# codex-storage/nim-groth16

Hardware: AMD Instinct MI355X
Metric: proofs/sec (BN254 Groth16, 2^20-constraint circuit) (higher is better)
Workload: dtype u32 (254-bit Montgomery: 8x32-bit limbs; 9x29-bit limbs in the bucket accumulation); 1 GPU; BN254 2^20-constraint synthetic R1CS (squaring chain, m=2^20-2), full prove: buildABC + 6 NTT + 4 G1 MSM + 1 G2 MSM, snarkjs flavour, 1 proof/step/GPU (3 proofs in flight per GPU, one shared key); mode=replica, nvars=1048576, domain_log2=20

## Files before the change

### include/g16hip.h

```cpp
#ifndef G16HIP_H
#define G16HIP_H

#include <stddef.h>
#include <stdint.h>

#ifdef __cplusplus
extern "C" {
#endif

#define G16_OK 0
#define G16_EINVAL (-1)
#define G16_ENODEV (-2)
#define G16_EHIP (-3)
#define G16_ENOMEM (-4)
#define G16_ESELFTEST (-5)

typedef struct g16_ctx g16_ctx;
typedef struct g16_points g16_points;

#define G16_SCALARS_MONT 1u
#define G16_SCALARS_STD 0u
#define G16_SCALARS_DEVICE 2u
#define G16_OUT_PARTIAL 4u
#define G16_OUT_DEVICE 8u
#define G16_NO_HOST_SYNC 32u

int32_t g16_ctx_create(int32_t device, g16_ctx** out);
void g16_ctx_destroy(g16_ctx* ctx);
const char* g16_last_error(const g16_ctx* ctx);
int32_t g16_ctx_set_stream(g16_ctx* ctx, void* hip_stream);
int32_t g16_ctx_synchronize(g16_ctx* ctx);
int32_t g16_ctx_cancel(g16_ctx* ctx);
int32_t g16_selftest(g16_ctx* ctx);

int32_t g16_msm_g1(g16_ctx* ctx, const void* scalars, uint32_t scalar_flags, const void* points, size_t n,
                   void* out_affine);
int32_t g16_msm_g2(g16_ctx* ctx, const void* scalars, uint32_t scalar_flags, const void* points, size_t n,
                   void* out_affine);
int32_t g16_msm_g1_dev(g16_ctx* ctx, const void* d_scalars, uint32_t scalar_flags, const void* d_points, size_t n,
                       void* out_affine);
int32_t g16_msm_g2_dev(g16_ctx* ctx, const void* d_scalars, uint32_t scalar_flags, const void* d_points, size_t n,
                       void* out_affine);
int32_t g16_msm_g1_partial_dev(g16_ctx* ctx, const void* d_scalars, uint32_t scalar_flags, const void* d_points,
                               size_t n, void* out_xyzz);
int32_t g16_msm_g2_partial_dev(g16_ctx* ctx, const void* d_scalars, uint32_t scalar_flags, const void* d_points,
                               size_t n, void* out_xyzz);
int32_t g16_g1_sum_partials(g16_ctx* ctx, const void* xyzz, size_t count, void* out_affine);
int32_t g16_g2_sum_partials(g16_ctx* ctx, const void* xyzz, size_t count, void* out_affine);

int32_t g16_points_register_g1(g16_ctx* ctx, const void* points, size_t n, g16_points** out);
int32_t g16_points_register_g2(g16_ctx* ctx, const void* points, size_t n, g16_points** out);
int32_t g16_points_register_g1_dev(g16_ctx* ctx, const void* d_points, size_t n, g16_points** out);
int32_t g16_points_register_g2_dev(g16_ctx* ctx, const void* d_points, size_t n, g16_points** out);
void g16_points_release(g16_points* pts);
size_t g16_points_count(const g16_points* pts);
size_t g16_points_inf_count(const g16_points* pts);
int32_t g16_points_info(const g16_points* pts, uint32_t* window_bits, uint32_t* ntables);

int32_t g16_points_register_g1_lean(g16_ctx* ctx, const void* points, size_t n, uint32_t table_stride, g16_points** out);
int32_t g16_points_register_g2_lean(g16_ctx* ctx, const void* points, size_t n, uint32_t table_stride, g16_points** out);
int32_t g16_points_register_g1_lean_dev(g16_ctx* ctx, const void* d_points, size_t n, uint32_t table_stride,
                                        g16_points** out);
int32_t g16_points_register_g2_lean_dev(g16_ctx* ctx, const void* d_points, size_t n, uint32_t table_stride,
                                        g16_points** out);
int32_t g16_points_table_bytes(const g16_points* pts, size_t* bytes);
int32_t g16_points_plan(int group, size_t n, uint32_t table_stride, uint32_t* window_bits, uint32_t* ntables,
                        size_t* bytes);
int32_t g16_msm_points(g16_ctx* ctx, const g16_points* pts, const void* scalars, uint32_t flags, void* out);

int32_t g16_points_check_g1(g16_ctx* ctx, const void* points, size_t n, size_t* first_bad);
int32_t g16_points_check_g2(g16_ctx* ctx, const void* points, size_t n, size_t* first_bad);

int32_t g16_fixed_base_g1(g16_ctx* ctx, const void* scalars, uint32_t scalar_flags, size_t n, void* out_points);
int32_t g16_fixed_base_g2(g16_ctx* ctx, const void* scalars, uint32_t scalar_flags, size_t n, void* out_points);

typedef struct {
  uint32_t nvars, npubs, nconstraints;
  uint32_t flavour;
  const uint32_t* row[3];
  const uint32_t* col[3];
  const void* val[3];
  size_t nnz[3];
  uint32_t flags;
  const void *alpha, *beta, *gamma, *delta, *tau;
} g16_setup_desc;
typedef struct {
  void *alpha1, *beta1, *delta1;
  void *beta2, *gamma2, *delta2;
  void* pointsIC;
  void *pointsA1, *pointsB1;
  void* pointsB2;
  void* pointsC1;
  void* pointsH1;
} g16_setup_points;
int32_t g16_setup_log2_domain(const g16_setup_desc* desc, uint32_t* log2_domain);
int32_t g16_fake_setup(g16_ctx* ctx, const g16_setup_desc* desc, g16_setup_points* out);
int32_t g16_lagrange_fr(g16_ctx* ctx, uint32_t log2n, uint32_t first, uint32_t step, size_t count, const void* tau,
                        const void* scale, void* out);
int32_t g16_powers_fr(g16_ctx* ctx, const void* base, const void* scale, size_t count, void* out);

typedef struct g16_r1cs_desc_s g16_r1cs_desc;
typedef struct g16_ptau_desc_s g16_ptau_desc;
int32_t g16_points_intt_g1(g16_ctx* ctx, const void* points, uint32_t log2n, void* out);
int32_t g16_points_intt_g2(g16_ctx* ctx, const void* points, uint32_t log2n, void* out);
int32_t g16_circuit_setup(g16_ctx* ctx, const g16_r1cs_desc* r1cs, const g16_ptau_desc* ptau, const void* delta,
                          g16_setup_points* out);

int32_t g16_ntt_fr(g16_ctx* ctx, const void* src, void* dst, uint32_t log2n, int32_t inverse);
int32_t g16_ntt_fr_dev(g16_ctx* ctx, const void* d_src, void* d_dst, uint32_t log2n, int32_t inverse);

#define G16_FLAVOUR_JENSGROTH 0u
#define G16_FLAVOUR_SNARKJS 1u
int32_t g16_quotient(g16_ctx* ctx, const void* Az, const void* Bz, const void* Cz, uint32_t log2n, uint32_t flavour,
                     void* out);
int32_t g16_quotient_dev(g16_ctx* ctx, const void* d_Az, const void* d_Bz, const void* d_Cz, uint32_t log2n,
                         uint32_t flavour, void* d_out);

typedef struct g16_pkey g16_pkey;
typedef struct {
  uint32_t matrix;
  uint32_t row;
  uint32_t col;
  uint32_t reserved;
  uint8_t value[32];
} g16_coeff;
typedef struct {
  uint32_t nvars, npubs;
  uint32_t log2_domain;
  uint32_t flavour;
  const void *pointsA1, *pointsB1;
  const void* pointsB2;
  const void* pointsC1;
  const void* pointsH1;
  const g16_coeff* coeffs;
  size_t ncoeffs;
  const void *alpha1, *beta1, *delta1;
  const void *beta2, *delta2;
  uint32_t shard_index, shard_count;
} g16_pkey_desc;
typedef struct {
  uint8_t pi_a[64];
  uint8_t pi_b[128];
  uint8_t pi_c[64];
} g16_proof;
int32_t g16_pkey_create(g16_ctx* ctx, const g16_pkey_desc* desc, g16_pkey** out);
int32_t g16_pkey_create_zkey(g16_ctx* ctx, const g16_pkey_desc* desc, const void* section4, size_t section4_bytes,
                             g16_pkey** out);
int32_t g16_pkey_create_lean(g16_ctx* ctx, const g16_pkey_desc* desc, uint32_t table_stride, g16_pkey** out);
int32_t g16_pkey_create_zkey_lean(g16_ctx* ctx, const g16_pkey_desc* desc, const void* section4, size_t section4_bytes,
                                  uint32_t table_stride, g16_pkey** out);
void g16_pkey_destroy(g16_pkey* key);
int32_t g16_pkey_inf_counts(const g16_pkey* key, size_t out[8]);
int32_t g16_pkey_b1_fold(const g16_pkey* key, size_t out[3]);
int32_t g16_pkey_b1_sparse(const g16_pkey* key, size_t out[3]);
int32_t g16_prove(g16_ctx* ctx, const g16_pkey* key, const void* witness, uint32_t flags, const void* mask_r,
                  const void* mask_s, g16_proof* out);
#define G16_PARTIALS_BYTES 768
int32_t g16_prove_partials(g16_ctx* ctx, const g16_pkey* key, const void* witness, uint32_t flags, void* out_partials);
int32_t g16_prove_combine(g16_ctx* ctx, const g16_pkey* key, const void* partials, size_t count, uint32_t flags,
                          const void* mask_r, const void* mask_s, g16_proof* out);
int32_t g16_prove_partials_begin(g16_ctx* ctx, const g16_pkey* key, const void* witness, uint32_t flags,
                                 uint32_t task_mask, void* d_task_out);
int32_t g16_prove_partials_end(g16_ctx* ctx, const g16_pkey* key, const void* d_a1_slice, const void* d_b1_slice,
                               const void* d_c1_slice, uint32_t flags, void* out_partials);
int32_t g16_build_abc(g16_ctx* ctx, const g16_pkey* key, const void* witness, uint32_t flags, void* out_abc);
int32_t g16_pkey_abc_info(const g16_pkey* key, size_t out[11]);
int32_t g16_spmv_fr(g16_ctx* ctx, const uint32_t* row, const uint32_t* col, const void* val, size_t nnz, const void* x,
                    size_t ncols, size_t nrows, void* y);

typedef struct g16_group g16_group;
typedef struct g16_group_pkey g16_group_pkey;
int32_t g16_group_create(const int32_t* devices, int32_t ndev, g16_group** out);
void g16_group_destroy(g16_group* group);
int32_t g16_group_size(const g16_group* group);
const char* g16_group_last_error(const g16_group* group);
int32_t g16_group_pkey_create(g16_group* group, const g16_pkey_desc* desc, g16_group_pkey** out);
int32_t g16_group_pkey_create_lean(g16_group* group, const g16_pkey_desc* desc, uint32_t table_stride,
                                   g16_group_pkey** out);
void g16_group_pkey_destroy(g16_group_pkey* key);
int32_t g16_group_prove(g16_group* group, const g16_group_pkey* key, const void* witness, uint32_t flags,
                        const void* mask_r, const void* mask_s, g16_proof* out);

#define G16_EBUSY (-6)
typedef struct g16_prover g16_prover;
int32_t g16_prover_create(int32_t device, const g16_pkey* key, uint32_t depth, g16_prover** out);
void g16_prover_destroy(g16_prover* p);
const char* g16_prover_last_error(const g16_prover* p);
int32_t g16_prover_submit(g16_prover* p, const void* witness, uint32_t flags, const void* mask_r, const void* mask_s,
                          uint64_t* ticket);
int32_t g16_prover_poll(g16_prover* p, uint64_t ticket);
int32_t g16_prover_collect(g16_prover* p, uint64_t ticket, g16_proof* out);
int32_t g16_host_alloc(int32_t device, size_t bytes, void** out);
void g16_host_free(void* p);

typedef struct g16_vkey g16_vkey;
typedef struct {
  uint32_t npubs;
  const void* alpha1;
  const void* beta2;
  const void* gamma2;
  const void* delta2;
  const void* pointsIC;
} g16_vkey_desc;
#define G16_VERIFY_SUBGROUP 16u
#define G16_GT_BYTES 384
int32_t g16_vkey_create(g16_ctx* ctx, const g16_vkey_desc* desc, g16_vkey** out);
void g16_vkey_destroy(g16_vkey* key);
int32_t g16_verify(g16_ctx* ctx, const g16_vkey* key, const g16_proof* proofs, const void* public_io, uint32_t flags,
                   size_t count, int32_t* status);
int32_t g16_pairing(g16_ctx* ctx, const void* g1_points, const void* g2_points, size_t n, void* out_gt);
int32_t g16_verify_batch(g16_ctx* ctx, const g16_vkey* key, const g16_proof* proofs, const void* public_io,
                         uint32_t flags, size_t count, const void* multipliers, int32_t* result, int32_t* status);

int32_t g16_points_audit_g1(g16_ctx* ctx, const void* points, size_t n, size_t first_bad[3], size_t bad_count[3]);
int32_t g16_points_audit_g2(g16_ctx* ctx, const void* points, size_t n, size_t first_bad[3], size_t bad_count[3]);
int32_t g16_points_pairs_check(g16_ctx* ctx, const void* g1_points, const void* g2_points, size_t n,
                               const void* multipliers, int32_t* result);
#define G16_AUDIT_SECTIONS 13
enum {
  G16_SEC_ALPHA1 = 0, G16_SEC_BETA1, G16_SEC_DELTA1, G16_SEC_BETA2, G16_SEC_GAMMA2, G16_SEC_DELTA2, G16_SEC_POINTS_IC,
  G16_SEC_POINTS_A1, G16_SEC_POINTS_B1, G16_SEC_POINTS_B2, G16_SEC_POINTS_C1, G16_SEC_POINTS_H1, G16_SEC_COEFFS
};
#define G16_AUDIT_CANONICAL 1u
#define G16_AUDIT_CURVE 2u
#define G16_AUDIT_SUBGROUP 4u
#define G16_AUDIT_RELATION 8u
#define G16_AUDIT_SPEC_INFINITY 16u
typedef struct {
  uint32_t failed;
  uint32_t spec_infinity;
  int32_t relation[3];
  uint32_t reserved;
  size_t first_bad[G16_AUDIT_SECTIONS][3];
  size_t bad_count[G16_AUDIT_SECTIONS][3];
} g16_key_report;
int32_t g16_key_audit(g16_ctx* ctx, const g16_pkey_desc* desc, const g16_vkey_desc* vk, const void* section4,
                      size_t section4_bytes, const void* multipliers, g16_key_report* out);

struct g16_r1cs_desc_s {
  uint32_t nvars, npubs, nconstraints;
  uint32_t flavour;
  const uint32_t* row[3];
  const uint32_t* col[3];
  const void* val[3];
  size_t nnz[3];
  uint32_t flags;
};
struct g16_ptau_desc_s {
  uint32_t power;
  const void *tauG1, *tauG2, *alphaTauG1, *betaTauG1, *betaG2;
};
#define G16_PTAU_SECTIONS 5
#define G16_CIRCUIT_RELATIONS 9
enum {
  G16_PTAU_TAU_G1 = 0, G16_PTAU_TAU_G2, G16_PTAU_ALPHA_TAU_G1, G16_PTAU_BETA_TAU_G1, G16_PTAU_BETA_G2
};
enum {
  G16_REL_COEFFS_A = 0, G16_REL_COEFFS_B, G16_REL_SPEC, G16_REL_A1, G16_REL_B1, G16_REL_B2, G16_REL_C1, G16_REL_IC,
  G16_REL_H1
};
#define G16_CIRCUIT_KEY 1u
#define G16_CIRCUIT_PTAU 2u
#define G16_CIRCUIT_COEFFS 4u
#define G16_CIRCUIT_SPEC 8u
#define G16_CIRCUIT_POINTS 16u
typedef struct {
  g16_key_report key;
  size_t ptau_first_bad[G16_PTAU_SECTIONS][3];
  size_t ptau_bad_count[G16_PTAU_SECTIONS][3];
  int32_t relation[G16_CIRCUIT_RELATIONS];
  uint32_t failed;
  size_t first_row[2];
} g16_circuit_report;
int32_t g16_circuit_audit(g16_ctx* ctx, const g16_pkey_desc* desc, const g16_vkey_desc* vk, const void* section4,
                          size_t section4_bytes, const g16_r1cs_desc* r1cs, const g16_ptau_desc* ptau,
                          const void* wire_multipliers, const void* h_multipliers, g16_circuit_report* out);

int32_t g16_points_scale_g1(g16_ctx* ctx, const void* points, size_t n, const void* k, uint32_t flags, void* out);
int32_t g16_points_scale_g2(g16_ctx* ctx, const void* points, size_t n, const void* k, uint32_t flags, void* out);

typedef struct {
  const void *delta1, *delta2;
  const void *pointsC1, *pointsH1;
  size_t nc1, nh1;
} g16_phase2_key;
typedef struct {
  uint8_t delta_after[64];
  uint8_t g1_s[64], g1_sx[64];
  uint8_t g2_spx[128];
} g16_contribution;
typedef struct {
  void *delta1, *delta2, *pointsC1, *pointsH1;
  g16_contribution* record;
} g16_phase2_out;
int32_t g16_key_contribute(g16_ctx* ctx, const g16_phase2_key* key, const void* d, const void* s, uint32_t flags,
                           const void* challenge_g2, g16_phase2_out* out);

#define G16_CHAIN_ARRAYS 9
enum {
  G16_CHAIN_DELTA_AFTER = 0, G16_CHAIN_G1_S, G16_CHAIN_G1_SX, G16_CHAIN_G2_SPX, G16_CHAIN_CHALLENGES,
  G16_CHAIN_FINAL_DELTA1, G16_CHAIN_FINAL_DELTA2, G16_CHAIN_FINAL_POINTS_C1, G16_CHAIN_FINAL_POINTS_H1
};
#define G16_CHAIN_RELATIONS 7
enum {
  G16_CHAIN_ELEMENTS = 0, G16_CHAIN_POK, G16_CHAIN_STEP, G16_CHAIN_LAST, G16_CHAIN_DELTA, G16_CHAIN_C1, G16_CHAIN_H1
};
typedef struct {
  uint32_t failed;
  int32_t relation[G16_CHAIN_RELATIONS];
  size_t first_record[2];
  size_t first_bad[G16_CHAIN_ARRAYS][3];
  size_t bad_count[G16_CHAIN_ARRAYS][3];
  size_t first_infinity[G16_CHAIN_ARRAYS];
} g16_chain_report;
int32_t g16_contributions_verify(g16_ctx* ctx, const g16_phase2_key* initial, const g16_phase2_key* final_,
                                 const g16_contribution* records, const void* challenges_g2, size_t count,
                                 const void* c1_multipliers, const void* h1_multipliers, g16_chain_report* out);

int32_t g16_profile_enable(g16_ctx* ctx, int32_t on);
int32_t g16_profile_reset(g16_ctx* ctx);
int32_t g16_profile_report(g16_ctx* ctx, char* buf, size_t buflen);
int32_t g16_profile_clock(g16_ctx* ctx, double* ghz);

#ifdef __cplusplus
}
#endif
#endif
```

### nim_groth16_amd/_lib.py

```python
from __future__ import annotations

import ctypes
import json
import os
import weakref

_HERE = os.path.dirname(os.path.abspath(__file__))

G16_OK, G16_EINVAL, G16_ENODEV, G16_EHIP, G16_ENOMEM, G16_ESELFTEST, G16_EBUSY = 0, -1, -2, -3, -4, -5, -6
SCALARS_MONT, SCALARS_STD, SCALARS_DEVICE, OUT_PARTIAL, OUT_DEVICE, NO_HOST_SYNC = 1, 0, 2, 4, 8, 32
PARTIALS_BYTES = 768

SYMBOLS = [
    "g16_ctx_create", "g16_ctx_destroy", "g16_last_error", "g16_ctx_set_stream", "g16_ctx_synchronize",
    "g16_selftest", "g16_msm_g1", "g16_msm_g2", "g16_msm_g1_dev", "g16_msm_g2_dev",
    "g16_msm_g1_partial_dev", "g16_msm_g2_partial_dev", "g16_g1_sum_partials", "g16_g2_sum_partials",
    "g16_points_register_g1", "g16_points_register_g2", "g16_points_register_g1_dev",
    "g16_points_register_g2_dev", "g16_points_release", "g16_points_count", "g16_points_inf_count", "g16_points_info", "g16_msm_points",
    "g16_points_check_g1", "g16_points_check_g2", "g16_fixed_base_g1", "g16_fixed_base_g2", "g16_quotient", "g16_quotient_dev", "g16_pkey_create",
    "g16_pkey_create_zkey", "g16_pkey_destroy", "g16_pkey_inf_counts", "g16_prove", "g16_build_abc", "g16_pkey_abc_info", "g16_spmv_fr", "g16_prove_partials", "g16_prove_combine",
    "g16_prove_partials_begin", "g16_prove_partials_end",
    "g16_ntt_fr", "g16_ntt_fr_dev", "g16_profile_enable", "g16_profile_reset", "g16_profile_report", "g16_profile_clock",
    "g16_vkey_create", "g16_vkey_destroy", "g16_verify", "g16_verify_batch", "g16_pairing",
    "g16_ctx_cancel", "g16_group_create", "g16_group_destroy", "g16_group_size", "g16_group_last_error",
    "g16_group_pkey_create", "g16_group_pkey_destroy", "g16_group_prove",
    "g16_prover_create", "g16_prover_destroy", "g16_prover_last_error", "g16_prover_submit", "g16_prover_poll",
    "g16_prover_collect", "g16_host_alloc", "g16_host_free",
    "g16_points_register_g1_lean", "g16_points_register_g2_lean", "g16_points_register_g1_lean_dev",
    "g16_points_register_g2_lean_dev", "g16_points_table_bytes", "g16_points_plan", "g16_pkey_create_lean",
    "g16_pkey_create_zkey_lean", "g16_group_pkey_create_lean",
    "g16_setup_log2_domain", "g16_fake_setup", "g16_lagrange_fr", "g16_powers_fr",
    "g16_points_audit_g1", "g16_points_audit_g2", "g16_points_pairs_check", "g16_key_audit",
    "g16_pkey_b1_fold", "g16_pkey_b1_sparse", "g16_circuit_audit",
    "g16_points_intt_g1", "g16_points_intt_g2", "g16_circuit_setup",
    "g16_points_scale_g1", "g16_points_scale_g2", "g16_key_contribute", "g16_contributions_verify",
]
VERIFY_SUBGROUP = 16
GT_BYTES = 384


class PkeyDesc(ctypes.Structure):
    _fields_ = [("nvars", ctypes.c_uint32), ("npubs", ctypes.c_uint32), ("log2_domain", ctypes.c_uint32),
                ("flavour", ctypes.c_uint32),
                ("pointsA1", ctypes.c_void_p), ("pointsB1", ctypes.c_void_p), ("pointsB2", ctypes.c_void_p),
                ("pointsC1", ctypes.c_void_p), ("pointsH1", ctypes.c_void_p),
                ("coeffs", ctypes.c_void_p), ("ncoeffs", ctypes.c_size_t),
                ("alpha1", ctypes.c_void_p), ("beta1", ctypes.c_void_p), ("delta1", ctypes.c_void_p),
                ("beta2", ctypes.c_void_p), ("delta2", ctypes.c_void_p),
                ("shard_index", ctypes.c_uint32), ("shard_count", ctypes.c_uint32)]


class VkeyDesc(ctypes.Structure):
    _fields_ = [("npubs", ctypes.c_uint32), ("alpha1", ctypes.c_void_p), ("beta2", ctypes.c_void_p),
                ("gamma2", ctypes.c_void_p), ("delta2", ctypes.c_void_p), ("pointsIC", ctypes.c_void_p)]


class SetupDesc(ctypes.Structure):
    _fields_ = [("nvars", ctypes.c_uint32), ("npubs", ctypes.c_uint32), ("nconstraints", ctypes.c_uint32),
                ("flavour", ctypes.c_uint32),
                ("row", ctypes.c_void_p * 3), ("col", ctypes.c_void_p * 3), ("val", ctypes.c_void_p * 3),
                ("nnz", ctypes.c_size_t * 3), ("flags", ctypes.c_uint32),
                ("alpha", ctypes.c_void_p), ("beta", ctypes.c_void_p), ("gamma", ctypes.c_void_p),
                ("delta", ctypes.c_void_p), ("tau", ctypes.c_void_p)]


SETUP_POINTS = ("alpha1", "beta1", "delta1", "beta2", "gamma2", "delta2", "pointsIC", "pointsA1", "pointsB1", "pointsB2",
                "pointsC1", "pointsH1")


class SetupPoints(ctypes.Structure):
    _fields_ = [(name, ctypes.c_void_p) for name in SETUP_POINTS]


AUDIT_SECTIONS = ("alpha1", "beta1", "delta1", "beta2", "gamma2", "delta2", "pointsIC", "pointsA1", "pointsB1", "pointsB2",
                  "pointsC1", "pointsH1", "coeffs")
AUDIT_CHECKS = ("canonical", "curve", "subgroup")
AUDIT_RELATIONS = ("pointsB1~pointsB2", "beta1~beta2", "delta1~delta2")
AUDIT_CANONICAL, AUDIT_CURVE, AUDIT_SUBGROUP, AUDIT_RELATION, AUDIT_SPEC_INFINITY = 1, 2, 4, 8, 16


class KeyReportC(ctypes.Structure):
    _fields_ = [("failed", ctypes.c_uint32), ("spec_infinity", ctypes.c_uint32), ("relation", ctypes.c_int32 * 3),
                ("reserved", ctypes.c_uint32),
                ("first_bad", (ctypes.c_size_t * 3) * len(AUDIT_SECTIONS)),
                ("bad_count", (ctypes.c_size_t * 3) * len(AUDIT_SECTIONS))]


class KeyReport:

    def __init__(self, failed, spec_infinity, relation, first_bad, bad_count):
        self.failed, self.spec_infinity, self.relation = failed, spec_infinity, list(relation)
        self.first_bad, self.bad_count = first_bad, bad_count

    @property
    def ok(self) -> bool:
        return self.failed == 0

    def as_dict(self) -> dict:
        return {"failed": self.failed, "spec_infinity": self.spec_infinity, "relation": self.relation,
                "first_bad": self.first_bad, "bad_count": self.bad_count}

    def findings(self):
        out = []
        for s, name in enumerate(AUDIT_SECTIONS):
            for k, check in enumerate(AUDIT_CHECKS):
                if self.bad_count[s][k]:
                    what = {"canonical": "is not a canonical encoding", "curve": "is not on the curve",
                            "subgroup": "is not in the order-r subgroup"}[check]
                    more = self.bad_count[s][k] - 1
                    out.append(f"{name}[{self.first_bad[s][k]}] {what}" + (f" (and {more} more)" if more else ""))
        for k, name in enumerate(AUDIT_RELATIONS):
            if self.relation[k] == 0:
                out.append(f"{name}: not the same multiples of the two generators")
        for s in range(6):
            if self.spec_infinity >> s & 1:
                out.append(f"{AUDIT_SECTIONS[s]} is the point at infinity")
        return out

    def __str__(self):
        if self.ok:
            skipped = [AUDIT_RELATIONS[k] for k in range(3) if self.relation[k] < 0]
            return "key audit: ok" + (f" (not run: {', '.join(skipped)})" if skipped else "")
        return "key audit: FAILED\n" + "\n".join("  " + f for f in self.findings())


class R1csDesc(ctypes.Structure):
    _fields_ = [("nvars", ctypes.c_uint32), ("npubs", ctypes.c_uint32), ("nconstraints", ctypes.c_uint32),
                ("flavour", ctypes.c_uint32),
                ("row", ctypes.c_void_p * 3), ("col", ctypes.c_void_p * 3), ("val", ctypes.c_void_p * 3),
                ("nnz", ctypes.c_size_t * 3), ("flags", ctypes.c_uint32)]


class PtauDesc(ctypes.Structure):
    _fields_ = [("power", ctypes.c_uint32), ("tauG1", ctypes.c_void_p), ("tauG2", ctypes.c_void_p),
                ("alphaTauG1", ctypes.c_void_p), ("betaTauG1", ctypes.c_void_p), ("betaG2", ctypes.c_void_p)]


PTAU_SECTIONS = ("tauG1", "tauG2", "alphaTauG1", "betaTauG1", "betaG2")
PTAU_GROUP = {"tauG1": 1, "tauG2": 2, "alphaTauG1": 1, "betaTauG1": 1, "betaG2": 2}
CIRCUIT_RELATIONS = ("COEFFS_A", "COEFFS_B", "SPEC", "A1", "B1", "B2", "C1", "IC", "H1")
CIRCUIT_KEY, CIRCUIT_PTAU, CIRCUIT_COEFFS, CIRCUIT_SPEC, CIRCUIT_POINTS = 1, 2, 4, 8, 16


class CircuitReportC(ctypes.Structure):
    _fields_ = [("key", KeyReportC),
                ("ptau_first_bad", (ctypes.c_size_t * 3) * len(PTAU_SECTIONS)),
                ("ptau_bad_count", (ctypes.c_size_t * 3) * len(PTAU_SECTIONS)),
                ("relation", ctypes.c_int32 * len(CIRCUIT_RELATIONS)), ("failed", ctypes.c_uint32),
                ("first_row", ctypes.c_size_t * 2)]


class CircuitReport:

    def __init__(self, key: KeyReport, ptau_first_bad, ptau_bad_count, relation, failed, first_row):
        self.key, self.ptau_first_bad, self.ptau_bad_count = key, ptau_first_bad, ptau_bad_count
        self.relation, self.failed, self.first_row = list(relation), failed, list(first_row)

    @property
    def ok(self) -> bool:
        return self.failed == 0

    def as_dict(self) -> dict:
        return {"key": self.key.as_dict(), "ptau_first_bad": self.ptau_first_bad, "ptau_bad_count": self.ptau_bad_count,
                "relation": self.relation, "failed": self.failed, "first_row": self.first_row}

    def findings(self):
        out = list(self.key.findings())
        for s, name in enumerate(PTAU_SECTIONS):
            for k, check in enumerate(AUDIT_CHECKS):
                if self.ptau_bad_count[s][k]:
                    what = {"canonical": "is not a canonical encoding", "curve": "is not on the curve",
                            "subgroup": "is not in the order-r subgroup"}[check]
                    more = self.ptau_bad_count[s][k] - 1
                    out.append(f"ptau {name}[{self.ptau_first_bad[s][k]}] {what}" + (f" (and {more} more)" if more else ""))
        for m in range(2):
            if self.relation[m] == 0:
                out.append(f"coeffs: matrix {'AB'[m]} differs from the r1cs first at row {self.first_row[m]}")
        if self.relation[2] == 0:
            out.append("alpha1 / beta1 / beta2 are not those of the powers of tau (or its first powers are not the generators)")
        for k in range(3, len(CIRCUIT_RELATIONS)):
            if self.relation[k] == 0:
                out.append(f"points{CIRCUIT_RELATIONS[k]} does not belong to the circuit")
        return out

    def __str__(self):
        if self.ok:
            skipped = [AUDIT_RELATIONS[k] for k in range(3) if self.key.relation[k] < 0]
            skipped += [CIRCUIT_RELATIONS[k] for k in range(len(CIRCUIT_RELATIONS)) if self.relation[k] < 0]
            return "circuit audit: ok" + (f" (not run: {', '.join(skipped)})" if skipped else "")
        return "circuit audit: FAILED\n" + "\n".join("  " + f for f in self.findings())


class Phase2Key(ctypes.Structure):
    _fields_ = [("delta1", ctypes.c_void_p), ("delta2", ctypes.c_void_p), ("pointsC1", ctypes.c_void_p),
                ("pointsH1", ctypes.c_void_p), ("nc1", ctypes.c_size_t), ("nh1", ctypes.c_size_t)]


class ContributionC(ctypes.Structure):
    _fields_ = [("delta_after", ctypes.c_uint8 * 64), ("g1_s", ctypes.c_uint8 * 64), ("g1_sx", ctypes.c_uint8 * 64),
                ("g2_spx", ctypes.c_uint8 * 128)]


CONTRIBUTION_BYTES = 320
assert ctypes.sizeof(ContributionC) == CONTRIBUTION_BYTES


class Phase2Out(ctypes.Structure):
    _fields_ = [("delta1", ctypes.c_void_p), ("delta2", ctypes.c_void_p), ("pointsC1", ctypes.c_void_p),
                ("pointsH1", ctypes.c_void_p), ("record", ctypes.POINTER(ContributionC))]


CHAIN_ARRAYS = ("delta_after", "g1_s", "g1_sx", "g2_spx", "challenges", "final delta1", "final delta2", "final pointsC1",
                "final pointsH1")
CHAIN_RELATIONS = ("ELEMENTS", "POK", "STEP", "LAST", "DELTA", "C1", "H1")


class ChainReportC(ctypes.Structure):
    _fields_ = [("failed", ctypes.c_uint32), ("relation", ctypes.c_int32 * len(CHAIN_RELATIONS)),
                ("first_record", ctypes.c_size_t * 2),
                ("first_bad", (ctypes.c_size_t * 3) * len(CHAIN_ARRAYS)),
                ("bad_count", (ctypes.c_size_t * 3) * len(CHAIN_ARRAYS)),
                ("first_infinity", ctypes.c_size_t * len(CHAIN_ARRAYS))]


class ChainReport:

    def __init__(self, failed, relation, first_record, first_bad, bad_count, first_infinity, transcript=None):
        self.failed, self.relation, self.first_record = failed, list(relation), list(first_record)
        self.first_bad, self.bad_count, self.first_infinity = first_bad, bad_count, list(first_infinity)
        self.transcript = transcript

    @property
    def ok(self) -> bool:
        return self.failed == 0 and self.transcript != 0

    def as_dict(self) -> dict:
        return {"failed": self.failed, "relation": self.relation, "first_record": self.first_record,
                "first_bad": self.first_bad, "bad_count": self.bad_count, "first_infinity": self.first_infinity,
                "transcript": self.transcript}

    def findings(self):
        out = []
        if self.transcript == 0:
            out.append("the transcript hashes are not those of the initial key and the records")
        for a, name in enumerate(CHAIN_ARRAYS):
            for k, check in enumerate(AUDIT_CHECKS):
                if self.bad_count[a][k]:
                    what = {"canonical": "is not a canonical encoding", "curve": "is not on the curve",
                            "subgroup": "is not in the order-r subgroup"}[check]
                    more = self.bad_count[a][k] - 1
                    out.append(f"{name}[{self.first_bad[a][k]}] {what}" + (f" (and {more} more)" if more else ""))
            if self.first_infinity[a] is not None:
                out.append(f"{name}[{self.first_infinity[a]}] is the point at infinity")
        if self.relation[1] == 0:
            out.append(f"record {self.first_record[0]}: the proof of knowledge does not hold")
        if self.relation[2] == 0:
            out.append(f"record {self.first_record[1]}: delta_after is not the contribution's multiple of the delta before")
        if self.relation[3] == 0:
            out.append("the final delta1 is not the last record's delta_after")
        if self.relation[4] == 0:
            out.append("the final delta1 / delta2 are not the same multiple of the two generators")
        for k in (5, 6):
            if self.relation[k] == 0:
                out.append(f"the final points{CHAIN_RELATIONS[k]} is not the initial one rescaled by the deltas")
        return out

    def __str__(self):
        if self.ok:
            skipped = [CHAIN_RELATIONS[k] for k in range(len(CHAIN_RELATIONS)) if self.relation[k] < 0]
            return "contribution chain: ok" + (f" (not run: {', '.join(skipped)})" if skipped else "")
        return "contribution chain: FAILED\n" + "\n".join("  " + f for f in self.findings())


class G16Error(RuntimeError):
    def __init__(self, code, msg):
        super().__init__(f"g16hip error {code}: {msg}")
        self.code = code


def lib_path() -> str:
    return os.environ.get("G16HIP_LIB", os.path.join(_HERE, "csrc", "libg16hip.so"))


def device_code_sha16(path: str = None) -> str:
    import hashlib
    import struct
    b = open(path or lib_path(), "rb").read()
    h = hashlib.sha256()
    try:
        assert b[:4] == b"\x7fELF" and b[4] == 2
        shoff = struct.unpack_from("<Q", b, 0x28)[0]
        shentsize, shnum, shstrndx = struct.unpack_from("<HHH", b, 0x3A)

        def sh(i):
            name, _typ, _flags, _addr, off, size = struct.unpack_from("<IIQQQQ", b, shoff + i * shentsize)
            return name, off, size
        _, stro, _ = sh(shstrndx)
        hit = False
        for i in range(shnum):
            n, off, size = sh(i)
            if b[stro + n: b.index(b"\0", stro + n)] == b".hip_fatbin":
                h.update(b[off: off + size])
                hit = True
        assert hit
    except Exception:
        h = hashlib.sha256(b)
    return h.hexdigest()[:16]


_lib = None


def load_library():
    global _lib
    if _lib is not None:
        return _lib
    path = lib_path()
    if not os.path.exists(path):
        raise G16Error(G16_ENODEV, f"{path} not found: build it with `make -C nim_groth16_amd/csrc` "
                                   "(or __graft_entry__.build()); there is no CPU fallback")
    try:
        import torch
    except ImportError:
        pass
    lib = ctypes.CDLL(path)
    vp, u32, i32, sz = ctypes.c_void_p, ctypes.c_uint32, ctypes.c_int32, ctypes.c_size_t
    lib.g16_ctx_create.argtypes = [i32, ctypes.POINTER(vp)]
    lib.g16_ctx_destroy.argtypes = [vp]
    lib.g16_ctx_destroy.restype = None
    lib.g16_last_error.argtypes = [vp]
    lib.g16_last_error.restype = ctypes.c_char_p
    lib.g16_ctx_set_stream.argtypes = [vp, vp]
    lib.g16_ctx_synchronize.argtypes = [vp]
    lib.g16_selftest.argtypes = [vp]
    for name in ("g16_msm_g1", "g16_msm_g2", "g16_msm_g1_dev", "g16_msm_g2_dev",
                 "g16_msm_g1_partial_dev", "g16_msm_g2_partial_dev"):
        getattr(lib, name).argtypes = [vp, vp, u32, vp, sz, vp]
    for name in ("g16_g1_sum_partials", "g16_g2_sum_partials"):
        getattr(lib, name).argtypes = [vp, vp, sz, vp]
    for name in ("g16_points_register_g1", "g16_points_register_g2", "g16_points_register_g1_dev",
                 "g16_points_register_g2_dev"):
        getattr(lib, name).argtypes = [vp, vp, sz, ctypes.POINTER(vp)]
    for name in ("g16_points_register_g1_lean", "g16_points_register_g2_lean", "g16_points_register_g1_lean_dev",
                 "g16_points_register_g2_lean_dev"):
        getattr(lib, name).argtypes = [vp, vp, sz, u32, ctypes.POINTER(vp)]
    lib.g16_points_table_bytes.argtypes = [vp, ctypes.POINTER(sz)]
    lib.g16_points_plan.argtypes = [ctypes.c_int, sz, u32, ctypes.POINTER(u32), ctypes.POINTER(u32), ctypes.POINTER(sz)]
    lib.g16_pkey_create_lean.argtypes = [vp, ctypes.POINTER(PkeyDesc), u32, ctypes.POINTER(vp)]
    lib.g16_pkey_create_zkey_lean.argtypes = [vp, ctypes.POINTER(PkeyDesc), vp, sz, u32, ctypes.POINTER(vp)]
    lib.g16_group_pkey_create_lean.argtypes = [vp, ctypes.POINTER(PkeyDesc), u32, ctypes.POINTER(vp)]
    lib.g16_points_release.argtypes = [vp]
    lib.g16_points_release.restype = None
    lib.g16_points_count.argtypes = [vp]
    lib.g16_points_count.restype = sz
    lib.g16_points_inf_count.argtypes = [vp]
    lib.g16_points_inf_count.restype = sz
    lib.g16_pkey_inf_counts.argtypes = [vp, ctypes.POINTER(sz)]
    lib.g16_pkey_b1_fold.argtypes = [vp, ctypes.POINTER(sz)]
    lib.g16_pkey_b1_sparse.argtypes = [vp, ctypes.POINTER(sz)]
    lib.g16_points_info.argtypes = [vp, ctypes.POINTER(u32), ctypes.POINTER(u32)]
    lib.g16_msm_points.argtypes = [vp, vp, vp, u32, vp]
    lib.g16_points_check_g1.argtypes = [vp, vp, sz, ctypes.POINTER(sz)]
    lib.g16_points_check_g2.argtypes = [vp, vp, sz, ctypes.POINTER(sz)]
    lib.g16_fixed_base_g1.argtypes = [vp, vp, u32, sz, vp]
    lib.g16_fixed_base_g2.argtypes = [vp, vp, u32, sz, vp]
    lib.g16_quotient.argtypes = [vp, vp, vp, vp, u32, u32, vp]
    lib.g16_quotient_dev.argtypes = [vp, vp, vp, vp, u32, u32, vp]
    lib.g16_pkey_create.argtypes = [vp, ctypes.POINTER(PkeyDesc), ctypes.POINTER(vp)]
    lib.g16_pkey_create_zkey.argtypes = [vp, ctypes.POINTER(PkeyDesc), vp, sz, ctypes.POINTER(vp)]
    lib.g16_pkey_destroy.argtypes = [vp]
    lib.g16_pkey_destroy.restype = None
    lib.g16_prove.argtypes = [vp, vp, vp, u32, vp, vp, vp]
    lib.g16_build_abc.argtypes = [vp, vp, vp, u32, vp]
    lib.g16_pkey_abc_info.argtypes = [vp, ctypes.POINTER(sz)]
    lib.g16_spmv_fr.argtypes = [vp, vp, vp, vp, sz, vp, sz, sz, vp]
    lib.g16_prove_partials.argtypes = [vp, vp, vp, u32, vp]
    lib.g16_prove_combine.argtypes = [vp, vp, vp, sz, u32, vp, vp, vp]
    lib.g16_prove_partials_begin.argtypes = [vp, vp, vp, u32, u32, vp]
    lib.g16_prove_partials_end.argtypes = [vp, vp, vp, vp, vp, u32, vp]
    lib.g16_ntt_fr.argtypes = [vp, vp, vp, u32, i32]
    lib.g16_ntt_fr_dev.argtypes = [vp, vp, vp, u32, i32]
    lib.g16_vkey_create.argtypes = [vp, ctypes.POINTER(VkeyDesc), ctypes.POINTER(vp)]
    lib.g16_vkey_destroy.argtypes = [vp]
    lib.g16_vkey_destroy.restype = None
    lib.g16_verify.argtypes = [vp, vp, vp, vp, u32, sz, ctypes.POINTER(i32)]
    lib.g16_verify_batch.argtypes = [vp, vp, vp, vp, u32, sz, vp, ctypes.POINTER(i32), ctypes.POINTER(i32)]
    lib.g16_pairing.argtypes = [vp, vp, vp, sz, vp]
    lib.g16_ctx_cancel.argtypes = [vp]
    lib.g16_group_create.argtypes = [ctypes.POINTER(i32), i32, ctypes.POINTER(vp)]
    lib.g16_group_destroy.argtypes = [vp]
    lib.g16_group_destroy.restype = None
    lib.g16_group_size.argtypes = [vp]
    lib.g16_group_last_error.argtypes = [vp]
    lib.g16_group_last_error.restype = ctypes.c_char_p
    lib.g16_group_pkey_create.argtypes = [vp, ctypes.POINTER(PkeyDesc), ctypes.POINTER(vp)]
    lib.g16_group_pkey_destroy.argtypes = [vp]
    lib.g16_group_pkey_destroy.restype = None
    lib.g16_group_prove.argtypes = [vp, vp, vp, u32, vp, vp, vp]
    lib.g16_prover_create.argtypes = [i32, vp, u32, ctypes.POINTER(vp)]
    lib.g16_prover_destroy.argtypes = [vp]
    lib.g16_prover_destroy.restype = None
    lib.g16_prover_last_error.argtypes = [vp]
    lib.g16_prover_last_error.restype = ctypes.c_char_p
    lib.g16_prover_submit.argtypes = [vp, vp, u32, vp, vp, ctypes.POINTER(ctypes.c_uint64)]
    lib.g16_prover_poll.argtypes = [vp, ctypes.c_uint64]
    lib.g16_prover_collect.argtypes = [vp, ctypes.c_uint64, vp]
    lib.g16_host_alloc.argtypes = [i32, sz, ctypes.POINTER(vp)]
    lib.g16_host_free.argtypes = [vp]
    lib.g16_host_free.restype = None
    lib.g16_profile_enable.argtypes = [vp, i32]
    lib.g16_profile_reset.argtypes = [vp]
    lib.g16_profile_report.argtypes = [vp, ctypes.c_char_p, sz]
    lib.g16_profile_clock.argtypes = [vp, ctypes.POINTER(ctypes.c_double)]
    lib.g16_setup_log2_domain.argtypes = [ctypes.POINTER(SetupDesc), ctypes.POINTER(u32)]
    lib.g16_fake_setup.argtypes = [vp, ctypes.POINTER(SetupDesc), ctypes.POINTER(SetupPoints)]
    lib.g16_lagrange_fr.argtypes = [vp, u32, u32, u32, sz, vp, vp, vp]
    lib.g16_powers_fr.argtypes = [vp, vp, vp, sz, vp]
    lib.g16_points_audit_g1.argtypes = [vp, vp, sz, ctypes.POINTER(sz), ctypes.POINTER(sz)]
    lib.g16_points_audit_g2.argtypes = [vp, vp, sz, ctypes.POINTER(sz), ctypes.POINTER(sz)]
    lib.g16_points_pairs_check.argtypes = [vp, vp, vp, sz, vp, ctypes.POINTER(i32)]
    lib.g16_key_audit.argtypes = [vp, ctypes.POINTER(PkeyDesc), ctypes.POINTER(VkeyDesc), vp, sz, vp,
                                  ctypes.POINTER(KeyReportC)]
    lib.g16_circuit_audit.argtypes = [vp, ctypes.POINTER(PkeyDesc), ctypes.POINTER(VkeyDesc), vp, sz,
                                      ctypes.POINTER(R1csDesc), ctypes.POINTER(PtauDesc), vp, vp,
                                      ctypes.POINTER(CircuitReportC)]
    lib.g16_points_intt_g1.argtypes = [vp, vp, u32, vp]
    lib.g16_points_intt_g2.argtypes = [vp, vp, u32, vp]
    lib.g16_circuit_setup.argtypes = [vp, ctypes.POINTER(R1csDesc), ctypes.POINTER(PtauDesc), vp,
                                      ctypes.POINTER(SetupPoints)]
    lib.g16_points_scale_g1.argtypes = [vp, vp, sz, vp, u32, vp]
    lib.g16_points_scale_g2.argtypes = [vp, vp, sz, vp, u32, vp]
    lib.g16_key_contribute.argtypes = [vp, ctypes.POINTER(Phase2Key), vp, vp, u32, vp, ctypes.POINTER(Phase2Out)]
    lib.g16_contributions_verify.argtypes = [vp, ctypes.POINTER(Phase2Key), ctypes.POINTER(Phase2Key),
                                             ctypes.POINTER(ContributionC), vp, sz, vp, vp, ctypes.POINTER(ChainReportC)]
    for name in SYMBOLS:
        if name not in ("g16_ctx_destroy", "g16_last_error", "g16_points_release", "g16_points_count",
                        "g16_points_inf_count",
                        "g16_pkey_destroy", "g16_vkey_destroy", "g16_group_destroy", "g16_group_last_error",
                        "g16_group_pkey_destroy", "g16_prover_destroy", "g16_prover_last_error", "g16_host_free"):
            getattr(lib, name).restype = i32
    _lib = lib
    return lib


def _buf(b):
    if isinstance(b, int):
        return ctypes.c_void_p(b)
    if isinstance(b, (bytes, bytearray)):
        return ctypes.cast(ctypes.c_char_p(bytes(b)), ctypes.c_void_p) if isinstance(b, bytes) else \
            ctypes.cast((ctypes.c_char * len(b)).from_buffer(b), ctypes.c_void_p)
    if hasattr(b, "ctypes"):
        return ctypes.c_void_p(b.ctypes.data)
    raise TypeError(type(b))


class Context:

    def __init__(self, device: int = 0):
        self._lib = load_library()
        h = ctypes.c_void_p()
        rc = self._lib.g16_ctx_create(device, ctypes.byref(h))
        if rc != G16_OK:
            raise G16Error(rc, "g16_ctx_create failed (no usable HIP device?)")
        self._h = h
        self.device = device
        self._children = weakref.WeakSet()

    def close(self, release_children: bool = False):
        if getattr(self, "_h", None):
            if release_children:
                for child in list(self._children):
                    child._free()
            self._lib.g16_ctx_destroy(self._h)
            self._h = None

    def __del__(self):
        try:
            self.close()
        except Exception:
            pass

    def _check(self, rc):
        if rc != G16_OK:
            raise G16Error(rc, self._lib.g16_last_error(self._h).decode())

    def selftest(self):
        self._check(self._lib.g16_selftest(self._h))

    def set_stream(self, stream_ptr):
        self._check(self._lib.g16_ctx_set_stream(self._h, ctypes.c_void_p(stream_ptr)))

    def synchronize(self):
        self._check(self._lib.g16_ctx_synchronize(self._h))

    def cancel(self):
        self._check(self._lib.g16_ctx_cancel(self._h))

    def msm(self, group: int, scalars, points, n: int, mont: bool = True, device: bool = False,
            partial: bool = False) -> bytes:
        psz = 64 if group == 1 else 128
        out = ctypes.create_string_buffer(2 * psz if partial else psz)
        if partial:
            fn = self._lib.g16_msm_g1_partial_dev if group == 1 else self._lib.g16_msm_g2_partial_dev
        elif device:
            fn = self._lib.g16_msm_g1_dev if group == 1 else self._lib.g16_msm_g2_dev
        else:
            fn = self._lib.g16_msm_g1 if group == 1 else self._lib.g16_msm_g2
        s = _buf(scalars) if n else None
        p = _buf(points) if n else None
        self._check(fn(self._h, s, SCALARS_MONT if mont else SCALARS_STD, p, n, out))
        return out.raw

    def register_points(self, group: int, points, n: int, device: bool = False, table_stride: int = 0) -> "PointSet":
        h = ctypes.c_void_p()
        p = _buf(points) if n else None
        if table_stride:
            name = f"g16_points_register_g{group}_lean" + ("_dev" if device else "")
            self._check(getattr(self._lib, name)(self._h, p, n, table_stride, ctypes.byref(h)))
        else:
            name = f"g16_points_register_g{group}" + ("_dev" if device else "")
            self._check(getattr(self._lib, name)(self._h, p, n, ctypes.byref(h)))
        return PointSet(self, h, group, n)

    def msm_points(self, pts: "PointSet", scalars, mont: bool = True, device: bool = False,
                   partial: bool = False) -> bytes:
        psz = 64 if pts.group == 1 else 128
        out = ctypes.create_string_buffer(2 * psz if partial else psz)
        flags = (SCALARS_MONT if mont else 0) | (SCALARS_DEVICE if device else 0) | (OUT_PARTIAL if partial else 0)
        self._check(self._lib.g16_msm_points(self._h, pts._h, _buf(scalars) if pts.n else None, flags, out))
        return out.raw

    def points_check(self, group: int, points: bytes):
        psz = 64 if group == 1 else 128
        n = len(points) // psz
        bad = ctypes.c_size_t()
        fn = self._lib.g16_points_check_g1 if group == 1 else self._lib.g16_points_check_g2
        self._check(fn(self._h, _buf(points) if n else None, n, ctypes.byref(bad)))
        return None if bad.value == ctypes.c_size_t(-1).value else bad.value

    def points_audit(self, group: int, points: bytes):
        psz = 64 if group == 1 else 128
        assert len(points) % psz == 0
        n = len(points) // psz
        first, count = (ctypes.c_size_t * 3)(), (ctypes.c_size_t * 3)()
        fn = self._lib.g16_points_audit_g1 if group == 1 else self._lib.g16_points_audit_g2
        self._check(fn(self._h, _buf(points) if n else None, n, first, count))
        none = ctypes.c_size_t(-1).value
        return [None if f == none else f for f in first], list(count)

    def pairs_check(self, g1_points: bytes, g2_points: bytes, multipliers) -> bool:
        n = len(g1_points) // 64
        assert len(g1_points) == 64 * n and len(g2_points) == 128 * n and len(multipliers) == n
        zs = b"".join(int(z).to_bytes(16, "little") for z in multipliers)
        res = ctypes.c_int32(-1)
        self._check(self._lib.g16_points_pairs_check(self._h, _buf(g1_points) if n else None,
                                                     _buf(g2_points) if n else None, n, _buf(zs) if n else None,
                                                     ctypes.byref(res)))
        return res.value == 1

    def key_audit(self, desc: PkeyDesc, vk: VkeyDesc = None, section4: bytes = None, multipliers=None) -> KeyReport:
        zs = None
        if isinstance(multipliers, (bytes, bytearray)):
            assert len(multipliers) == 16 * desc.nvars, "one multiplier per wire"
            zs = bytes(multipliers)
        elif multipliers is not None:
            assert len(multipliers) == desc.nvars, "one multiplier per wire"
            zs = b"".join(int(z).to_bytes(16, "little") for z in multipliers)
        rep = KeyReportC()
        self._check(self._lib.g16_key_audit(self._h, ctypes.byref(desc), ctypes.byref(vk) if vk is not None else None,
                                            _buf(section4) if section4 is not None else None,
                                            len(section4) if section4 is not None else 0,
                                            _buf(zs) if zs is not None else None, ctypes.byref(rep)))
        none = ctypes.c_size_t(-1).value
        return KeyReport(rep.failed, rep.spec_infinity, list(rep.relation),
                         [[None if f == none else f for f in row] for row in rep.first_bad],
                         [list(row) for row in rep.bad_count])

    def circuit_audit(self, desc: PkeyDesc, vk, section4, r1cs: R1csDesc, ptau: PtauDesc, wire_multipliers,
                      h_multipliers) -> CircuitReport:
        def enc(zs, n, what):
            if isinstance(zs, (bytes, bytearray)):
                assert len(zs) == 16 * n, f"one {what} multiplier of 16 bytes each"
                return bytes(zs)
            assert len(zs) == n, f"{n} {what} multipliers"
            return b"".join(int(z).to_bytes(16, "little") for z in zs)
        zw = enc(wire_multipliers, desc.nvars, "wire")
        zh = enc(h_multipliers, 1 << min(desc.log2_domain, 28), "h")
        rep = CircuitReportC()
        self._check(self._lib.g16_circuit_audit(self._h, ctypes.byref(desc), ctypes.byref(vk) if vk is not None else None,
                                                _buf(section4) if section4 is not None else None,
                                                len(section4) if section4 is not None else 0,
                                                ctypes.byref(r1cs), ctypes.byref(ptau), _buf(zw), _buf(zh),
                                                ctypes.byref(rep)))
        none = ctypes.c_size_t(-1).value
        fix = lambda rows: [[None if f == none else f for f in row] for row in rows]
        key = KeyReport(rep.key.failed, rep.key.spec_infinity, list(rep.key.relation), fix(rep.key.first_bad),
                        [list(row) for row in rep.key.bad_count])
        return CircuitReport(key, fix(rep.ptau_first_bad), [list(row) for row in rep.ptau_bad_count], list(rep.relation),
                             rep.failed, [None if f == none else f for f in rep.first_row])

    def fixed_base(self, group: int, scalars: bytes, mont: bool = True) -> bytes:
        n = len(scalars) // 32
        psz = 64 if group == 1 else 128
        out = ctypes.create_string_buffer(max(n, 1) * psz)
        fn = self._lib.g16_fixed_base_g1 if group == 1 else self._lib.g16_fixed_base_g2
        self._check(fn(self._h, _buf(scalars) if n else None, SCALARS_MONT if mont else 0, n, out))
        return out.raw[: n * psz]

    def spmv(self, row, col, val, x: bytes, nrows: int) -> bytes:
        import numpy as np
        row = np.ascontiguousarray(row, dtype=np.uint32)
        col = np.ascontiguousarray(col, dtype=np.uint32)
        nnz = len(row)
        if not isinstance(val, (bytes, bytearray)):
            val = np.ascontiguousarray(val, dtype=np.uint8)
        assert len(col) == nnz and (len(val) if isinstance(val, (bytes, bytearray)) else val.size) == 32 * nnz
        out = ctypes.create_string_buffer(max(1, 32 * nrows))
        self._check(self._lib.g16_spmv_fr(self._h, _buf(row) if nnz else None, _buf(col) if nnz else None,
                                          _buf(val) if nnz else None, nnz, _buf(x) if len(x) else None, len(x) // 32,
                                          nrows, out))
        return out.raw[: 32 * nrows]

    def lagrange(self, log2n: int, tau: bytes, first: int = 0, step: int = 1, count: int = None,
                 scale: bytes = None) -> bytes:
        if count is None:
            count = ((1 << log2n) - first + step - 1) // step if step else 1
        out = ctypes.create_string_buffer(max(1, 32 * count))
        self._check(self._lib.g16_lagrange_fr(self._h, log2n, first, step, count, _buf(tau),
                                              _buf(scale) if scale is not None else None, out))
        return out.raw[: 32 * count]

    def powers(self, base: bytes, count: int, scale: bytes = None) -> bytes:
        out = ctypes.create_string_buffer(max(1, 32 * count))
        self._check(self._lib.g16_powers_fr(self._h, _buf(base), _buf(scale) if scale is not None else None, count, out))
        return out.raw[: 32 * count]

    def fake_setup(self, nvars: int, npubs: int, nconstraints: int, flavour: int, matrices, toxic, mont: bool = True):
        import numpy as np
        d = SetupDesc()
        d.nvars, d.npubs, d.nconstraints, d.flavour = nvars, npubs, nconstraints, flavour
        d.flags = SCALARS_MONT if mont else SCALARS_STD
        keep = []
        for k, (rows, wires, vals) in enumerate(matrices):
            rows = np.ascontiguousarray(rows, dtype=np.uint32)
            wires = np.ascontiguousarray(wires, dtype=np.uint32)
            if not isinstance(vals, (bytes, bytearray)):
                vals = np.ascontiguousarray(vals, dtype=np.uint8)
            nnz = len(rows)
            assert len(wires) == nnz and (len(vals) if isinstance(vals, (bytes, bytearray)) else vals.size) == 32 * nnz
            keep += [rows, wires, vals]
            d.nnz[k] = nnz
            if nnz:
                d.row[k], d.col[k], d.val[k] = (_buf(x).value for x in (rows, wires, vals))
        toxic = [bytes(t) for t in toxic]
        d.alpha, d.beta, d.gamma, d.delta, d.tau = (_buf(t).value for t in toxic)
        log2 = ctypes.c_uint32()
        rc = self._lib.g16_setup_log2_domain(ctypes.byref(d), ctypes.byref(log2))
        if rc != G16_OK:
            raise G16Error(rc, "g16_setup_log2_domain failed")
        sizes = dict(alpha1=64, beta1=64, delta1=64, beta2=128, gamma2=128, delta2=128, pointsIC=64 * (npubs + 1),
                     pointsA1=64 * nvars, pointsB1=64 * nvars, pointsB2=128 * nvars,
                     pointsC1=64 * max(0, nvars - npubs - 1), pointsH1=64 << min(log2.value, 40))
        if log2.value + (1 if flavour == 1 else 0) > 28:
            sizes = dict.fromkeys(sizes, 0)
        o = SetupPoints()
        bufs = {}
        for name, nbytes in sizes.items():
            bufs[name] = ctypes.create_string_buffer(max(1, nbytes))
            setattr(o, name, ctypes.cast(bufs[name], ctypes.c_void_p).value)
        self._check(self._lib.g16_fake_setup(self._h, ctypes.byref(d), ctypes.byref(o)))
        return log2.value, {name: bufs[name].raw[: sizes[name]] for name in SETUP_POINTS}

    def points_intt(self, group: int, points: bytes, log2n: int) -> bytes:
        psz = 64 if group == 1 else 128
        assert len(points) == psz << log2n, f"2^{log2n} points of {psz} bytes"
        out = ctypes.create_string_buffer(len(points))
        fn = self._lib.g16_points_intt_g1 if group == 1 else self._lib.g16_points_intt_g2
        self._check(fn(self._h, _buf(points), log2n, out))
        return out.raw

    def circuit_setup(self, r1cs: R1csDesc, ptau: PtauDesc, delta: bytes = None):
        nvars, npubs = r1cs.nvars, r1cs.npubs
        log2 = max(0, (r1cs.nconstraints + npubs).bit_length())
        sizes = dict(alpha1=64, beta1=64, delta1=64, beta2=128, gamma2=128, delta2=128, pointsIC=64 * (npubs + 1),
                     pointsA1=64 * nvars, pointsB1=64 * nvars, pointsB2=128 * nvars,
                     pointsC1=64 * max(0, nvars - npubs - 1), pointsH1=64 << log2)
        if log2 > 24:
            sizes = dict.fromkeys(sizes, 0)
        o = SetupPoints()
        bufs = {}
        for name, nbytes in sizes.items():
            bufs[name] = ctypes.create_string_buffer(max(1, nbytes))
            setattr(o, name, ctypes.cast(bufs[name], ctypes.c_void_p).value)
        self._check(self._lib.g16_circuit_setup(self._h, ctypes.byref(r1cs), ctypes.byref(ptau),
                                                _buf(bytes(delta)) if delta is not None else None, ctypes.byref(o)))
        return log2, {name: bufs[name].raw[: sizes[name]] for name in SETUP_POINTS}

    def points_scale(self, group: int, points: bytes, k: bytes, mont: bool = True) -> bytes:
        psz = 64 if group == 1 else 128
        assert len(points) % psz == 0 and len(k) == 32, f"points of {psz} bytes and a 32-byte scalar"
        out = ctypes.create_string_buffer(max(1, len(points)))
        fn = self._lib.g16_points_scale_g1 if group == 1 else self._lib.g16_points_scale_g2
        self._check(fn(self._h, _buf(bytes(points)), len(points) // psz, _buf(bytes(k)),
                       SCALARS_MONT if mont else SCALARS_STD, out))
        return out.raw[: len(points)]

    @staticmethod
    def _phase2_key(key: dict):
        assert len(key["delta1"]) == 64 and len(key["delta2"]) == 128, "delta1: 64 bytes, delta2: 128 bytes"
        assert len(key["pointsC1"]) % 64 == 0 and len(key["pointsH1"]) % 64 == 0, "G1 points of 64 bytes"
        keep = {name: bytes(key[name]) for name in ("delta1", "delta2", "pointsC1", "pointsH1")}
        pk = Phase2Key()
        for name, b in keep.items():
            setattr(pk, name, ctypes.cast(ctypes.c_char_p(b), ctypes.c_void_p).value if b else None)
        pk.nc1, pk.nh1 = len(keep["pointsC1"]) // 64, len(keep["pointsH1"]) // 64
        return pk, keep

    def key_contribute(self, key: dict, d: bytes, s: bytes, challenge_g2: bytes, mont: bool = True):
        assert len(d) == 32 and len(s) == 32 and len(challenge_g2) == 128
        pk, keep = self._phase2_key(key)
        bufs = {name: ctypes.create_string_buffer(max(1, len(b))) for name, b in keep.items()}
        rec = ContributionC()
        o = Phase2Out()
        for name in bufs:
            setattr(o, name, ctypes.cast(bufs[name], ctypes.c_void_p).value)
        o.record = ctypes.pointer(rec)
        self._check(self._lib.g16_key_contribute(self._h, ctypes.byref(pk), _buf(bytes(d)), _buf(bytes(s)),
                                                 SCALARS_MONT if mont else SCALARS_STD, _buf(bytes(challenge_g2)),
                                                 ctypes.byref(o)))
        return {name: bufs[name].raw[: len(keep[name])] for name in keep}, bytes(rec)

    def contributions_verify(self, initial: dict, final: dict, records, challenges_g2, c1_multipliers,
                             h1_multipliers) -> ChainReport:
        def enc(zs, n, what):
            if isinstance(zs, (bytes, bytearray)):
                assert len(zs) == 16 * n, f"one {what} multiplier of 16 bytes each"
                return bytes(zs)
            assert len(zs) == n, f"{n} {what} multipliers"
            return b"".join(int(z).to_bytes(16, "little") for z in zs)
        records, challenges_g2 = list(records), list(challenges_g2)
        assert len(records) == len(challenges_g2) and all(len(r) == CONTRIBUTION_BYTES for r in records) and \
            all(len(c) == 128 for c in challenges_g2), "one 320-byte record and one 128-byte challenge per contribution"
        ki, keep_i = self._phase2_key(initial)
        kf, keep_f = self._phase2_key(final)
        zc, zh = enc(c1_multipliers, kf.nc1, "c1"), enc(h1_multipliers, kf.nh1, "h1")
        recs = (ContributionC * max(1, len(records))).from_buffer_copy(b"".join(records) or bytes(CONTRIBUTION_BYTES))
        ch = b"".join(challenges_g2)
        rep = ChainReportC()
        self._check(self._lib.g16_contributions_verify(self._h, ctypes.byref(ki), ctypes.byref(kf), recs,
                                                       _buf(ch) if ch else None, len(records),
                                                       _buf(zc) if zc else None, _buf(zh) if zh else None,
                                                       ctypes.byref(rep)))
        none = ctypes.c_size_t(-1).value
        opt = lambda row: [None if f == none else f for f in row]
        return ChainReport(rep.failed, list(rep.relation), opt(rep.first_record), [opt(row) for row in rep.first_bad],
                           [list(row) for row in rep.bad_count], opt(rep.first_infinity))

    def quotient(self, Az, Bz, Cz, log2n: int, flavour: int, out=None, device: bool = False):
        if device:
            self._check(self._lib.g16_quotient_dev(self._h, _buf(Az), _buf(Bz), _buf(Cz), log2n, flavour, _buf(out)))
            return None
        res = ctypes.create_string_buffer(32 << log2n)
        self._check(self._lib.g16_quotient(self._h, _buf(Az), _buf(Bz), _buf(Cz), log2n, flavour, res))
        return res.raw

    def sum_partials(self, group: int, xyzz: bytes, count: int) -> bytes:
        psz = 64 if group == 1 else 128
        out = ctypes.create_string_buffer(psz)
        fn = self._lib.g16_g1_sum_partials if group == 1 else self._lib.g16_g2_sum_partials
        self._check(fn(self._h, _buf(xyzz) if count else None, count, out))
        return out.raw

    def ntt(self, src, log2n: int, inverse: bool, dst=None, device: bool = False):
        n = 1 << log2n
        if device:
            self._check(self._lib.g16_ntt_fr_dev(self._h, _buf(src), _buf(dst), log2n, 1 if inverse else 0))
            return None
        out = ctypes.create_string_buffer(32 * n)
        self._check(self._lib.g16_ntt_fr(self._h, _buf(src), out, log2n, 1 if inverse else 0))
        return out.raw

    def pairing(self, g1_points: bytes, g2_points: bytes) -> bytes:
        n = len(g1_points) // 64
        assert len(g1_points) == 64 * n and len(g2_points) == 128 * n
        out = ctypes.create_string_buffer(max(1, GT_BYTES * n))
        self._check(self._lib.g16_pairing(self._h, _buf(g1_points) if n else None, _buf(g2_points) if n else None,
                                          n, out))
        return out.raw[:GT_BYTES * n]

    def profile(self, on):
        self._check(self._lib.g16_profile_enable(self._h, int(on)))

    def profile_reset(self):
        self._check(self._lib.g16_profile_reset(self._h))

    def profile_clock(self) -> float:
        g = ctypes.c_double()
        self._check(self._lib.g16_profile_clock(self._h, ctypes.byref(g)))
        return g.value

    def profile_report(self) -> dict:
        buf = ctypes.create_string_buffer(1 << 16)
        self._check(self._lib.g16_profile_report(self._h, buf, len(buf)))
        return json.loads(buf.value.decode())


class ProvingKey:

    def __init__(self, ctx: Context, desc: PkeyDesc, keepalive, section4: bytes = None, table_stride: int = 0):
        self.ctx = ctx
        h = ctypes.c_void_p()
        if table_stride and section4 is not None:
            ctx._check(ctx._lib.g16_pkey_create_zkey_lean(ctx._h, ctypes.byref(desc), _buf(section4), len(section4),
                                                          table_stride, ctypes.byref(h)))
        elif table_stride:
            ctx._check(ctx._lib.g16_pkey_create_lean(ctx._h, ctypes.byref(desc), table_stride, ctypes.byref(h)))
        elif section4 is not None:
            ctx._check(ctx._lib.g16_pkey_create_zkey(ctx._h, ctypes.byref(desc), _buf(section4), len(section4),
                                                     ctypes.byref(h)))
        else:
            ctx._check(ctx._lib.g16_pkey_create(ctx._h, ctypes.byref(desc), ctypes.byref(h)))
        self._h = h
        self.nvars, self.npubs, self.log2n = desc.nvars, desc.npubs, desc.log2_domain
        ctx._children.add(self)
        del keepalive

    def _check_len(self, witness):
        if isinstance(witness, (bytes, bytearray)) and len(witness) != 32 * self.nvars:
            raise ValueError(f"wrong witness length: {len(witness)} bytes, expected {32 * self.nvars}")

    def prove(self, witness, mont: bool = True, r: bytes = None, s: bytes = None, device: bool = False, ctx=None):
        c = ctx or self.ctx
        self._check_len(witness)
        out = ctypes.create_string_buffer(256)
        flags = (SCALARS_MONT if mont else 0) | (SCALARS_DEVICE if device else 0)
        c._check(c._lib.g16_prove(c._h, self._h, _buf(witness), flags, _buf(r) if r else None,
                                  _buf(s) if s else None, out))
        raw = out.raw
        return raw[0:64], raw[64:192], raw[192:256]

    def prove_partials(self, witness, mont: bool = True, device: bool = False, out=None, ctx=None):
        c = ctx or self.ctx
        self._check_len(witness)
        flags = (SCALARS_MONT if mont else 0) | (SCALARS_DEVICE if device else 0)
        if out is not None:
            c._check(c._lib.g16_prove_partials(c._h, self._h, _buf(witness), flags | OUT_DEVICE, _buf(out)))
            return None
        buf = ctypes.create_string_buffer(PARTIALS_BYTES)
        c._check(c._lib.g16_prove_partials(c._h, self._h, _buf(witness), flags, buf))
        return buf.raw

    def prove_partials_begin(self, witness, task_mask: int, task_out=None, mont: bool = True, device: bool = False,
                             ctx=None, nosync: bool = False):
        c = ctx or self.ctx
        self._check_len(witness)
        flags = (SCALARS_MONT if mont else 0) | (SCALARS_DEVICE if device else 0) | (NO_HOST_SYNC if nosync else 0)
        c._check(c._lib.g16_prove_partials_begin(c._h, self._h, _buf(witness), flags, task_mask,
                                                 _buf(task_out) if task_out is not None else None))

    def prove_partials_end(self, a1, b1, c1, out=None, ctx=None, nosync: bool = False):
        c = ctx or self.ctx
        ptr = lambda x: _buf(x) if x is not None else None
        if out is not None:
            c._check(c._lib.g16_prove_partials_end(c._h, self._h, ptr(a1), ptr(b1), ptr(c1),
                                                   OUT_DEVICE | (NO_HOST_SYNC if nosync else 0), _buf(out)))
            return None
        buf = ctypes.create_string_buffer(PARTIALS_BYTES)
        c._check(c._lib.g16_prove_partials_end(c._h, self._h, ptr(a1), ptr(b1), ptr(c1), 0, buf))
        return buf.raw

    def prove_combine(self, partials, count: int, r: bytes = None, s: bytes = None, device: bool = False, ctx=None):
        c = ctx or self.ctx
        out = ctypes.create_string_buffer(256)
        c._check(c._lib.g16_prove_combine(c._h, self._h, _buf(partials), count, SCALARS_DEVICE if device else 0,
                                          _buf(r) if r else None, _buf(s) if s else None, out))
        raw = out.raw
        return raw[0:64], raw[64:192], raw[192:256]

    def inf_counts(self) -> dict:
        out = (ctypes.c_size_t * 8)()
        self.ctx._check(self.ctx._lib.g16_pkey_inf_counts(self._h, out))
        v = list(out)
        return {"A1": v[0], "B1": v[1], "B2": v[2], "C1": v[3], "H1": v[4], "B1_and_B2": v[5],
                "compact_A": bool(v[6]), "compact_B": bool(v[7])}

    def b1_fold(self) -> dict:
        out = (ctypes.c_size_t * 3)()
        self.ctx._check(self.ctx._lib.g16_pkey_b1_fold(self._h, out))
        return {"form": ("PLAIN", "EMPTY", "DELTA")[out[0]], "live_b1": out[1], "live_delta": out[2]}

    def b1_sparse(self) -> dict:
        out = (ctypes.c_size_t * 3)()
        self.ctx._check(self.ctx._lib.g16_pkey_b1_sparse(self._h, out))
        return {"sparse": bool(out[0]), "live": out[1], "max": out[2]}

    def abc_info(self) -> dict:
        out = (ctypes.c_size_t * 11)()
        self.ctx._check(self.ctx._lib.g16_pkey_abc_info(self._h, out))
        v = list(out)
        names = ("L<=1", "L=2", "L<=4", "L<=8", "L<=16", "L<=32", "L<=64", "L<=128", "L>128")
        return {"ncoeffs": v[0], "dict_values": v[1], "rows_by_terms": dict(zip(names, v[2:]))}

    def build_abc(self, witness: bytes, mont: bool = True, ctx=None):
        c = ctx or self.ctx
        self._check_len(witness)
        n = 1 << self.log2n
        out = ctypes.create_string_buffer(3 * n * 32)
        c._check(c._lib.g16_build_abc(c._h, self._h, _buf(witness), SCALARS_MONT if mont else 0, out))
        raw = out.raw
        return raw[: 32 * n], raw[32 * n: 64 * n], raw[64 * n:]

    def _free(self):
        if self._h:
            self.ctx._lib.g16_pkey_destroy(self._h)
        self._h = None

    destroy = _free

    def __del__(self):
        try:
            self._free()
        except Exception:
            pass


class DeviceGroup:

    def __init__(self, devices):
        self._lib = load_library()
        arr = (ctypes.c_int32 * len(devices))(*devices)
        h = ctypes.c_void_p()
        rc = self._lib.g16_group_create(arr, len(devices), ctypes.byref(h))
        if rc != G16_OK:
            raise G16Error(rc, "g16_group_create failed")
        self._h, self.devices = h, list(devices)

    def _check(self, rc):
        if rc != G16_OK:
            raise G16Error(rc, self._lib.g16_group_last_error(self._h).decode())

    def size(self) -> int:
        return self._lib.g16_group_size(self._h)

    def load_key(self, desc: PkeyDesc, keepalive=None, table_stride: int = 0) -> "GroupKey":
        h = ctypes.c_void_p()
        if table_stride:
            self._check(self._lib.g16_group_pkey_create_lean(self._h, ctypes.byref(desc), table_stride, ctypes.byref(h)))
        else:
            self._check(self._lib.g16_group_pkey_create(self._h, ctypes.byref(desc), ctypes.byref(h)))
        return GroupKey(self, h, desc.nvars)

    def close(self):
        if getattr(self, "_h", None):
            self._lib.g16_group_destroy(self._h)
            self._h = None

    def __del__(self):
        try:
            self.close()
        except Exception:
            pass


class GroupKey:
    def __init__(self, group: DeviceGroup, handle, nvars: int):
        self.group, self._h, self.nvars = group, handle, nvars

    def prove(self, witness: bytes, mont: bool = True, r: bytes = None, s: bytes = None):
        if len(witness) != 32 * self.nvars:
            raise ValueError(f"wrong witness length: {len(witness)} bytes, expected {32 * self.nvars}")
        out = ctypes.create_string_buffer(256)
        g = self.group
        g._check(g._lib.g16_group_prove(g._h, self._h, _buf(witness), SCALARS_MONT if mont else 0,
                                        _buf(r) if r else None, _buf(s) if s else None, out))
        raw = out.raw
        return raw[0:64], raw[64:192], raw[192:256]

    def destroy(self):
        if self._h:
            self.group._lib.g16_group_pkey_destroy(self._h)
        self._h = None

    def __del__(self):
        try:
            self.destroy()
        except Exception:
            pass


class ProverPool:

    def __init__(self, pkey: ProvingKey, depth: int = 3, device: int = 0):
        self._lib = load_library()
        self.pkey, self.depth, self.device = pkey, depth, device
        h = ctypes.c_void_p()
        rc = self._lib.g16_prover_create(device, pkey._h, depth, ctypes.byref(h))
        if rc != G16_OK:
            raise G16Error(rc, "g16_prover_create failed (sharded key, key of another device, or depth not in 1..8)")
        self._h = h
        self._witness = {}

    def _check(self, rc):
        if rc == G16_EBUSY:
            raise G16Error(rc, f"{self.depth + 1} proofs outstanding: collect one first")
        if rc < 0:
            raise G16Error(rc, self._lib.g16_prover_last_error(self._h).decode())
        return rc

    def submit(self, witness, mont: bool = True, r: bytes = None, s: bytes = None, device: bool = False) -> int:
        self.pkey._check_len(witness)
        if isinstance(witness, HostBuffer) and witness.nbytes < 32 * self.pkey.nvars:
            raise ValueError("host buffer shorter than the witness")
        ptr = ctypes.c_void_p(witness.data_ptr()) if device and hasattr(witness, "data_ptr") else _buf(witness)
        t = ctypes.c_uint64()
        flags = (SCALARS_MONT if mont else 0) | (SCALARS_DEVICE if device else 0)
        self._check(self._lib.g16_prover_submit(self._h, ptr, flags, _buf(r) if r else None,
                                                _buf(s) if s else None, ctypes.byref(t)))
        self._witness[t.value] = witness
        return t.value

    def poll(self, ticket: int) -> bool:
        return self._check(self._lib.g16_prover_poll(self._h, ticket)) == 1

    def collect(self, ticket: int):
        out = ctypes.create_string_buffer(256)
        self._check(self._lib.g16_prover_collect(self._h, ticket, out))
        self._witness.pop(ticket, None)
        raw = out.raw
        return raw[0:64], raw[64:192], raw[192:256]

    def close(self):
        if getattr(self, "_h", None):
            self._lib.g16_prover_destroy(self._h)
            self._h = None
            self._witness.clear()

    def __del__(self):
        try:
            self.close()
        except Exception:
            pass


class HostBuffer:

    def __init__(self, nbytes: int, device: int = 0):
        import numpy as np
        self._lib = load_library()
        p = ctypes.c_void_p()
        rc = self._lib.g16_host_alloc(device, nbytes, ctypes.byref(p))
        if rc != G16_OK:
            raise G16Error(rc, "g16_host_alloc failed")
        self._p, self.nbytes = p, nbytes
        self.array = np.ctypeslib.as_array((ctypes.c_uint8 * nbytes).from_address(p.value))
        self.ctypes = self.array.ctypes

    @classmethod
    def from_bytes(cls, data: bytes, device: int = 0) -> "HostBuffer":
        import numpy as np
        b = cls(len(data), device)
        b.array[:] = np.frombuffer(data, dtype=np.uint8)
        return b

    def __len__(self):
        return self.nbytes

    def free(self):
        if getattr(self, "_p", None):
            self.array = self.ctypes = None
            self._lib.g16_host_free(self._p)
            self._p = None

    def __del__(self):
        try:
            self.free()
        except Exception:
            pass


class VerifyingKey:

    def __init__(self, ctx: Context, npubs: int, alpha1: bytes, beta2: bytes, gamma2: bytes, delta2: bytes,
                 pointsIC: bytes):
        assert len(alpha1) == 64 and len(beta2) == len(gamma2) == len(delta2) == 128
        assert len(pointsIC) == 64 * (npubs + 1), "pointsIC must hold npubs + 1 points"
        self.ctx, self.npubs = ctx, npubs
        bufs = [ctypes.create_string_buffer(x, len(x)) for x in (alpha1, beta2, gamma2, delta2, pointsIC)]
        a = [ctypes.cast(b, ctypes.c_void_p) for b in bufs]
        desc = VkeyDesc(npubs, a[0], a[1], a[2], a[3], a[4])
        h = ctypes.c_void_p()
        ctx._check(ctx._lib.g16_vkey_create(ctx._h, ctypes.byref(desc), ctypes.byref(h)))
        self._h = h
        ctx._children.add(self)

    def verify(self, proofs, public_io: bytes, mont: bool = True, subgroup: bool = False):
        n = len(proofs)
        assert len(public_io) == 32 * n * (self.npubs + 1)
        raw = b"".join(a + b + c for a, b, c in proofs)
        assert len(raw) == 256 * n
        st = (ctypes.c_int32 * max(n, 1))()
        flags = (SCALARS_MONT if mont else 0) | (VERIFY_SUBGROUP if subgroup else 0)
        self.ctx._check(self.ctx._lib.g16_verify(self.ctx._h, self._h, _buf(raw) if n else None,
                                                 _buf(public_io) if n else None, flags, n, st))
        return list(st)[:n]

    def verify_batch(self, proofs, public_io: bytes, mont: bool = True, multipliers=None, want_status: bool = False):
        n = len(proofs)
        assert len(public_io) == 32 * n * (self.npubs + 1)
        raw = b"".join(a + b + c for a, b, c in proofs)
        assert len(raw) == 256 * n
        if multipliers is None:
            import secrets
            multipliers = [secrets.randbelow((1 << 128) - 1) + 1 for _ in range(n)]
        assert len(multipliers) == n, "one multiplier per proof"
        zs = b"".join(int(z).to_bytes(16, "little") for z in multipliers)
        res = ctypes.c_int32(-1)
        st = (ctypes.c_int32 * max(n, 1))() if want_status else None
        flags = SCALARS_MONT if mont else 0
        self.ctx._check(self.ctx._lib.g16_verify_batch(self.ctx._h, self._h, _buf(raw) if n else None,
                                                       _buf(public_io) if n else None, flags, n,
                                                       _buf(zs) if n else None, ctypes.byref(res), st))
        return (res.value == 1, list(st)[:n]) if want_status else res.value == 1

    def _free(self):
        if self._h:
            self.ctx._lib.g16_vkey_destroy(self._h)
        self._h = None

    destroy = _free

    def __del__(self):
        try:
            self._free()
        except Exception:
            pass


def points_plan(group: int, n: int, table_stride: int = 0):
    lib = load_library()
    c, t, b = ctypes.c_uint32(), ctypes.c_uint32(), ctypes.c_size_t()
    rc = lib.g16_points_plan(group, n, table_stride, ctypes.byref(c), ctypes.byref(t), ctypes.byref(b))
    if rc != G16_OK:
        raise G16Error(rc, "g16_points_plan: bad group, or too many points for 31-bit entry indices")
    return c.value, t.value, b.value


class PointSet:

    def __init__(self, ctx: Context, handle, group: int, n: int):
        self.ctx, self._h, self.group, self.n = ctx, handle, group, n
        ctx._children.add(self)

    def inf_count(self) -> int:
        return self.ctx._lib.g16_points_inf_count(self._h)

    def info(self):
        c, w = ctypes.c_uint32(), ctypes.c_uint32()
        self.ctx._check(self.ctx._lib.g16_points_info(self._h, ctypes.byref(c), ctypes.byref(w)))
        return c.value, w.value

    @property
    def table_bytes(self) -> int:
        b = ctypes.c_size_t()
        self.ctx._check(self.ctx._lib.g16_points_table_bytes(self._h, ctypes.byref(b)))
        return b.value

    def _free(self):
        if self._h:
            self.ctx._lib.g16_points_release(self._h)
        self._h = None

    release = _free

    def __del__(self):
        try:
            self._free()
        except Exception:
            pass


_default_ctx = None


def default_context() -> Context:
    global _default_ctx
    if _default_ctx is None:
        _default_ctx = Context(int(os.environ.get("LOCAL_RANK", "0")))
    return _default_ctx
```

### nim_groth16_amd/csrc/g16_env.hpp

```cpp
#pragma once

struct G16Env {
  int msm_window = 0;
  int table_window = 0;
  int msm_seg = 0;
  char msm_sort = 0;
  int g1_lanes[3] = {3, 2, 0};
  char stream_prio[7] = "lhllln";
  int red_slice_log2 = 0;
  int inf_compact_pct = 10;
  int r2_width = -1;
  int ntt_tile = 2048;
  int quotient_first = 1;
  int lanes_after_quotient = 0;
  int g1_batch = 0;
  int mtab = 2;
  int chain_ch = 1;
  int tail_quad = 1;
  int red_chunk = 0;
  int cu_split = 0;
  int heavy_grid = 0;
  int cz_on_the_fly = 1;
  int abc_dict = 1;
  int g2_first = -1;
  int b1_fold = 1;
};
```

### nim_groth16_amd/csrc/g16_internal.hpp

```cpp
#pragma once
#include "../../include/g16hip.h"

#include <hip/hip_runtime.h>

#include <cstdio>
#include <cstring>
#include <map>
#include <string>
#include <vector>


#include "g16_env.hpp"
#include "hip_owners.hpp"
#include "msm_params.hpp"
#include "circuit_setup_plan.hpp"
#include "msm_plan.hpp"
#include "proof_plan.hpp"

const G16Env& g16_env();

struct ProfEntry {
  const char* name;
  Event e0, e1;
};

struct g16_ctx {
  int device = 0;
  hipStream_t stream = nullptr;
  Stream own_stream;
  std::string err;
  struct Buf {
    DevMem<> mem;
    size_t bytes = 0;
    void* p() const { return mem.get(); }
  };
  struct MsmSort {
    Buf buf;
    g16::MsmParams P;
    bool narrow_tail = false;
    uint32_t *count = nullptr, *cursor = nullptr, *offset = nullptr, *xoff = nullptr, *heavy = nullptr,
             *info = nullptr, *entries = nullptr, *perm = nullptr, *ghist = nullptr, *blk_base = nullptr, *tile_hist = nullptr;
    uint2* tmp = nullptr;
    uint32_t* slice_hist = nullptr;
    uint2* tiles2 = nullptr;
    uint2* tiles = nullptr;
    uint2* xseg = nullptr;
  };
  struct MsmLane {
    Stream stream;
    Event done;
    Buf acc;
  };
  MsmSort sort[4];
  MsmLane lane[5];
  Event ev[g16::EV_COUNT];
  Buf stage_s;
  Buf stage_p;
  Buf stage_p29;
  Buf stage_o;
  Buf ntt_tw;
  Buf ntt_tmp;
  Buf coset[2];
  Buf quot;
  Buf prove;
  Buf fb_table[2];
  bool fb_ready[2] = {false, false};
  DevMem<unsigned long long> clk_buf;
  const void* shard_begun = nullptr;
  uint32_t tw_log2n = 0xffffffffu;
  uint32_t coset_log2n[2] = {0xffffffffu, 0xffffffffu};
  bool profiling = false;
  bool prof_accum_only = false;
  std::vector<ProfEntry> prof;
  std::vector<Event> free_events;
};

inline int32_t g16_hip_check(std::string& err, const char* call, hipError_t e) {
  if (e == hipSuccess) return G16_OK;
  err = std::string(call) + ": " + hipGetErrorString(e);
  (void)hipGetLastError();
  return e == hipErrorOutOfMemory ? G16_ENOMEM : G16_EHIP;
}
#define HIPCHK(ctx, call)                                                          \
  do {                                                                             \
    if (int32_t hiprc__ = g16_hip_check((ctx)->err, #call, (call))) return hiprc__; \
  } while (0)

inline void ctx_quiesce(g16_ctx* ctx) {
  if (ctx->stream) (void)hipStreamSynchronize(ctx->stream);
  for (auto& l : ctx->lane)
    if (l.stream) (void)hipStreamSynchronize(l.stream.get());
}
struct SyncOnExit {
  hipStream_t stream;
  ~SyncOnExit() { (void)hipStreamSynchronize(stream); }
};

inline int32_t ctx_enter(g16_ctx* ctx, bool keep_shard = false) {
  HIPCHK(ctx, hipSetDevice(ctx->device));
  if (ctx->shard_begun && !keep_shard) {
    ctx_quiesce(ctx);
    ctx->shard_begun = nullptr;
  }
  return G16_OK;
}
#define CTX_ENTER(ctx)                              \
  do {                                              \
    if (int32_t rc__ = ctx_enter(ctx)) return rc__; \
  } while (0)
#define CTX_ENTER_KEEP(ctx)                               \
  do {                                                    \
    if (int32_t rc__ = ctx_enter(ctx, true)) return rc__; \
  } while (0)

inline int32_t ensure(g16_ctx* ctx, g16_ctx::Buf& b, size_t bytes) {
  if (b.bytes >= bytes) return G16_OK;
  HIPCHK(ctx, hipSetDevice(ctx->device));
  if (b.mem) {
    ctx_quiesce(ctx);
    b.mem.reset();
    b.bytes = 0;
  }
  size_t want = bytes + bytes / 8 + 4096;
  HIPCHK(ctx, dev_alloc(b.mem, want));
  b.bytes = want;
  return G16_OK;
}

#define G16_COMBINE_RES_BYTES 384
constexpr size_t STAGE_O_RESULT = 0, STAGE_O_RESULT_BYTES = G16_PARTIALS_BYTES;
constexpr size_t STAGE_O_COUNTERS = STAGE_O_RESULT + STAGE_O_RESULT_BYTES, STAGE_O_COUNTER_WORDS = 2;
constexpr size_t STAGE_O_COMBINE = 1024;
constexpr size_t STAGE_O_BYTES = 2048;
static_assert(STAGE_O_COUNTERS % 4 == 0 && STAGE_O_COUNTERS + 4 * STAGE_O_COUNTER_WORDS <= STAGE_O_COMBINE &&
                  STAGE_O_COMBINE % 128 == 0 && STAGE_O_COMBINE + G16_COMBINE_RES_BYTES <= STAGE_O_BYTES,
              "the pieces of stage_o overlap or do not fit");
inline int32_t ensure_stage_o(g16_ctx* ctx) { return ensure(ctx, ctx->stage_o, STAGE_O_BYTES); }
inline char* stage_o_at(g16_ctx* ctx, size_t offset) { return (char*)ctx->stage_o.p() + offset; }

template <class Launch>
inline int32_t counted_launch(g16_ctx* ctx, int fill, uint32_t* words, size_t nwords, Launch&& launch) {
  if (int32_t rc = ensure_stage_o(ctx)) return rc;
  uint32_t* d_words = (uint32_t*)stage_o_at(ctx, STAGE_O_COUNTERS);
  HIPCHK(ctx, hipMemsetAsync(d_words, fill, 4 * nwords, ctx->stream));
  if (int32_t rc = launch(d_words)) return rc;
  HIPCHK(ctx, hipMemcpyAsync(words, d_words, 4 * nwords, hipMemcpyDeviceToHost, ctx->stream));
  HIPCHK(ctx, hipStreamSynchronize(ctx->stream));
  return G16_OK;
}

struct ProfScope {
  g16_ctx* ctx;
  bool on;
  ProfEntry e;
  hipStream_t st;
  ProfScope(g16_ctx* c, const char* name, hipStream_t stream = nullptr)
      : ctx(c), on(c->profiling && (!c->prof_accum_only || strncmp(name, "msm_accum", 9) == 0)),
        st(stream ? stream : c->stream) {
    if (!on) return;
    e.name = name;
    auto get = [&](Event& ev) {
      if (!ctx->free_events.empty()) {
        ev = std::move(ctx->free_events.back());
        ctx->free_events.pop_back();
      } else {
        (void)event_create(ev, hipEventDefault);
      }
    };
    get(e.e0);
    get(e.e1);
    (void)hipEventRecord(e.e0.get(), st);
  }
  ~ProfScope() {
    if (!on) return;
    (void)hipEventRecord(e.e1.get(), st);
    ctx->prof.push_back(std::move(e));
  }
};
#define KLAUNCH_ON(ctx, stream_, name, kernel, grid, block, shmem, ...)                        \
  do {                                                                                         \
    ProfScope ps__(ctx, name, stream_);                                                        \
    hipLaunchKernelGGL(kernel, dim3(grid), dim3(block), shmem, stream_, __VA_ARGS__);          \
  } while (0)
#define KLAUNCH(ctx, name, kernel, grid, block, shmem, ...) \
  KLAUNCH_ON(ctx, (ctx)->stream, name, kernel, grid, block, shmem, __VA_ARGS__)


struct g16_points {
  int device = 0;
  int group = 1;
  size_t n = 0;
  uint32_t c = 0, nwin = 0;
  uint32_t mtab = 1;
  uint32_t stride = 1;
  uint32_t ntables() const { return mtab * ((nwin + stride - 1) / stride); }
  uint32_t cfg() const { return g16::msm_table_cfg(c, mtab, stride); }
  DevMem<> d_tables;
  DevMem<uint32_t> d_live;
  size_t n_inf = 0;
};
const uint32_t* g16_points_live_if_sparse(const g16_points* p);
int32_t g16_msm_sort(g16_ctx* ctx, hipStream_t stream, const void* d_scalars, uint32_t flags, size_t n,
                     uint32_t table_c, g16_ctx::MsmSort& sort, const uint32_t* d_live = nullptr);
struct g16_msm_sparse {
  const void* d_scalars;
  const uint32_t* d_wires;
  uint32_t nlive;
  const uint32_t* d_info;
};
struct g16_msm_run {
  const g16_ctx::MsmSort* sort;
  g16_ctx::Buf* acc;
  const void* d_points;
  void* d_out_aff;
  void* d_out_acc;
  const void* init_partial;
  const g16_msm_sparse* sparse = nullptr;
};
int32_t g16_msm_batch(g16_ctx* ctx, hipStream_t stream, int group, const g16_msm_run* runs, int n_accum, int n_tail,
                      hipEvent_t after_heavy);
inline const void* g16_msm_partial_ptr(const g16_ctx::Buf& acc) { return acc.p(); }
int32_t g16_lanes_init(g16_ctx* ctx);
int32_t g16_bitmap_or_device(g16_ctx* ctx, uint32_t* d_out, const uint32_t* d_a, const uint32_t* d_b, size_t n,
                             uint32_t* d_n_dead);

namespace g16 {
template <class C>
struct MsmBatch;
}
template <class C>
int32_t msm_device(g16_ctx* ctx, const void* d_scalars, uint32_t flags, const void* d_points, size_t n, void* d_out_aff,
                   void* d_out_acc, uint32_t table_c, const uint32_t* d_live = nullptr);
template <class C>
int32_t stage_accum(g16_ctx* ctx, hipStream_t st, const g16::MsmParams& P, const g16::MsmBatch<C>& B, uint32_t ny);
template <class C>
int32_t stage_accum_sparse(g16_ctx* ctx, hipStream_t st, const g16::MsmParams& P, const g16_msm_sparse& sp,
                           const void* d_points, void* d_partial, bool own_entry);
template <class C>
int32_t stage_heavy(g16_ctx* ctx, hipStream_t st, const g16::MsmParams& P, const g16::MsmTailPlan& T,
                    const g16::MsmBatch<C>& B, uint32_t ny);
template <class C>
int32_t stage_reduce1(g16_ctx* ctx, hipStream_t st, const g16::MsmParams& P, const g16::MsmTailPlan& T,
                      const g16::MsmBatch<C>& B, uint32_t ny);
template <class C>
int32_t stage_reduce2_fold(g16_ctx* ctx, hipStream_t st, const g16::MsmParams& P, const g16::MsmTailPlan& T,
                           const g16::MsmBatch<C>& B, uint32_t ny);
template <class C>
int32_t to29_device(g16_ctx* ctx, hipStream_t st, const void* d_points, size_t n, void* d_out);
template <class C>
int32_t precompute_device(g16_ctx* ctx, const void* d_points, size_t n, uint32_t c, uint32_t mtab, uint32_t stride,
                          void* d_tables);
template <class C>
int32_t fixed_base_device(g16_ctx* ctx, void* d_table, bool table_ready, const void* d_scalars, uint32_t mont, size_t n,
                          void* d_out);
template <class C>
int32_t on_curve_device(g16_ctx* ctx, const void* d_points, size_t n, uint32_t* d_first_bad);
template <class C>
int32_t live_bitmap_device(g16_ctx* ctx, const void* d_points, size_t n, uint32_t* d_bitmap, uint32_t* d_n_inf);
template <class C>
int32_t sum_partials_device(g16_ctx* ctx, const void* d_parts, uint32_t count, void* d_out_aff);

struct g16_spmat;
int32_t g16_spmat_create(g16_ctx* ctx, uint32_t nmat, uint32_t nrows, size_t nnz, const uint32_t* vrow,
                         size_t vrow_stride, const uint32_t* col, size_t col_stride, const void* val_base,
                         size_t val_stride, g16_spmat** out, bool values_r2 = false);
void g16_spmat_destroy(g16_spmat* m);
void g16_spmat_info(const g16_spmat* m, size_t out[10]);
int32_t g16_spmat_apply(g16_ctx* ctx, const g16_spmat* m, const void* d_x, uint32_t x_mont, void* d_out,
                        bool need_cz = true);
int32_t g16_ntt_device(g16_ctx* ctx, const void* d_src, void* d_dst, uint32_t log2n, int inverse);
int32_t g16_quotient_device(g16_ctx* ctx, const void* d_a, const void* d_b, const void* d_c, uint32_t log2n,
                            int flavour, void* d_out, int c_from_ab = 0);
int32_t g16_coset_pipeline_device(g16_ctx* ctx, const void* d_in, uint32_t log2n, void* d_out);
int32_t g16_abc_pointwise_device(g16_ctx* ctx, const void* d_a, const void* d_b, const void* d_c, size_t count,
                                 void* d_out);

int32_t g16_widen_multipliers(g16_ctx* ctx, const char* who, const void* multipliers, size_t n, std::vector<uint64_t>& out);
int32_t g16_key_audit_body(g16_ctx* ctx, const g16_pkey_desc* d, const g16_vkey_desc* vk, const void* section4,
                           size_t section4_bytes, const void* multipliers, g16_key_report* out);
struct g16_audit_section {
  int group;
  const void* p;
  size_t n;
};
int32_t g16_audit_sections(g16_ctx* ctx, const g16_audit_section* sec, int nsec, size_t (*first_bad)[3],
                           size_t (*bad_count)[3]);

int32_t g16_pairing_products4(g16_ctx* ctx, const void* d_P, const void* d_Q, uint32_t count, uint32_t neg_mask,
                              int32_t* d_result);

namespace g16 {
struct u256;
}
int32_t g16_setup_geometric(g16_ctx* ctx, bool lagrange, const g16::u256& w0, const g16::u256& s, const g16::u256& c,
                            const g16::u256& tau, size_t count, g16::u256* d_out, uint32_t* d_first_zero);
namespace g16 {
template <class C>
int32_t cs_term_device(g16_ctx* ctx, const void* d_pts, const uint32_t* d_src, const void* d_val, const uint32_t* d_ord,
                       uint32_t vstride, uint32_t mont, uint32_t log2rev, size_t count, void* d_out_acc);
template <class C>
int32_t cs_butterflies_device(g16_ctx* ctx, void* d_v, const void* d_tw, uint32_t log2n);
template <class C>
int32_t cs_segsum_device(g16_ctx* ctx, const void* d_terms, const uint32_t* d_off, const uint32_t* d_wires,
                         const CsSumPlan& plan, void* d_out_aff);
template <class C>
int32_t cs_to_affine_device(g16_ctx* ctx, const void* d_acc, size_t count, void* d_out_aff);
template <class C>
int32_t cs_diff_device(g16_ctx* ctx, const void* d_p, const void* d_q, size_t count, void* d_out_aff);
}

namespace g16 {
struct ScalePlan;
struct ScaleJob;
template <class C>
int32_t scale_uniform_device(g16_ctx* ctx, const void* d_pts, size_t n, const ScaleJob& job, void* d_out_aff);
}
int32_t g16_scale_job(g16_ctx* ctx, const g16::u256& k_std, g16::ScalePlan& plan, uint32_t* d_steps, g16::ScaleJob& job);

struct g16_combine_pre {
  unsigned char r_std[32], s_std[32];
  unsigned char a_pre[64], b_pre[128], c_pre[64];
};
int32_t g16_combine_enqueue(g16_ctx* ctx, const g16_pkey* k, const void* partials, size_t count, uint32_t flags,
                            const void* mask_r, const void* mask_s, void* res_host, hipEvent_t done,
                            g16_combine_pre* pre);
void g16_combine_finish(const g16_combine_pre* pre, const void* res_host, g16_proof* out);
```

### nim_groth16_amd/csrc/g16hip.hip

```cpp
#include "g16_internal.hpp"
#include "ec.cuh"

using namespace g16;

static G16Env read_env() {
  G16Env e;
  auto num = [](const char* name, int lo, int hi) {
    const char* v = getenv(name);
    if (!v) return 0;
    int x = atoi(v);
    return x >= lo && x <= hi ? x : 0;
  };
  e.msm_window = num("G16_MSM_WINDOW", 5, 22);
  e.table_window = num("G16_TABLE_WINDOW", 5, 22);
  e.msm_seg = num("G16_MSM_SEG", 8, 4096);
  e.red_slice_log2 = num("G16_RED_SLICE", 8, 11);
  e.cu_split = num("G16_CU_SPLIT", 1, 24);
  e.heavy_grid = num("G16_HEAVY_GRID", 1, 4096);
  if (const char* v = getenv("G16_INF_COMPACT")) e.inf_compact_pct = atoi(v) < 0 ? 0 : atoi(v) > 101 ? 101 : atoi(v);
  if (const char* v = getenv("G16_R2_WIDTH")) e.r2_width = v[0] == '0' ? 0 : v[0] == '2' ? 2 : 1;
  if (const char* v = getenv("G16_LANES_AFTER_QUOTIENT")) e.lanes_after_quotient = v[0] != '0';
  if (const char* v = getenv("G16_QUOTIENT_FIRST")) e.quotient_first = v[0] != '0';
  if (const char* v = getenv("G16_G1_BATCH")) e.g1_batch = v[0] != '0';
  if (const char* v = getenv("G16_CHAIN_CH")) e.chain_ch = v[0] != '0';
  if (const char* v = getenv("G16_ABC_DICT")) e.abc_dict = v[0] != '0';
  if (const char* v = getenv("G16_CZ_FLY")) e.cz_on_the_fly = v[0] != '0';
  if (const char* v = getenv("G16_RED_CHUNK")) e.red_chunk = atoi(v) == 2 || atoi(v) == 4 || atoi(v) == 8 || atoi(v) == 16 ? atoi(v) : 0;
  if (const char* v = getenv("G16_TAIL_QUAD")) e.tail_quad = v[0] != '0';
  if (const char* v = getenv("G16_G2_FIRST")) e.g2_first = v[0] == '2' ? 2 : v[0] != '0';
  if (const char* v = getenv("G16_B1_FOLD")) e.b1_fold = v[0] != '0';
  if (const char* v = getenv("G16_MTAB")) e.mtab = v[0] == '1' ? 1 : 2;
  if (const char* v = getenv("G16_NTT_TILE")) e.ntt_tile = atoi(v) == 1024 ? 1024 : atoi(v) == 4096 ? 4096 : 2048;
  if (const char* v = getenv("G16_MSM_SORT")) e.msm_sort = v[0];
  if (const char* v = getenv("G16_G1_LANES"))
    if (strlen(v) == 3 && strspn(v, "023") == 3)
      for (int i = 0; i < 3; ++i) e.g1_lanes[i] = v[i] - '0';
  if (const char* v = getenv("G16_STREAM_PRIO"))
    if (strlen(v) >= 6 && strspn(v, "hnl") >= 6) memcpy(e.stream_prio, v, 6);
  return e;
}
const G16Env& g16_env() {
  static const G16Env env = read_env();
  return env;
}

static hipError_t ctx_stream_create(Stream& out, int prio_index, bool front) {
  hipStream_t st = nullptr;
  hipError_t e;
  if (g16_env().cu_split <= 0) {
    int lo = 0, hi = 0;
    (void)hipDeviceGetStreamPriorityRange(&lo, &hi);
    e = hipStreamCreateWithPriority(&st, hipStreamNonBlocking, stream_priority(g16_env(), prio_index, lo, hi));
  } else {
    uint32_t mask[8];
    stream_cu_mask(g16_env(), front, mask);
    e = hipExtStreamCreateWithCUMask(&st, 8, mask);
  }
  out.reset(st);
  return e;
}

extern "C" int32_t g16_ctx_create(int32_t device, g16_ctx** out) {
  if (!out) return G16_EINVAL;
  *out = nullptr;
  (void)g16_env();
  int ndev = 0;
  if (hipGetDeviceCount(&ndev) != hipSuccess || ndev <= 0) return G16_ENODEV;
  if (device < 0 || device >= ndev) return G16_EINVAL;
  if (hipSetDevice(device) != hipSuccess) return G16_ENODEV;
  Building<g16_ctx, g16_ctx_destroy> ctx(new (std::nothrow) g16_ctx());
  if (!ctx) return G16_ENOMEM;
  ctx->device = device;
  if (ctx_stream_create(ctx->own_stream, 5, true) != hipSuccess) return G16_ENODEV;
  ctx->stream = ctx->own_stream.get();
  if (g16_lanes_init(ctx.get()) != G16_OK) return G16_ENODEV;
  *out = ctx.release();
  return G16_OK;
}

int32_t g16_lanes_init(g16_ctx* ctx) {
  for (int i = 0; i < 5; ++i) {
    auto& l = ctx->lane[i];
    HIPCHK(ctx, ctx_stream_create(l.stream, i, false));
    HIPCHK(ctx, event_create(l.done));
  }
  for (Event& e : ctx->ev) HIPCHK(ctx, event_create(e));
  return G16_OK;
}

extern "C" void g16_ctx_destroy(g16_ctx* ctx) {
  if (!ctx) return;
  (void)hipSetDevice(ctx->device);
  ctx_quiesce(ctx);
  delete ctx;
}

extern "C" const char* g16_last_error(const g16_ctx* ctx) { return ctx ? ctx->err.c_str() : "null context"; }

extern "C" int32_t g16_ctx_set_stream(g16_ctx* ctx, void* hip_stream) {
  if (!ctx) return G16_EINVAL;
  CTX_ENTER(ctx);
  HIPCHK(ctx, hipStreamSynchronize(ctx->stream));
  ctx->own_stream.reset();
  if (!hip_stream) HIPCHK(ctx, stream_create(ctx->own_stream));
  ctx->stream = hip_stream ? (hipStream_t)hip_stream : ctx->own_stream.get();
  return G16_OK;
}

extern "C" int32_t g16_ctx_cancel(g16_ctx* ctx) {
  if (!ctx) return G16_EINVAL;
  HIPCHK(ctx, hipSetDevice(ctx->device));
  ctx_quiesce(ctx);
  ctx->shard_begun = nullptr;
  return G16_OK;
}

extern "C" int32_t g16_ctx_synchronize(g16_ctx* ctx) {
  if (!ctx) return G16_EINVAL;
  CTX_ENTER_KEEP(ctx);
  HIPCHK(ctx, hipStreamSynchronize(ctx->stream));
  return G16_OK;
}

extern "C" int32_t g16_profile_enable(g16_ctx* ctx, int32_t on) {
  if (!ctx) return G16_EINVAL;
  CTX_ENTER_KEEP(ctx);
  if (on && !ctx->clk_buf) {
    HIPCHK(ctx, dev_alloc(ctx->clk_buf, 16));
    HIPCHK(ctx, hipMemset(ctx->clk_buf.get(), 0, 16));
  }
  ctx->profiling = on != 0;
  ctx->prof_accum_only = on == 2;
  return G16_OK;
}
extern "C" int32_t g16_profile_reset(g16_ctx* ctx) {
  if (!ctx) return G16_EINVAL;
  CTX_ENTER_KEEP(ctx);
  HIPCHK(ctx, hipStreamSynchronize(ctx->stream));
  for (auto& e : ctx->prof) {
    ctx->free_events.push_back(std::move(e.e0));
    ctx->free_events.push_back(std::move(e.e1));
  }
  ctx->prof.clear();
  return G16_OK;
}
extern "C" int32_t g16_profile_report(g16_ctx* ctx, char* buf, size_t buflen) {
  if (!ctx || !buf || buflen < 3) return G16_EINVAL;
  CTX_ENTER_KEEP(ctx);
  HIPCHK(ctx, hipStreamSynchronize(ctx->stream));
  std::map<std::string, std::pair<int, double>> agg;
  for (auto& e : ctx->prof) {
    float ms = 0;
    if (hipEventElapsedTime(&ms, e.e0.get(), e.e1.get()) == hipSuccess) {
      auto& a = agg[e.name];
      a.first++;
      a.second += ms;
    }
  }
  std::string s = "{";
  bool first = true;
  for (auto& kv : agg) {
    char tmp[256];
    snprintf(tmp, sizeof tmp, "%s\"%s\": {\"calls\": %d, \"total_ms\": %.6f}", first ? "" : ", ", kv.first.c_str(),
             kv.second.first, kv.second.second);
    s += tmp;
    first = false;
  }
  s += "}";
  if (s.size() + 1 > buflen) return G16_EINVAL;
  memcpy(buf, s.c_str(), s.size() + 1);
  return G16_OK;
}

extern "C" int32_t g16_profile_clock(g16_ctx* ctx, double* ghz) {
  if (!ctx || !ghz) return G16_EINVAL;
  CTX_ENTER_KEEP(ctx);
  *ghz = 0.0;
  if (!ctx->clk_buf) return G16_OK;
  ctx_quiesce(ctx);
  unsigned long long h[2] = {0, 0};
  HIPCHK(ctx, hipMemcpy(h, ctx->clk_buf.get(), 16, hipMemcpyDeviceToHost));
  HIPCHK(ctx, hipMemset(ctx->clk_buf.get(), 0, 16));
  if (h[1]) *ghz = (double)h[0] / (double)h[1] * 0.1;
  return G16_OK;
}

template <class C>
constexpr int group_of = sizeof(typename C::Aff) == sizeof(g1_aff) ? 1 : 2;

template <class C>
static int32_t msm_entry(g16_ctx* ctx, const void* scalars, uint32_t flags, const void* points, size_t n, void* out,
                         bool on_device, bool partial) {
  if (!ctx) return G16_EINVAL;
  if (!out || (n > 0 && (!scalars || !points))) {
    ctx->err = "null pointer argument";
    return G16_EINVAL;
  }
  if (n >= (size_t(1) << 27)) {
    ctx->err = "n too large (must be < 2^27)";
    return G16_EINVAL;
  }
  CTX_ENTER(ctx);
  const size_t out_bytes = partial ? sizeof(typename C::Acc) : sizeof(typename C::Aff);
  if (n == 0) {
    memset(out, 0, out_bytes);
    return G16_OK;
  }
  const void* d_s = scalars;
  const void* d_p = points;
  int32_t rc;
  if (!on_device) {
    if ((rc = ensure(ctx, ctx->stage_s, n * 32))) return rc;
    if ((rc = ensure(ctx, ctx->stage_p, n * sizeof(typename C::Aff)))) return rc;
    HIPCHK(ctx, hipMemcpyAsync(ctx->stage_s.p(), scalars, n * 32, hipMemcpyHostToDevice, ctx->stream));
    HIPCHK(ctx, hipMemcpyAsync(ctx->stage_p.p(), points, n * sizeof(typename C::Aff), hipMemcpyHostToDevice,
                               ctx->stream));
    d_s = ctx->stage_s.p();
    d_p = ctx->stage_p.p();
  }
  if ((rc = ensure_stage_o(ctx))) return rc;
  auto* d_aff = partial ? nullptr : (typename C::Aff*)ctx->stage_o.p();
  auto* d_acc = partial ? (typename C::Acc*)ctx->stage_o.p() : nullptr;
  if ((rc = msm_device<C>(ctx, d_s, flags, d_p, n, d_aff, d_acc, 0))) return rc;
  HIPCHK(ctx, hipMemcpyAsync(out, ctx->stage_o.p(), out_bytes, hipMemcpyDeviceToHost, ctx->stream));
  HIPCHK(ctx, hipStreamSynchronize(ctx->stream));
  return G16_OK;
}

template <class C>
static int32_t points_register(g16_ctx* ctx, const void* points, size_t n, bool on_device, uint32_t table_stride,
                               g16_points** out) {
  if (!ctx) return G16_EINVAL;
  if (!out || (n && !points) || n >= (size_t(1) << 26)) {
    ctx->err = "bad argument";
    return G16_EINVAL;
  }
  *out = nullptr;
  CTX_ENTER(ctx);
  Building<g16_points, g16_points_release> h(new (std::nothrow) g16_points());
  if (!h) return G16_ENOMEM;
  h->device = ctx->device;
  h->group = group_of<C>;
  h->n = n;
  const MsmTableChoice choice = msm_table_choice(n, table_stride, g16_env());
  h->c = choice.c;
  h->nwin = 254 / h->c + 1;
  h->mtab = choice.mtab;
  h->stride = choice.stride;
  constexpr size_t psz = sizeof(typename C::Aff);
  if (!choice.fits) {
    ctx->err = "point set too large for 31-bit table indices";
    return G16_EINVAL;
  }
  if (n) {
    if (h->mtab == 2 && dev_alloc(h->d_tables, (size_t)h->ntables() * n * psz) != hipSuccess) {
      (void)hipGetLastError();
      h->mtab = 1;
    }
    if (!h->d_tables) HIPCHK(ctx, dev_alloc(h->d_tables, (size_t)h->ntables() * n * psz));
    const void* d_src = points;
    int32_t rc;
    if (!on_device) {
      if ((rc = ensure(ctx, ctx->stage_p, n * psz))) return rc;
      HIPCHK(ctx, hipMemcpyAsync(ctx->stage_p.p(), points, n * psz, hipMemcpyHostToDevice, ctx->stream));
      d_src = ctx->stage_p.p();
    }
    if ((rc = precompute_device<C>(ctx, d_src, n, h->c, h->mtab, h->stride, h->d_tables.get()))) return rc;
    uint32_t n_inf = 0;
    HIPCHK(ctx, dev_alloc(h->d_live, ((n + 31) / 32 + 1) * 4));
    rc = counted_launch(ctx, 0, &n_inf, 1, [&](uint32_t* d_n_inf) {
      return live_bitmap_device<C>(ctx, d_src, n, h->d_live.get(), d_n_inf);
    });
    if (rc) return rc;
    h->n_inf = n_inf;
  }
  *out = h.release();
  return G16_OK;
}
extern "C" int32_t g16_points_register_g1(g16_ctx* ctx, const void* points, size_t n, g16_points** out) {
  return points_register<G1>(ctx, points, n, false, 0, out);
}
extern "C" int32_t g16_points_register_g2(g16_ctx* ctx, const void* points, size_t n, g16_points** out) {
  return points_register<G2>(ctx, points, n, false, 0, out);
}
extern "C" int32_t g16_points_register_g1_dev(g16_ctx* ctx, const void* d_points, size_t n, g16_points** out) {
  return points_register<G1>(ctx, d_points, n, true, 0, out);
}
extern "C" int32_t g16_points_register_g2_dev(g16_ctx* ctx, const void* d_points, size_t n, g16_points** out) {
  return points_register<G2>(ctx, d_points, n, true, 0, out);
}
extern "C" int32_t g16_points_register_g1_lean(g16_ctx* ctx, const void* points, size_t n, uint32_t table_stride,
                                               g16_points** out) {
  return points_register<G1>(ctx, points, n, false, table_stride, out);
}
extern "C" int32_t g16_points_register_g2_lean(g16_ctx* ctx, const void* points, size_t n, uint32_t table_stride,
                                               g16_points** out) {
  return points_register<G2>(ctx, points, n, false, table_stride, out);
}
extern "C" int32_t g16_points_register_g1_lean_dev(g16_ctx* ctx, const void* d_points, size_t n, uint32_t table_stride,
                                                   g16_points** out) {
  return points_register<G1>(ctx, d_points, n, true, table_stride, out);
}
extern "C" int32_t g16_points_register_g2_lean_dev(g16_ctx* ctx, const void* d_points, size_t n, uint32_t table_stride,
                                                   g16_points** out) {
  return points_register<G2>(ctx, d_points, n, true, table_stride, out);
}
extern "C" int32_t g16_points_plan(int group, size_t n, uint32_t table_stride, uint32_t* window_bits, uint32_t* ntables,
                                   size_t* bytes) {
  if ((group != 1 && group != 2) || n >= (size_t(1) << 26)) return G16_EINVAL;
  const MsmTableChoice choice = msm_table_choice(n, table_stride, g16_env());
  if (!choice.fits) return G16_EINVAL;
  if (window_bits) *window_bits = choice.c;
  if (ntables) *ntables = choice.ntables;
  if (bytes) *bytes = (size_t)choice.ntables * n * (group == 1 ? sizeof(g1_aff) : sizeof(g2_aff));
  return G16_OK;
}
extern "C" int32_t g16_points_table_bytes(const g16_points* h, size_t* bytes) {
  if (!h || !bytes) return G16_EINVAL;
  *bytes = (size_t)h->ntables() * h->n * (h->group == 1 ? sizeof(g1_aff) : sizeof(g2_aff));
  return G16_OK;
}
extern "C" void g16_points_release(g16_points* h) {
  if (!h) return;
  if (h->d_tables) {
    (void)hipSetDevice(h->device);
    (void)hipDeviceSynchronize();
  }
  delete h;
}
extern "C" size_t g16_points_inf_count(const g16_points* h) { return h ? h->n_inf : 0; }
const uint32_t* g16_points_live_if_sparse(const g16_points* p) {
  return p && p->d_live && p->n && points_sparse(p->n_inf, p->n, g16_env()) ? p->d_live.get() : nullptr;
}
// ... 250 lines not shown
```

### nim_groth16_amd/csrc/key_plan.hpp

```cpp
#pragma once
#include <stddef.h>
#include <stdint.h>

#include "g16_env.hpp"

namespace g16 {

struct KeyRange {
  size_t lo, hi;
  size_t size() const { return hi - lo; }
};
inline KeyRange shard_range(size_t N, uint32_t index, uint32_t count) {
  return KeyRange{(N * index) / count, (N * (index + 1)) / count};
}
inline size_t c1_padding(KeyRange w, uint32_t npubs) {
  const size_t pub_end = w.hi < (size_t)npubs + 1 ? w.hi : (size_t)npubs + 1;
  return pub_end > w.lo ? pub_end - w.lo : 0;
}

inline bool points_sparse(size_t n_inf, size_t n, const G16Env& env) {
  return n_inf && n_inf * 100 >= (size_t)env.inf_compact_pct * n;
}
enum B1Form : int { B1_PLAIN = 0, B1_EMPTY = 1, B1_DELTA = 2 };
inline B1Form b1_fold_form(size_t live_b1, size_t live_delta, size_t n, const G16Env& env) {
  if (!env.b1_fold) return B1_PLAIN;
  if (live_delta == 0) return B1_EMPTY;
  const long long keep = 100 - (long long)env.inf_compact_pct;
  if ((long long)live_delta * 100 > (long long)live_b1 * keep) return B1_PLAIN;
  const bool b1_compacted = n >= live_b1 && points_sparse(n - live_b1, n, env);
  if (b1_compacted && live_delta * 64 > live_b1) return B1_PLAIN;
  return B1_DELTA;
}
constexpr size_t B1_SPARSE_MAX = 64;
inline bool b1_sparse_run(size_t live_delta) { return live_delta != 0 && live_delta <= B1_SPARSE_MAX; }

enum LiveSource : int { LIVE_NONE = 0, LIVE_B2 = 1, LIVE_UNION = 2 };
inline LiveSource live_b_source(int b1_form, size_t nw, bool b1_bitmap, bool b2_bitmap) {
  if (!nw || !b2_bitmap) return LIVE_NONE;
  if (b1_form == B1_DELTA) return LIVE_B2;
  return b1_bitmap ? LIVE_UNION : LIVE_NONE;
}
inline bool live_b_kept(LiveSource source, size_t dead, size_t nw, const G16Env& env) {
  return source != LIVE_NONE && points_sparse(dead, nw, env);
}

}
```

### nim_groth16_amd/csrc/ntt.cuh

```cuda
#pragma once
#include "ff.cuh"

namespace g16 {

__device__ __forceinline__ u256 ntt_gen28() {
  u256 g;
  g.v[0] = 0x725b19f0u; g.v[1] = 0x9bd61b6eu; g.v[2] = 0x41112ed4u; g.v[3] = 0x402d111eu;
  g.v[4] = 0x8ef62abcu; g.v[5] = 0x00e0a7ebu; g.v[6] = 0xa58a7e85u; g.v[7] = 0x2a3c09f0u;
  return Fr::to_mont(g);
}
__device__ __forceinline__ u256 ntt_omega(uint32_t log2n) {
  u256 w = ntt_gen28();
  for (uint32_t i = log2n; i < 28; ++i) w = Fr::sqr(w);
  return w;
}
__device__ __forceinline__ u256 fr_pow_u32(u256 b, uint32_t e) {
  u256 r = Fr::one();
  while (e) {
    if (e & 1) r = Fr::mul(r, b);
    b = Fr::sqr(b);
    e >>= 1;
  }
  return r;
}

static __global__ void __launch_bounds__(256) ntt_make_twiddles(u256* __restrict__ tw, uint32_t log2n) {
  const uint32_t half = log2n ? (1u << (log2n - 1)) : 0u;
  uint32_t i = blockIdx.x * 256 + threadIdx.x;
  if (i < half) {
    tw[i] = fr_pow_u32(ntt_omega(log2n), i);
  } else if (i == half) {
    u256 h = Fr::one();
    for (uint32_t k = 0; k < log2n; ++k) h = Fr::div2(h);
    tw[half] = h;
  }
}

__device__ __forceinline__ u256 ntt_tw(const u256* __restrict__ tw, uint32_t e, uint32_t log2n, int inverse) {
  const uint32_t n = 1u << log2n, half = n >> 1;
  if (inverse && e) e = n - e;
  if (e < half) return tw[e];
  return Fr::neg(tw[e - half]);
}

constexpr int NTT_BLOCK = 1024;
constexpr int NTT_TILE = 4096;
constexpr uint32_t NTT_MAX_RHO = 10;
constexpr int NTT_BLOCK_SMALL = 256;
constexpr int NTT_TILE_SMALL = 1024;
constexpr uint32_t NTT_MAX_RHO_SMALL = 8;
constexpr int NTT_BLOCK_MID = 512;
constexpr int NTT_TILE_MID = 2048;

__device__ __forceinline__ uint32_t bitrev(uint32_t x, uint32_t bits) { return bits ? __brev(x) >> (32 - bits) : 0u; }

__device__ __forceinline__ uint32_t ntt_tile_of_block(uint32_t bid, uint32_t ntiles) {
  return (ntiles & 7u) ? bid : (bid & 7u) * (ntiles >> 3) + (bid >> 3);
}

template <int BLOCK>
__device__ __forceinline__ void ntt_tile_stages(u256* lds, const u256* twl, uint32_t rho, uint32_t log2b,
                                                uint32_t tile) {
  const uint32_t tid = threadIdx.x, B = 1u << log2b;
  uint32_t lh = rho;
  if (lh & 1u) {
    --lh;
    const uint32_t h = 1u << lh;
    for (uint32_t bf = tid; bf < (tile >> 1); bf += BLOCK) {
      uint32_t b = bf & (B - 1), pi = bf >> log2b;
      uint32_t p = pi & (h - 1);
      uint32_t i = ((pi >> lh) << (lh + 1)) | p;
      uint32_t ia = (i << log2b) | b, ib = ((i + h) << log2b) | b;
      u256 a = lds[ia], c = lds[ib];
      u256 sum = Fr::add(a, c), dif = Fr::sub(a, c);
      if (p) dif = Fr::mul(dif, twl[p << (rho - lh - 1)]);
      lds[ia] = sum;
      lds[ib] = dif;
    }
    __syncthreads();
  }
  while (lh >= 2) {
    lh -= 2;
    const uint32_t hh = 1u << lh, h = hh << 1;
    const uint32_t sA = rho - lh - 2;
    for (uint32_t g = tid; g < (tile >> 2); g += BLOCK) {
      const uint32_t b = g & (B - 1), pi = g >> log2b;
      const uint32_t p = pi & (hh - 1);
      const uint32_t i = ((pi >> lh) << (lh + 2)) | p;
      const uint32_t i0 = (i << log2b) | b, i1 = ((i + hh) << log2b) | b, i2 = ((i + h) << log2b) | b,
                     i3 = ((i + h + hh) << log2b) | b;
      const u256 x0 = lds[i0], x1 = lds[i1], x2 = lds[i2], x3 = lds[i3];
      u256 a0 = Fr::add(x0, x2), a2 = Fr::sub(x0, x2);
      u256 a1 = Fr::add(x1, x3), a3 = Fr::sub(x1, x3);
      if (p) a2 = Fr::mul(a2, twl[p << sA]);
      a3 = Fr::mul(a3, twl[(p + hh) << sA]);
      u256 b0 = Fr::add(a0, a1), b1 = Fr::sub(a0, a1);
      u256 b2 = Fr::add(a2, a3), b3 = Fr::sub(a2, a3);
      if (p) {
        const u256 tb = twl[p << (sA + 1)];
        b1 = Fr::mul(b1, tb);
        b3 = Fr::mul(b3, tb);
      }
      lds[i0] = b0;
      lds[i1] = b1;
      lds[i2] = b2;
      lds[i3] = b3;
    }
    __syncthreads();
  }
}

template <int BLOCK>
static __global__ void __launch_bounds__(BLOCK) ntt_pass(const u256* __restrict__ x, u256* __restrict__ y,
                                                      const u256* __restrict__ tw, uint32_t log2n, uint32_t log2s,
                                                      uint32_t rho, uint32_t log2b, int inverse, int last,
                                                      size_t xstride, size_t ystride,
                                                      const u256* __restrict__ scale, int mul_src) {
  extern __shared__ __align__(16) unsigned char smem[];
  u256* lds = reinterpret_cast<u256*>(smem);
  x += xstride * blockIdx.y;
  y += ystride * blockIdx.y;
  const uint32_t R = 1u << rho, B = 1u << log2b;
  const uint32_t nR = 1u << (log2n - rho);
  const uint32_t base0 = ntt_tile_of_block(blockIdx.x, gridDim.x) << log2b;
  const uint32_t tile = R << log2b;
  const uint32_t tid = threadIdx.x;

  u256* twl = lds + tile;
  for (uint32_t t = tid; t < (R >> 1); t += BLOCK) twl[t] = ntt_tw(tw, t << (log2n - rho), log2n, inverse);
  if (mul_src && blockIdx.y == 2) {
    const u256* xa = x - 2 * xstride;
    const u256* xb = x - xstride;
    for (uint32_t e = tid; e < tile; e += BLOCK) {
      uint32_t b = e & (B - 1), r = e >> log2b;
      const size_t gi = (size_t)base0 + b + (size_t)nR * r;
      lds[e] = Fr::mul(xa[gi], xb[gi]);
    }
  } else {
    for (uint32_t e = tid; e < tile; e += BLOCK) {
      uint32_t b = e & (B - 1), r = e >> log2b;
      lds[e] = x[(size_t)base0 + b + (size_t)nR * r];
    }
  }
  __syncthreads();

  ntt_tile_stages<BLOCK>(lds, twl, rho, log2b, tile);

  const uint32_t s_mask = (1u << log2s) - 1;
  for (uint32_t e = tid; e < tile; e += BLOCK) {
    uint32_t b = e & (B - 1), q = e >> log2b;
    uint32_t base = base0 + b;
    uint32_t k = base & s_mask, j = base >> log2s;
    u256 v = lds[(bitrev(q, rho) << log2b) | b];
    if (!last) {
      uint64_t ex = ((uint64_t)j * q) << log2s;
      uint32_t em = (uint32_t)(ex & ((1ull << log2n) - 1));
      if (em) v = Fr::mul(v, ntt_tw(tw, em, log2n, inverse));
    }
    const size_t oi = (size_t)k + ((size_t)(((size_t)j << rho) + q) << log2s);
    if (last) {
      if (scale) v = Fr::mul(v, scale[oi]);
      else if (inverse) v = Fr::mul(v, tw[(1u << log2n) >> 1]);
    }
    y[oi] = v;
  }
}

template <int BLOCK, int TILE>
static __global__ void __launch_bounds__(BLOCK) ntt_last_pass_abc(const u256* __restrict__ x, u256* __restrict__ out,
                                                               const u256* __restrict__ tw, uint32_t log2n,
                                                               uint32_t log2s, uint32_t rho, uint32_t log2b,
                                                               size_t xstride, int mul_invz) {
  extern __shared__ __align__(16) unsigned char smem[];
  u256* lds = reinterpret_cast<u256*>(smem);
  constexpr int PER = TILE / BLOCK;
  const uint32_t R = 1u << rho, B = 1u << log2b;
  const uint32_t nR = 1u << (log2n - rho);
  const uint32_t base0 = ntt_tile_of_block(blockIdx.x, gridDim.x) << log2b;
  const uint32_t tile = R << log2b;
  const uint32_t tid = threadIdx.x;
  u256* twl = lds + tile;
  for (uint32_t t = tid; t < (R >> 1); t += BLOCK) twl[t] = ntt_tw(tw, t << (log2n - rho), log2n, 0);
  u256 acc[PER];
#pragma unroll 1
  for (int v = 0; v < 3; ++v) {
    const u256* xv = x + xstride * v;
    for (uint32_t e = tid; e < tile; e += BLOCK) {
      uint32_t b = e & (B - 1), r = e >> log2b;
      lds[e] = xv[(size_t)base0 + b + (size_t)nR * r];
    }
    __syncthreads();
    ntt_tile_stages<BLOCK>(lds, twl, rho, log2b, tile);
#pragma unroll
    for (int i = 0; i < PER; ++i) {
      const uint32_t e = tid + i * BLOCK;
      if (e < tile) {
        uint32_t b = e & (B - 1), q = e >> log2b;
        u256 z = lds[(bitrev(q, rho) << log2b) | b];
        acc[i] = v == 0 ? z : v == 1 ? Fr::mul(acc[i], z) : Fr::sub(acc[i], z);
      }
    }
    __syncthreads();
  }
  const uint32_t s_mask = (1u << log2s) - 1;
#pragma unroll
  for (int i = 0; i < PER; ++i) {
    const uint32_t e = tid + i * BLOCK;
    if (e < tile) {
      uint32_t b = e & (B - 1), q = e >> log2b;
      uint32_t base = base0 + b;
      uint32_t k = base & s_mask, j = base >> log2s;
      const size_t oi = (size_t)k + ((size_t)(((size_t)j << rho) + q) << log2s);
      u256 r = acc[i];
      if (mul_invz) r = Fr::neg(Fr::div2(r));
      out[oi] = r;
    }
  }
}

static __global__ void __launch_bounds__(256) ntt_make_coset_table(u256* __restrict__ tab, uint32_t log2n, int mode) {
  uint32_t i = blockIdx.x * 256 + threadIdx.x;
  const uint32_t n = 1u << log2n;
  if (i >= n) return;
  u256 ninv = Fr::one();
  for (uint32_t k = 0; k < log2n; ++k) ninv = Fr::div2(ninv);
  u256 eta = ntt_omega(log2n + 1);
  uint32_t e = mode ? (2 * n - i) % (2 * n) : i;
  tab[i] = Fr::mul(fr_pow_u32(eta, e), ninv);
}

static __global__ void __launch_bounds__(256) fr_abc_pointwise(const u256* __restrict__ a, const u256* __restrict__ b,
                                                        const u256* __restrict__ c, u256* __restrict__ out,
                                                        uint32_t n) {
  uint32_t j = blockIdx.x * 256 + threadIdx.x;
  if (j >= n) return;
  out[j] = Fr::sub(Fr::mul(a[j], b[j]), c[j]);
}

}
```

### nim_groth16_amd/csrc/ntt.hip

```cpp
#include <atomic>
#include <mutex>

#include "g16_internal.hpp"
#include "ntt.cuh"
#include "ntt_plan.hpp"

using namespace g16;

static int32_t ensure_twiddles(g16_ctx* ctx, uint32_t log2n) {
  if (ctx->tw_log2n == log2n) return G16_OK;
  const size_t n = size_t(1) << log2n;
  int32_t rc;
  if ((rc = ensure(ctx, ctx->ntt_tw, (n / 2 + 1) * 32))) return rc;
  KLAUNCH(ctx, "ntt_twiddles", ntt_make_twiddles, (uint32_t)((n / 2 + 1 + 255) / 256), 256, 0, (u256*)ctx->ntt_tw.p(),
          log2n);
  ctx->tw_log2n = log2n;
  return G16_OK;
}

static_assert(ntt_geom(NTT_TILE_SMALL).max_rho == NTT_MAX_RHO_SMALL &&
                  (1 << ntt_geom(NTT_TILE_SMALL).log2tile) == NTT_TILE_SMALL,
              "ntt_plan.hpp and ntt.cuh disagree on the 1024 geometry");
static_assert(ntt_geom(NTT_TILE_MID).max_rho == NTT_MAX_RHO && (1 << ntt_geom(NTT_TILE_MID).log2tile) == NTT_TILE_MID,
              "ntt_plan.hpp and ntt.cuh disagree on the 2048 geometry");
static_assert(ntt_geom(NTT_TILE).max_rho == NTT_MAX_RHO && (1 << ntt_geom(NTT_TILE).log2tile) == NTT_TILE,
              "ntt_plan.hpp and ntt.cuh disagree on the 4096 geometry");
static_assert(ntt_optin_shmem() == ntt_pass_shmem(NTT_MAX_RHO, 2), "the opt-in covers the largest pass");
static int32_t ntt_kernels_init(g16_ctx* ctx) {
  static std::atomic<bool> done_on[64];
  static std::mutex mu;
  std::atomic<bool>& done = done_on[ctx->device & 63];
  if (done.load(std::memory_order_acquire)) return G16_OK;
  std::lock_guard<std::mutex> lock(mu);
  if (done.load(std::memory_order_relaxed)) return G16_OK;
  const int max_shmem = (int)ntt_optin_shmem();
  static_assert((size_t(32) * NTT_TILE) + (size_t(16) << NTT_MAX_RHO) <= 160 * 1024, "tile + twiddles must fit the LDS");
  HIPCHK(ctx, hipFuncSetAttribute(reinterpret_cast<const void*>(&ntt_pass<NTT_BLOCK>),
                                  hipFuncAttributeMaxDynamicSharedMemorySize, max_shmem));
  HIPCHK(ctx, hipFuncSetAttribute(reinterpret_cast<const void*>(&ntt_last_pass_abc<NTT_BLOCK, NTT_TILE>),
                                  hipFuncAttributeMaxDynamicSharedMemorySize, max_shmem));
  HIPCHK(ctx, hipFuncSetAttribute(reinterpret_cast<const void*>(&ntt_pass<NTT_BLOCK_MID>),
                                  hipFuncAttributeMaxDynamicSharedMemorySize, max_shmem));
  HIPCHK(ctx, hipFuncSetAttribute(reinterpret_cast<const void*>(&ntt_last_pass_abc<NTT_BLOCK_MID, NTT_TILE_MID>),
                                  hipFuncAttributeMaxDynamicSharedMemorySize, max_shmem));
  done.store(true, std::memory_order_release);
  return G16_OK;
}

struct NttKernels {
  uint32_t block;
  decltype(&ntt_last_pass_abc<NTT_BLOCK, NTT_TILE>) last_pass_abc;
  decltype(&ntt_pass<NTT_BLOCK>) pass;
};
static const NttKernels ntt_kernels[3] = {
    {NTT_BLOCK_SMALL, ntt_last_pass_abc<NTT_BLOCK_SMALL, NTT_TILE_SMALL>, ntt_pass<NTT_BLOCK_SMALL>},
    {NTT_BLOCK_MID, ntt_last_pass_abc<NTT_BLOCK_MID, NTT_TILE_MID>, ntt_pass<NTT_BLOCK_MID>},
    {NTT_BLOCK, ntt_last_pass_abc<NTT_BLOCK, NTT_TILE>, ntt_pass<NTT_BLOCK>},
};

static int32_t ntt_batched(g16_ctx* ctx, const u256* in, size_t in_stride, u256* out, size_t out_stride,
                           uint32_t batch, uint32_t log2n, int inverse, const u256* scale, int fuse_abc = 0,
                           int c_from_ab = 0) {
  const size_t n = size_t(1) << log2n;
  int32_t rc;
  if ((rc = ensure_twiddles(ctx, log2n))) return rc;
  if ((rc = ntt_kernels_init(ctx))) return rc;
  if (log2n == 0 && !fuse_abc) {
    for (uint32_t b = 0; b < batch; ++b)
      HIPCHK(ctx, hipMemcpyAsync(out + b * out_stride, in + b * in_stride, 32, hipMemcpyDeviceToDevice, ctx->stream));
    return G16_OK;
  }
  const int tile = g16_env().ntt_tile;
  const NttGeom geom = ntt_geom(tile);
  const NttKernels& K = ntt_kernels[tile == NTT_TILE_SMALL ? 0 : tile == NTT_TILE_MID ? 1 : 2];
  const uint32_t npass = ntt_npass(geom, log2n);
  u256 *tmpA = nullptr, *tmpB = nullptr;
  if (npass > 1) {
    if ((rc = ensure(ctx, ctx->ntt_tmp, (npass > 2 ? 2 : 1) * n * 32 * batch))) return rc;
    tmpA = (u256*)ctx->ntt_tmp.p();
    tmpB = tmpA + n * batch;
  }
  const u256* src = in;
  size_t src_stride = in_stride;
  for (uint32_t p = 0; p < npass; ++p) {
    const NttPass plan = ntt_pass_plan(geom, log2n, p);
    const bool last = p + 1 == npass;
    if (last && fuse_abc) {
      KLAUNCH(ctx, "ntt_last_pass_abc", K.last_pass_abc, plan.ntiles, K.block, plan.shmem, src, out,
              (const u256*)ctx->ntt_tw.p(), log2n, plan.log2s, plan.rho, plan.log2b, src_stride, fuse_abc == 2 ? 1 : 0);
      break;
    }
    u256* dst = last ? out : ((p & 1) ? tmpB : tmpA);
    const size_t dst_stride = last ? out_stride : n;
    KLAUNCH(ctx, inverse ? "ntt_pass_inv" : "ntt_pass_fwd", K.pass, dim3(plan.ntiles, batch), K.block, plan.shmem, src, dst,
            (const u256*)ctx->ntt_tw.p(), log2n, plan.log2s, plan.rho, plan.log2b, inverse, last ? 1 : 0, src_stride,
            dst_stride, last ? scale : (const u256*)nullptr, p == 0 ? c_from_ab : 0);
    src = dst;
    src_stride = dst_stride;
  }
  HIPCHK(ctx, hipGetLastError());
  return G16_OK;
}

int32_t g16_ntt_device(g16_ctx* ctx, const void* d_src, void* d_dst, uint32_t log2n, int inverse) {
  if (d_src == d_dst && ntt_one_pass(ntt_geom(g16_env().ntt_tile), log2n) && log2n > 0) {
    int32_t rc = ensure(ctx, ctx->ntt_tmp, (size_t(32) << log2n));
    if (rc) return rc;
    if ((rc = ntt_batched(ctx, (const u256*)d_src, 0, (u256*)ctx->ntt_tmp.p(), 0, 1, log2n, inverse, nullptr))) return rc;
    HIPCHK(ctx, hipMemcpyAsync(d_dst, ctx->ntt_tmp.p(), size_t(32) << log2n, hipMemcpyDeviceToDevice, ctx->stream));
    return G16_OK;
  }
  return ntt_batched(ctx, (const u256*)d_src, 0, (u256*)d_dst, 0, 1, log2n, inverse, nullptr);
}

static int32_t ensure_coset(g16_ctx* ctx, uint32_t log2n, int mode) {
  if (ctx->coset_log2n[mode] == log2n) return G16_OK;
  const size_t n = size_t(1) << log2n;
  int32_t rc;
  if ((rc = ensure(ctx, ctx->coset[mode], n * 32))) return rc;
  KLAUNCH(ctx, "ntt_coset_table", ntt_make_coset_table, (uint32_t)((n + 255) / 256), 256, 0,
          (u256*)ctx->coset[mode].p(), log2n, mode);
  ctx->coset_log2n[mode] = log2n;
  return G16_OK;
}

int32_t g16_quotient_device(g16_ctx* ctx, const void* d_a, const void* d_b, const void* d_c, uint32_t log2n,
                            int flavour, void* d_out, int c_from_ab) {
  if (log2n > 27) {
    ctx->err = "quotient needs the 2n domain: log2n <= 27";
    return G16_EINVAL;
  }
  const size_t n = size_t(1) << log2n;
  int32_t rc;
  if ((rc = ensure(ctx, ctx->quot, 4 * n * 32))) return rc;
  if ((rc = ensure_coset(ctx, log2n, 0))) return rc;
  u256* X = (u256*)ctx->quot.p();
  u256* Y = X + 3 * n;
  const u256* in = (const u256*)d_a;
  if (c_from_ab && ((const u256*)d_b != in + n || (const u256*)d_c != in + 2 * n || log2n == 0)) {
    ctx->err = "quotient: Cz can only be formed on the fly from contiguous Az | Bz | Cz";
    return G16_EINVAL;
  }
  if ((const u256*)d_b != in + n || (const u256*)d_c != in + 2 * n) {
    HIPCHK(ctx, hipMemcpyAsync(X, d_a, n * 32, hipMemcpyDeviceToDevice, ctx->stream));
    HIPCHK(ctx, hipMemcpyAsync(X + n, d_b, n * 32, hipMemcpyDeviceToDevice, ctx->stream));
    HIPCHK(ctx, hipMemcpyAsync(X + 2 * n, d_c, n * 32, hipMemcpyDeviceToDevice, ctx->stream));
    in = X;
    if (ntt_one_pass(ntt_geom(g16_env().ntt_tile), log2n)) {
      if ((rc = ensure(ctx, ctx->ntt_tmp, 3 * n * 32))) return rc;
      HIPCHK(ctx, hipMemcpyAsync(ctx->ntt_tmp.p(), X, 3 * n * 32, hipMemcpyDeviceToDevice, ctx->stream));
      in = (const u256*)ctx->ntt_tmp.p();
    }
  }
  if ((rc = ntt_batched(ctx, in, n, X, n, 3, log2n, 1, (const u256*)ctx->coset[0].p(), 0, c_from_ab))) return rc;
  if (flavour == 1) {
    if ((rc = ntt_batched(ctx, X, n, (u256*)d_out, 0, 3, log2n, 0, nullptr, 1))) return rc;
  } else {
    if ((rc = ensure_coset(ctx, log2n, 1))) return rc;
    if ((rc = ntt_batched(ctx, X, n, Y, 0, 3, log2n, 0, nullptr, 2))) return rc;
    if ((rc = ntt_batched(ctx, Y, n, (u256*)d_out, n, 1, log2n, 1, (const u256*)ctx->coset[1].p()))) return rc;
  }
  HIPCHK(ctx, hipGetLastError());
  return G16_OK;
}

int32_t g16_coset_pipeline_device(g16_ctx* ctx, const void* d_in, uint32_t log2n, void* d_out) {
  if (log2n > 27) {
    ctx->err = "quotient needs the 2n domain: log2n <= 27";
    return G16_EINVAL;
  }
  const size_t n = size_t(1) << log2n;
  int32_t rc;
  if ((rc = ensure(ctx, ctx->quot, 4 * n * 32))) return rc;
  if ((rc = ensure_coset(ctx, log2n, 0))) return rc;
  u256* X = (u256*)ctx->quot.p();
  if ((rc = ntt_batched(ctx, (const u256*)d_in, n, X, n, 1, log2n, 1, (const u256*)ctx->coset[0].p()))) return rc;
  return ntt_batched(ctx, X, n, (u256*)d_out, n, 1, log2n, 0, nullptr);
}

int32_t g16_abc_pointwise_device(g16_ctx* ctx, const void* d_a, const void* d_b, const void* d_c, size_t count,
                                 void* d_out) {
  if (count)
    KLAUNCH(ctx, "fr_abc_pointwise", fr_abc_pointwise, (uint32_t)((count + 255) / 256), 256, 0, (const u256*)d_a,
            (const u256*)d_b, (const u256*)d_c, (u256*)d_out, (uint32_t)count);
  HIPCHK(ctx, hipGetLastError());
  return G16_OK;
}
```

### nim_groth16_amd/csrc/pkey.hip

```cpp
#include <algorithm>
#include <cstddef>
#include <new>

#include "pkey.hpp"
#include "b1_fold.cuh"

using namespace g16;

extern "C" void g16_pkey_destroy(g16_pkey* k) {
  if (!k) return;
  for (g16_points* p : {k->A1, k->B1, k->B2, k->C1, k->H1}) g16_points_release(p);
  (void)hipSetDevice(k->device);
  (void)hipDeviceSynchronize();
  g16_spmat_destroy(k->abc);
  delete k;
}

extern "C" int32_t g16_pkey_inf_counts(const g16_pkey* k, size_t out[8]) {
  if (!k || !out) return G16_EINVAL;
  out[0] = k->A1->n_inf, out[1] = k->b1_inf, out[2] = k->B2->n_inf, out[4] = k->H1->n_inf;
  out[3] = k->C1->n_inf - c1_padding(k->w, k->npubs);
  out[5] = k->deadB, out[6] = k->liveA ? 1 : 0, out[7] = k->liveB ? 1 : 0;
  return G16_OK;
}

extern "C" int32_t g16_pkey_b1_fold(const g16_pkey* k, size_t out[3]) {
  if (!k || !out) return G16_EINVAL;
  out[0] = (size_t)k->b1_form, out[1] = k->live_b1, out[2] = k->live_delta;
  return G16_OK;
}

extern "C" int32_t g16_pkey_b1_sparse(const g16_pkey* k, size_t out[3]) {
  if (!k || !out) return G16_EINVAL;
  out[0] = k->b1_sparse ? 1 : 0, out[1] = k->b1_nlive, out[2] = B1_SPARSE_MAX;
  return G16_OK;
}

extern "C" int32_t g16_pkey_abc_info(const g16_pkey* k, size_t out[11]) {
  if (!k || !out) return G16_EINVAL;
  out[0] = k->ncoeffs;
  g16_spmat_info(k->abc, out + 1);
  return G16_OK;
}

struct CoeffSource {
  const unsigned char* base = nullptr;
  size_t count = 0, stride = 0, value_off = 0;
  bool values_r2 = false;
};
static inline uint32_t rd32(const unsigned char* p) {
  uint32_t v;
  memcpy(&v, p, 4);
  return v;
}

static __global__ void __launch_bounds__(256) b1_compare_kernel(const uint4* __restrict__ a1, const uint4* __restrict__ b1,
                                                                uint32_t n, uint32_t* __restrict__ cnt) {
  const uint32_t i = blockIdx.x * 256 + threadIdx.x;
  bool live = false, differs = false;
  if (i < n) {
    uint32_t any = 0, diff = 0;
#pragma unroll
    for (int q = 0; q < 4; ++q) {
      const uint4 a = a1[(size_t)i * 4 + q], b = b1[(size_t)i * 4 + q];
      any |= b.x | b.y | b.z | b.w;
      diff |= (a.x ^ b.x) | (a.y ^ b.y) | (a.z ^ b.z) | (a.w ^ b.w);
    }
    live = any != 0, differs = diff != 0;
  }
  const uint32_t nl = (uint32_t)__popcll(__ballot(live)), nd = (uint32_t)__popcll(__ballot(differs));
  if ((threadIdx.x & 63) == 0) {
    if (nl) atomicAdd(&cnt[0], nl);
    if (nd) atomicAdd(&cnt[1], nd);
  }
}
static __global__ void __launch_bounds__(256) b1_delta_kernel(const g1_aff* __restrict__ a1, g1_aff* __restrict__ b1,
                                                              uint32_t n) {
  const uint32_t i = blockIdx.x * 256 + threadIdx.x;
  if (i >= n) return;
  b1[i] = point_difference<G1>(b1[i], a1[i]);
}

static bool desc_well_formed(const g16_pkey_desc* d) {
  return d->log2_domain <= 27 && d->nvars != 0 && d->npubs + 1 <= d->nvars && d->flavour <= 1 && d->pointsA1 &&
         d->pointsB1 && d->pointsB2 && d->pointsH1 && (d->nvars - d->npubs - 1 == 0 || d->pointsC1) && d->alpha1 &&
         d->beta1 && d->delta1 && d->beta2 && d->delta2;
}

static int32_t key_layout(g16_ctx* ctx, const g16_pkey_desc* d, g16_pkey* k) {
  k->device = ctx->device;
  k->nvars = d->nvars;
  k->npubs = d->npubs;
  k->log2n = d->log2_domain;
  k->flavour = d->flavour;
  memcpy(&k->alpha1, d->alpha1, 64);
  memcpy(&k->beta1, d->beta1, 64);
  memcpy(&k->delta1, d->delta1, 64);
  memcpy(&k->beta2, d->beta2, 128);
  memcpy(&k->delta2, d->delta2, 128);
  k->shard_count = d->shard_count ? d->shard_count : 1;
  k->shard_index = d->shard_index;
  if (k->shard_index >= k->shard_count) {
    ctx->err = "shard_index >= shard_count";
    return G16_EINVAL;
  }
  k->w = shard_range(d->nvars, k->shard_index, k->shard_count);
  k->h = shard_range(size_t(1) << d->log2_domain, k->shard_index, k->shard_count);
  return G16_OK;
}

static int32_t b1_form_of_whole_arrays(g16_ctx* ctx, const g16_pkey_desc* d, g16_pkey* k) {
  const size_t nv = d->nvars;
  uint32_t cnt[2] = {0, 0};
  if (g16_env().b1_fold) {
    constexpr size_t CHUNK = size_t(1) << 16;
    const size_t step = std::min(nv, CHUNK);
    DevMem<g1_aff> c_a1, c_b1;
    SyncOnExit sync{ctx->stream};
    HIPCHK(ctx, dev_alloc(c_a1, step * sizeof(g1_aff)));
    HIPCHK(ctx, dev_alloc(c_b1, step * sizeof(g1_aff)));
    const int32_t rc = counted_launch(ctx, 0, cnt, 2, [&](uint32_t* d_cnt) -> int32_t {
      for (size_t lo = 0; lo < nv; lo += step) {
        const size_t m = std::min(step, nv - lo);
        HIPCHK(ctx, hipMemcpyAsync(c_a1.get(), (const char*)d->pointsA1 + 64 * lo, m * 64, hipMemcpyHostToDevice, ctx->stream));
        HIPCHK(ctx, hipMemcpyAsync(c_b1.get(), (const char*)d->pointsB1 + 64 * lo, m * 64, hipMemcpyHostToDevice, ctx->stream));
        hipLaunchKernelGGL(b1_compare_kernel, dim3((uint32_t)((m + 255) / 256)), dim3(256), 0, ctx->stream,
                           (const uint4*)c_a1.get(), (const uint4*)c_b1.get(), (uint32_t)m, d_cnt);
        HIPCHK(ctx, hipGetLastError());
      }
      return G16_OK;
    });
    if (rc) return rc;
  }
  k->live_b1 = cnt[0], k->live_delta = cnt[1];
  k->b1_form = b1_fold_form(cnt[0], cnt[1], nv, g16_env());
  return G16_OK;
}

static int32_t b1_live_wires(g16_ctx* ctx, g16_pkey* k) {
  if (!b1_sparse_run(k->live_delta)) return G16_OK;
  const size_t nw = k->w.size(), words = (nw + 31) / 32;
  std::vector<uint32_t> bitmap(words), list(g16_pkey::B1_VIEW_WORDS, 0u);
  HIPCHK(ctx, hipMemcpyAsync(bitmap.data(), k->B1->d_live.get(), words * 4, hipMemcpyDeviceToHost, ctx->stream));
  HIPCHK(ctx, hipStreamSynchronize(ctx->stream));
  for (size_t i = 0; i < nw; ++i)
    if ((bitmap[i >> 5] >> (i & 31)) & 1u) list.push_back((uint32_t)i);
  const size_t nlive = list.size() - g16_pkey::B1_VIEW_WORDS;
  if (nlive > B1_SPARSE_MAX || nlive != nw - k->B1->n_inf) {
    ctx->err = "the live differences of pointsB1 do not match their count";
    return G16_EINVAL;
  }
  list.push_back(0u);
  HIPCHK(ctx, dev_alloc(k->b1_sparse, list.size() * 4));
  HIPCHK(ctx, hipMemcpyAsync(k->b1_sparse.get(), list.data(), list.size() * 4, hipMemcpyHostToDevice, ctx->stream));
  HIPCHK(ctx, hipStreamSynchronize(ctx->stream));
  k->b1_nlive = (uint32_t)nlive;
  return G16_OK;
}

static int32_t register_b1(g16_ctx* ctx, const g16_pkey_desc* d, uint32_t table_stride, g16_pkey* k) {
  const size_t nw = k->w.size();
  int32_t rc;
  if (k->b1_form != B1_DELTA || !nw) {
    if ((rc = g16_points_register_g1_lean(ctx, (const char*)d->pointsB1 + 64 * k->w.lo, nw, table_stride, &k->B1))) return rc;
    k->b1_inf = k->B1->n_inf;
    return G16_OK;
  }
  DevMem<g1_aff> d_a1, d_b1;
  DevMem<uint32_t> scratch_live;
  SyncOnExit sync{ctx->stream};
  HIPCHK(ctx, dev_alloc(d_a1, nw * sizeof(g1_aff)));
  HIPCHK(ctx, dev_alloc(d_b1, nw * sizeof(g1_aff)));
  HIPCHK(ctx, hipMemcpyAsync(d_a1.get(), (const char*)d->pointsA1 + 64 * k->w.lo, nw * 64, hipMemcpyHostToDevice, ctx->stream));
  HIPCHK(ctx, hipMemcpyAsync(d_b1.get(), (const char*)d->pointsB1 + 64 * k->w.lo, nw * 64, hipMemcpyHostToDevice, ctx->stream));
  HIPCHK(ctx, dev_alloc(scratch_live, ((nw + 31) / 32 + 1) * 4));
  uint32_t n_inf = 0;
  rc = counted_launch(ctx, 0, &n_inf, 1, [&](uint32_t* d_n_inf) -> int32_t {
    if (int32_t e = live_bitmap_device<G1>(ctx, d_b1.get(), nw, scratch_live.get(), d_n_inf)) return e;
    hipLaunchKernelGGL(b1_delta_kernel, dim3((uint32_t)((nw + 255) / 256)), dim3(256), 0, ctx->stream,
                       (const g1_aff*)d_a1.get(), d_b1.get(), (uint32_t)nw);
    HIPCHK(ctx, hipGetLastError());
    return G16_OK;
  });
  if (rc) return rc;
  k->b1_inf = n_inf;
  if ((rc = g16_points_register_g1_lean_dev(ctx, d_b1.get(), nw, table_stride, &k->B1))) return rc;
  return b1_live_wires(ctx, k);
}

static std::vector<unsigned char> c1_wire_aligned(const g16_pkey_desc* d, const g16_pkey* k) {
  std::vector<unsigned char> c1pad(k->w.size() * 64, 0);
  for (size_t wI = k->w.lo + c1_padding(k->w, d->npubs); wI < k->w.hi; ++wI)
    memcpy(&c1pad[(wI - k->w.lo) * 64], (const char*)d->pointsC1 + 64 * (wI - d->npubs - 1), 64);
  return c1pad;
}

static int32_t live_lists(g16_ctx* ctx, g16_pkey* k) {
  const size_t nw = k->w.size(), bitmap_bytes = ((nw + 31) / 32 + 1) * 4;
  k->liveA = g16_points_live_if_sparse(k->A1);
  const LiveSource source = live_b_source(k->b1_form, nw, (bool)k->B1->d_live, (bool)k->B2->d_live);
  if (source == LIVE_B2) {
    k->deadB = k->B2->n_inf;
    if (live_b_kept(source, k->deadB, nw, g16_env())) {
      HIPCHK(ctx, dev_alloc(k->liveB, bitmap_bytes));
      HIPCHK(ctx, hipMemcpyAsync(k->liveB.get(), k->B2->d_live.get(), bitmap_bytes, hipMemcpyDeviceToDevice, ctx->stream));
      HIPCHK(ctx, hipStreamSynchronize(ctx->stream));
    }
  } else if (source == LIVE_UNION) {
    uint32_t dead = 0;
    HIPCHK(ctx, dev_alloc(k->liveB, bitmap_bytes));
    const int32_t rc = counted_launch(ctx, 0, &dead, 1, [&](uint32_t* d_dead) {
      return g16_bitmap_or_device(ctx, k->liveB.get(), k->B1->d_live.get(), k->B2->d_live.get(), nw, d_dead);
    });
    if (rc) return rc;
    k->deadB = dead;
    if (!live_b_kept(source, dead, nw, g16_env())) k->liveB.reset();
  }
  return G16_OK;
}

static int32_t bin_coefficients(g16_ctx* ctx, const g16_pkey_desc* d, const CoeffSource& cs, g16_pkey* k) {
  const size_t n = size_t(1) << d->log2_domain;
  std::vector<uint32_t> vrow;
  try {
    vrow.resize(cs.count ? cs.count : 1);
  } catch (const std::bad_alloc&) {
    ctx->err = "out of host memory";
    return G16_ENOMEM;
  }
  for (size_t e = 0; e < cs.count; ++e) {
    const unsigned char* ent = cs.base + e * cs.stride;
    const uint32_t matrix = rd32(ent), row = rd32(ent + 4), col = rd32(ent + 8);
    if (matrix > 1 || row >= n || col >= d->nvars) {
      ctx->err = "coefficient entry out of range (matrix must be 0=A or 1=B)";
      return G16_EINVAL;
    }
    vrow[e] = 2 * row + matrix;
  }
  k->ncoeffs = cs.count;
  return g16_spmat_create(ctx, 2, (uint32_t)n, cs.count, vrow.data(), 4, (const uint32_t*)(cs.count ? cs.base + 8 : nullptr),
                          cs.stride, cs.count ? cs.base + cs.value_off : nullptr, cs.stride, &k->abc, cs.values_r2);
}

static int32_t pkey_create(g16_ctx* ctx, const g16_pkey_desc* d, const CoeffSource& cs, uint32_t table_stride,
                           g16_pkey** out) {
  if (!desc_well_formed(d)) {
    ctx->err = "bad proving-key description";
    return G16_EINVAL;
  }
  CTX_ENTER(ctx);
  Building<g16_pkey, g16_pkey_destroy> k(new (std::nothrow) g16_pkey());
  if (!k) return G16_ENOMEM;
  const uint32_t ts = table_stride;
  int32_t rc;
  if ((rc = key_layout(ctx, d, k.get()))) return rc;
  const std::vector<unsigned char> c1pad = c1_wire_aligned(d, k.get());
  if ((rc = g16_points_register_g1_lean(ctx, (const char*)d->pointsA1 + 64 * k->w.lo, k->w.size(), ts, &k->A1))) return rc;
  if ((rc = b1_form_of_whole_arrays(ctx, d, k.get()))) return rc;
  if ((rc = register_b1(ctx, d, ts, k.get()))) return rc;
  if ((rc = g16_points_register_g2_lean(ctx, (const char*)d->pointsB2 + 128 * k->w.lo, k->w.size(), ts, &k->B2))) return rc;
  if ((rc = g16_points_register_g1_lean(ctx, c1pad.data(), k->w.size(), ts, &k->C1))) return rc;
  if ((rc = g16_points_register_g1_lean(ctx, (const char*)d->pointsH1 + 64 * k->h.lo, k->h.size(), ts, &k->H1))) return rc;
  if ((rc = live_lists(ctx, k.get()))) return rc;
  if ((rc = bin_coefficients(ctx, d, cs, k.get()))) return rc;
  *out = k.release();
  return G16_OK;
}

extern "C" int32_t g16_pkey_create_lean(g16_ctx* ctx, const g16_pkey_desc* d, uint32_t table_stride, g16_pkey** out) {
  if (!ctx) return G16_EINVAL;
  if (!d || !out || (d->ncoeffs && !d->coeffs)) {
    ctx->err = "null argument";
    return G16_EINVAL;
  }
  *out = nullptr;
  static_assert(sizeof(g16_coeff) == 48 && offsetof(g16_coeff, value) == 16, "g16_coeff layout");
  CoeffSource cs;
  cs.base = (const unsigned char*)d->coeffs, cs.count = d->ncoeffs, cs.stride = sizeof(g16_coeff), cs.value_off = 16;
  return pkey_create(ctx, d, cs, table_stride, out);
}
extern "C" int32_t g16_pkey_create(g16_ctx* ctx, const g16_pkey_desc* d, g16_pkey** out) {
  return g16_pkey_create_lean(ctx, d, 0, out);
}

extern "C" int32_t g16_pkey_create_zkey_lean(g16_ctx* ctx, const g16_pkey_desc* d, const void* section4,
                                             size_t section4_bytes, uint32_t table_stride, g16_pkey** out) {
  if (!ctx) return G16_EINVAL;
  if (!d || !out || !section4 || section4_bytes < 4 || d->coeffs || d->ncoeffs) {
    ctx->err = "bad argument (section 4 of the .zkey in, desc.coeffs = NULL, desc.ncoeffs = 0)";
    return G16_EINVAL;
  }
  *out = nullptr;
  const unsigned char* p = (const unsigned char*)section4;
  const size_t count = rd32(p);
  if (section4_bytes != 4 + count * 44) {
    ctx->err = "unexpected length of the coefficient section (4 + 44 * count bytes)";
    return G16_EINVAL;
  }
  CoeffSource cs;
  cs.base = p + 4, cs.count = count, cs.stride = 44, cs.value_off = 12, cs.values_r2 = true;
  return pkey_create(ctx, d, cs, table_stride, out);
}
extern "C" int32_t g16_pkey_create_zkey(g16_ctx* ctx, const g16_pkey_desc* d, const void* section4, size_t section4_bytes,
                                        g16_pkey** out) {
  return g16_pkey_create_zkey_lean(ctx, d, section4, section4_bytes, 0, out);
}
```

### nim_groth16_amd/csrc/pkey.hpp

```cpp
#pragma once
#include "g16_internal.hpp"
#include "ec.cuh"

struct g16_pkey {
  int device = 0;
  uint32_t nvars = 0, npubs = 0, log2n = 0, flavour = 1;
  uint32_t shard_index = 0, shard_count = 1;
  g16::KeyRange w{0, 0};
  g16::KeyRange h{0, 0};
  g16_points *A1 = nullptr, *B1 = nullptr, *B2 = nullptr, *C1 = nullptr, *H1 = nullptr;
  g16_spmat* abc = nullptr;
  size_t ncoeffs = 0;
  g16::g1_aff alpha1, beta1, delta1;
  g16::g2_aff beta2, delta2;
  const uint32_t* liveA = nullptr;
  DevMem<uint32_t> liveB;
  size_t deadB = 0;
  int b1_form = g16::B1_PLAIN;
  size_t b1_inf = 0;
  size_t live_b1 = 0, live_delta = 0;
  static constexpr size_t B1_VIEW_WORDS = 16;
  DevMem<uint32_t> b1_sparse;
  uint32_t b1_nlive = 0;
};
```

### nim_groth16_amd/csrc/proof_plan.hpp

```cpp
#pragma once
#include <stddef.h>
#include <stdint.h>

#include "g16_env.hpp"
#include "key_plan.hpp"

namespace g16 {

inline void stream_cu_mask(const G16Env& env, bool front, uint32_t mask[8]) {
  for (int w = 0; w < 8; ++w) mask[w] = 0;
  for (int bit = 0; bit < 256; ++bit)
    if ((bit / 8 < env.cu_split) == front) mask[bit / 32] |= 1u << (bit % 32);
}
inline int stream_priority(const G16Env& env, int index, int lo, int hi) {
  switch (env.stream_prio[index]) {
    case 'h': return hi;
    case 'l': return lo;
    default: return (lo + hi) / 2;
  }
}

constexpr int8_t PS_MAIN = 5;
enum ProofEvent : int8_t { EV_NONE = -1, EV_A, EV_B, EV_Q, EV_B2, EV_C, EV_G2, EV_COUNT, EV_DONE0 = EV_COUNT };
enum ProofRun : int8_t { RUN_A1, RUN_B1, RUN_C1, RUN_B2, RUN_H, RUN_COUNT };
enum ProofSort : int8_t { SORT_W = 0, SORT_H = 1, SORT_WA = 2, SORT_WB = 3 };

enum ProofOp : uint8_t {
  OP_UPLOAD,
  OP_WAIT,
  OP_RECORD,
  OP_SORT_W,
  OP_SORT_H,
  OP_BUILD_ABC,
  OP_QUOTIENT,
  OP_COSET,
  OP_POINTWISE,
  OP_MSM,
  OP_COPY_OUT,
  OP_HOST_SYNC,
};
struct ProofStep {
  uint8_t op;
  int8_t stream;
  int8_t a, b, c, d, e;
};

enum ProofEntry : int { PROOF_WHOLE, PROOF_BEGIN, PROOF_END };
struct ProofShape {
  size_t nw, nh;
  uint32_t log2n;
  bool liveA, liveB;
  bool cfg_equal;
  int b1_form = B1_PLAIN;
};

constexpr size_t G2_FIRST_MAX = size_t(1) << 18;

constexpr int PROOF_PLAN_CAP = 48;
struct ProofPlan {
  int count = 0, cap = PROOF_PLAN_CAP;
  bool overflow = false;
  bool narrow_tail = true;
  int8_t sort_a = SORT_W, sort_b = SORT_W;
  int8_t sort_b1 = SORT_W;
  ProofStep steps[PROOF_PLAN_CAP];

  void push(ProofOp op, int stream, int a = 0, int b = 0, int c = 0, int d = 0, int e = 0) {
    if (count >= cap || count >= PROOF_PLAN_CAP) {
      overflow = true;
      return;
    }
    steps[count++] = ProofStep{(uint8_t)op, (int8_t)stream, (int8_t)a, (int8_t)b, (int8_t)c, (int8_t)d, (int8_t)e};
  }
  void record(int stream, int ev) { push(OP_RECORD, stream, ev); }
  void wait(int stream, int ev) {
    for (int i = count - 1; i >= 0; --i) {
      const ProofStep& s = steps[i];
      if ((s.op == OP_RECORD && s.a == ev) || (s.op == OP_MSM && s.d == ev)) break;
      if (s.op == OP_WAIT && s.stream == stream && s.a == ev) return;
    }
    push(OP_WAIT, stream, ev);
  }
  void msm(int stream, int first, int n_accum, int n_tail, int after_heavy = EV_NONE, bool continues_c1 = false) {
    push(OP_MSM, stream, first, n_accum, n_tail, after_heavy, continues_c1);
  }
};

inline bool proof_chains_c_into_h(const G16Env& env, const ProofShape& s) {
  return env.chain_ch && s.nw && s.nh && s.cfg_equal;
}
inline int proof_witness_lanes(const G16Env& env) { return env.g1_batch ? 2 : 4; }

inline void proof_plan_witness(ProofPlan& p, const G16Env& env, const ProofShape& s, int after) {
  if (!s.nw) return;
  p.wait(0, EV_A);
  p.push(OP_SORT_W, 0, SORT_W, 0, RUN_A1);
  if (s.liveA) p.push(OP_SORT_W, 0, SORT_WA, 1, RUN_A1);
  p.record(0, EV_B);
  if (s.liveB) {
    p.wait(1, EV_A);
    p.push(OP_SORT_W, 1, SORT_WB, 2, RUN_B2);
    p.record(1, EV_B2);
  }
  const bool batch = env.g1_batch != 0;
  const bool chain = proof_chains_c_into_h(env, s);
  const int nlanes = proof_witness_lanes(env);
  const int la = batch ? 0 : env.g1_lanes[0], lb = batch ? 0 : env.g1_lanes[1], lc = batch ? 0 : env.g1_lanes[2];
  for (int i = 1; i < nlanes; ++i) p.wait(i, i == 1 && s.liveB ? EV_B2 : EV_B);
  if (s.liveB) p.wait(lb, EV_B2);
  if (after != EV_NONE)
    for (int i = 0; i < nlanes; ++i) p.wait(i, after);
  const bool g2_first = env.g2_first >= 0 ? env.g2_first != 0 : s.nw <= G2_FIRST_MAX;
  p.msm(1, RUN_B2, 1, 1, g2_first ? EV_G2 : EV_NONE);
  if (g2_first) {
    p.wait(la, EV_G2);
    p.wait(lb, EV_G2);
    if (!chain || env.g2_first == 2) p.wait(lc, EV_G2);
  }
  const int after_c = chain ? EV_C : EV_NONE;
  if (batch) {
    p.msm(0, RUN_A1, 3, chain ? 2 : 3, after_c);
  } else {
    p.msm(la, RUN_A1, 1, 1);
    p.msm(lb, RUN_B1, 1, 1);
    p.msm(lc, RUN_C1, 1, chain ? 0 : 1, after_c);
  }
  for (int i = 0; i < nlanes; ++i) p.record(i, EV_DONE0 + i);
}

inline void proof_plan_h_and_collect(ProofPlan& p, const G16Env& env, const ProofShape& s, bool sorted, bool host_sync) {
  if (s.nh) {
    if (!sorted) p.push(OP_SORT_H, PS_MAIN);
    const int hs = env.cu_split ? 4 : PS_MAIN;
    if (hs != PS_MAIN) {
      p.record(PS_MAIN, EV_Q);
      p.wait(hs, EV_Q);
    }
    const bool chain = proof_chains_c_into_h(env, s);
    if (chain) p.wait(hs, EV_C);
    p.msm(hs, RUN_H, 1, 1, EV_NONE, chain);
    if (hs != PS_MAIN) {
      p.record(hs, EV_DONE0 + 4);
      p.wait(PS_MAIN, EV_DONE0 + 4);
    }
  }
  if (s.nw)
    for (int i = 0; i < proof_witness_lanes(env); ++i) p.wait(PS_MAIN, EV_DONE0 + i);
  p.push(OP_COPY_OUT, PS_MAIN);
  if (host_sync) p.push(OP_HOST_SYNC, PS_MAIN);
}

inline bool proof_plan_build(ProofPlan& p, const G16Env& env, ProofEntry entry, uint32_t task_mask, bool host_sync,
                             const ProofShape& s, int cap = PROOF_PLAN_CAP) {
  p = ProofPlan();
  p.cap = cap;
  p.sort_a = s.liveA ? SORT_WA : SORT_W;
  p.sort_b = s.liveB ? SORT_WB : SORT_W;
  p.sort_b1 = s.b1_form == B1_PLAIN ? p.sort_b : SORT_W;
  if (entry == PROOF_END) {
    p.push(OP_POINTWISE, PS_MAIN);
    proof_plan_h_and_collect(p, env, s, false, host_sync);
    return !p.overflow;
  }
  p.push(OP_UPLOAD, PS_MAIN);
  p.record(PS_MAIN, EV_A);
  if (entry == PROOF_BEGIN) {
    if (task_mask) p.push(OP_BUILD_ABC, PS_MAIN, (task_mask & 4u) != 0);
    for (int v = 0; v < 3; ++v)
      if (task_mask & (1u << v)) p.push(OP_COSET, PS_MAIN, v);
    int after = EV_NONE;
    if (task_mask && env.quotient_first && env.lanes_after_quotient) p.record(PS_MAIN, after = EV_Q);
    proof_plan_witness(p, env, s, after);
    if (host_sync) p.push(OP_HOST_SYNC, PS_MAIN);
    return !p.overflow;
  }
  const int fly = s.log2n >= 1 && env.cz_on_the_fly ? 1 : 0;
  if (!env.quotient_first) proof_plan_witness(p, env, s, EV_NONE);
  p.push(OP_BUILD_ABC, PS_MAIN, fly == 0);
  p.push(OP_QUOTIENT, PS_MAIN, fly);
  if (env.quotient_first) {
    if (s.nh) p.push(OP_SORT_H, PS_MAIN);
    int after = EV_NONE;
    if (env.lanes_after_quotient) p.record(PS_MAIN, after = EV_Q);
    proof_plan_witness(p, env, s, after);
  }
  proof_plan_h_and_collect(p, env, s, env.quotient_first != 0, host_sync);
  return !p.overflow;
}

}
```

### nim_groth16_amd/csrc/prover.hip

```cpp
#include "pkey.hpp"
#include "host_curve.hpp"

using namespace g16;

static int32_t build_abc_device(g16_ctx* ctx, const g16_pkey* k, const u256* d_wit, uint32_t wit_mont, u256* d_abc,
                                bool need_cz = true) {
  return g16_spmat_apply(ctx, k->abc, d_wit, wit_mont, d_abc, need_cz);
}

extern "C" int32_t g16_build_abc(g16_ctx* ctx, const g16_pkey* k, const void* witness, uint32_t flags, void* out_abc) {
  if (!ctx) return G16_EINVAL;
  if (!k || !witness || !out_abc || k->device != ctx->device) {
    ctx->err = "bad argument";
    return G16_EINVAL;
  }
  CTX_ENTER(ctx);
  const size_t n = size_t(1) << k->log2n;
  int32_t rc;
  if ((rc = ensure(ctx, ctx->prove, ((size_t)k->nvars + 4 * n) * 32))) return rc;
  u256* d_w = (u256*)ctx->prove.p();
  u256* d_abc = d_w + k->nvars;
  HIPCHK(ctx, hipMemcpyAsync(d_w, witness, (size_t)k->nvars * 32, hipMemcpyHostToDevice, ctx->stream));
  if ((rc = build_abc_device(ctx, k, d_w, (flags & G16_SCALARS_MONT) ? 1u : 0u, d_abc))) return rc;
  HIPCHK(ctx, hipMemcpyAsync(out_abc, d_abc, 3 * n * 32, hipMemcpyDeviceToHost, ctx->stream));
  HIPCHK(ctx, hipStreamSynchronize(ctx->stream));
  return G16_OK;
}

static constexpr size_t PART_A = 0, PART_B1 = 128, PART_B2 = 256, PART_H = 512, PART_C = 640, PART_BYTES = G16_PARTIALS_BYTES;
static_assert(PART_C + sizeof(g1_acc) == PART_BYTES && PART_BYTES <= STAGE_O_RESULT_BYTES, "record layout");

static ProofShape proof_shape(const g16_pkey* k) {
  return ProofShape{k->w.size(), k->h.size(), k->log2n, k->liveA != nullptr, (bool)k->liveB,
                    k->C1->cfg() == k->H1->cfg(), k->b1_form};
}

struct ProofArgs {
  const void* witness = nullptr;
  uint32_t flags = 0;
  u256* task_out = nullptr;
  const void *d_a1 = nullptr, *d_b1 = nullptr, *d_c1 = nullptr;
  bool qs_is_slice = false;
  void* out_partials = nullptr;
};

static int32_t run_plan(g16_ctx* ctx, const g16_pkey* k, ProofEntry entry, uint32_t task_mask, bool host_sync,
                        const ProofArgs& a) {
  ProofPlan plan;
  if (!proof_plan_build(plan, g16_env(), entry, task_mask, host_sync, proof_shape(k))) {
    ctx->err = "proof launch plan exceeds its capacity";
    return G16_EINVAL;
  }
  const size_t n = size_t(1) << k->log2n, nw = k->w.size(), nh = k->h.size();
  int32_t rc;
  if ((rc = ensure(ctx, ctx->prove, ((size_t)k->nvars + 4 * n) * 32))) return rc;
  if ((rc = ensure_stage_o(ctx))) return rc;
  u256* const d_w = (u256*)ctx->prove.p();
  u256* const d_abc = d_w + k->nvars;
  u256* const d_qs = d_abc + 3 * n;
  char* const slots = stage_o_at(ctx, STAGE_O_RESULT);
  const u256* const d_wr = d_w + k->w.lo;
  const u256* const d_qs_slice = a.qs_is_slice ? d_qs : d_qs + k->h.lo;
  const uint32_t wit_mont = (a.flags & G16_SCALARS_MONT) ? 1u : 0u;
  g16_ctx::MsmLane* L = ctx->lane;
  const g16_points* const sets[RUN_COUNT] = {k->A1, k->B1, k->C1, k->B2, k->H1};
  g16_msm_run runs[RUN_COUNT] = {
      {&ctx->sort[plan.sort_a], &L[0].acc, k->A1->d_tables.get(), nullptr, slots + PART_A, nullptr},
      {&ctx->sort[plan.sort_b1], &L[2].acc, k->b1_form == B1_EMPTY ? nullptr : k->B1->d_tables.get(), nullptr,
       slots + PART_B1, nullptr},
      {&ctx->sort[SORT_W], &L[3].acc, k->C1->d_tables.get(), nullptr, slots + PART_C, nullptr},
      {&ctx->sort[plan.sort_b], &L[1].acc, k->B2->d_tables.get(), nullptr, slots + PART_B2, nullptr},
      {&ctx->sort[SORT_H], &L[4].acc, k->H1->d_tables.get(), nullptr, slots + PART_H, nullptr}};
  g16_msm_sparse b1_sparse{d_wr, nullptr, k->b1_nlive, k->b1_sparse.get()};
  if (k->b1_sparse) {
    b1_sparse.d_wires = k->b1_sparse.get() + g16_pkey::B1_VIEW_WORDS;
    runs[RUN_B1].sparse = &b1_sparse;
  }
  auto event = [&](int e) { return e == EV_NONE ? nullptr : e < EV_COUNT ? ctx->ev[e].get() : L[e - EV_DONE0].done.get(); };
  for (int i = 0; i < plan.count; ++i) {
    const ProofStep& s = plan.steps[i];
    rc = G16_OK;
    hipStream_t st = s.stream == PS_MAIN ? ctx->stream : L[s.stream].stream.get();
    switch (s.op) {
      case OP_UPLOAD:
        HIPCHK(ctx, hipMemcpyAsync(d_w, a.witness, (size_t)k->nvars * 32,
                                   (a.flags & G16_SCALARS_DEVICE) ? hipMemcpyDeviceToDevice : hipMemcpyHostToDevice, st));
        HIPCHK(ctx, hipMemsetAsync(slots, 0, PART_BYTES, st));
        break;
      case OP_WAIT: HIPCHK(ctx, hipStreamWaitEvent(st, event(s.a), 0)); break;
      case OP_RECORD: HIPCHK(ctx, hipEventRecord(event(s.a), st)); break;
      case OP_SORT_W:
        ctx->sort[s.a].narrow_tail = plan.narrow_tail;
        rc = g16_msm_sort(ctx, st, d_wr, wit_mont ? G16_SCALARS_MONT : 0u, nw, sets[s.c]->cfg(), ctx->sort[s.a],
                          s.b == 0 ? nullptr : s.b == 1 ? k->liveA : k->liveB.get());
        break;
      case OP_SORT_H:
        ctx->sort[SORT_H].narrow_tail = plan.narrow_tail;
        rc = g16_msm_sort(ctx, st, d_qs_slice, G16_SCALARS_MONT, nh, k->H1->cfg(), ctx->sort[SORT_H]);
        break;
      case OP_BUILD_ABC: rc = build_abc_device(ctx, k, d_w, wit_mont, d_abc, s.a != 0); break;
      case OP_QUOTIENT:
        rc = g16_quotient_device(ctx, d_abc, d_abc + n, d_abc + 2 * n, k->log2n, (int)k->flavour, d_qs, s.a);
        break;
      case OP_COSET: {
        const int at = __builtin_popcount(task_mask & ((1u << s.a) - 1));
        rc = g16_coset_pipeline_device(ctx, d_abc + s.a * n, k->log2n, a.task_out + at * n);
        break;
      }
      case OP_POINTWISE: rc = g16_abc_pointwise_device(ctx, a.d_a1, a.d_b1, a.d_c1, nh, d_qs); break;
      case OP_MSM:
        runs[RUN_H].init_partial = s.e ? g16_msm_partial_ptr(L[3].acc) : nullptr;
        rc = g16_msm_batch(ctx, st, s.a == RUN_B2 ? 2 : 1, &runs[s.a], s.b, s.c, event(s.d));
        break;
      case OP_COPY_OUT:
        HIPCHK(ctx, hipMemcpyAsync(a.out_partials, slots, PART_BYTES,
                                   (a.flags & G16_OUT_DEVICE) ? hipMemcpyDeviceToDevice : hipMemcpyDeviceToHost, st));
        break;
      case OP_HOST_SYNC: HIPCHK(ctx, hipStreamSynchronize(st)); break;
    }
    if (rc) return rc;
  }
  return G16_OK;
}

extern "C" int32_t g16_prove_partials(g16_ctx* ctx, const g16_pkey* k, const void* witness, uint32_t flags,
                                      void* out_partials) {
  if (!ctx) return G16_EINVAL;
  if (!k || !witness || !out_partials || k->device != ctx->device) {
    ctx->err = "bad argument";
    return G16_EINVAL;
  }
  CTX_ENTER(ctx);
  ProofArgs a;
  a.witness = witness, a.flags = flags, a.out_partials = out_partials;
  const bool host_sync = !((flags & G16_NO_HOST_SYNC) && (flags & G16_OUT_DEVICE));
  const int32_t rc = run_plan(ctx, k, PROOF_WHOLE, 0, host_sync, a);
  if (rc != G16_OK) ctx_quiesce(ctx);
  return rc;
}

extern "C" int32_t g16_prove_partials_begin(g16_ctx* ctx, const g16_pkey* k, const void* witness, uint32_t flags,
                                            uint32_t task_mask, void* d_task_out) {
  if (!ctx) return G16_EINVAL;
  if (!k || !witness || k->device != ctx->device || task_mask > 7 || (task_mask && !d_task_out)) {
    ctx->err = "bad argument";
    return G16_EINVAL;
  }
  if (k->flavour != G16_FLAVOUR_SNARKJS) {
    ctx->err = "the task-parallel quotient serves snarkjs-flavour keys (JensGroth needs a 7th transform of the whole "
               "vector: use g16_prove_partials)";
    return G16_EINVAL;
  }
  CTX_ENTER(ctx);
  ProofArgs a;
  a.witness = witness, a.flags = flags, a.task_out = (u256*)d_task_out;
  const int32_t rc = run_plan(ctx, k, PROOF_BEGIN, task_mask, !(flags & G16_NO_HOST_SYNC), a);
  if (rc != G16_OK) {
    ctx_quiesce(ctx);
    return rc;
  }
  ctx->shard_begun = k;
  return G16_OK;
}

extern "C" int32_t g16_prove_partials_end(g16_ctx* ctx, const g16_pkey* k, const void* d_a1, const void* d_b1,
                                          const void* d_c1, uint32_t flags, void* out_partials) {
  if (!ctx) return G16_EINVAL;
  const size_t nh = k ? k->h.size() : 0;
  if (!k || !out_partials || k->device != ctx->device || (nh && (!d_a1 || !d_b1 || !d_c1))) {
    ctx->err = "bad argument";
    return G16_EINVAL;
  }
  if (ctx->shard_begun != k) {
    ctx->err = "g16_prove_partials_end without a matching g16_prove_partials_begin on this context";
    return G16_EINVAL;
  }
  CTX_ENTER_KEEP(ctx);
  ctx->shard_begun = nullptr;
  ProofArgs a;
  a.flags = flags, a.d_a1 = d_a1, a.d_b1 = d_b1, a.d_c1 = d_c1, a.qs_is_slice = true, a.out_partials = out_partials;
  const int32_t rc = run_plan(ctx, k, PROOF_END, 0, !((flags & G16_NO_HOST_SYNC) && (flags & G16_OUT_DEVICE)), a);
  if (rc != G16_OK) ctx_quiesce(ctx);
  return rc;
}

static __global__ void prove_combine_kernel(const unsigned char* __restrict__ gathered, uint32_t count, uint32_t fold_b1,
                                            unsigned char* __restrict__ out) {
  if (threadIdx.x != 0) return;
  const uint32_t b = blockIdx.x;
  if (b == 2) {
    g2_acc r = G2::acc_inf();
    for (uint32_t i = 0; i < count; ++i) G2::add(r, *(const g2_acc*)(gathered + (size_t)i * PART_BYTES + PART_B2));
    *(g2_aff*)(out + 128) = G2::to_affine(r);
  } else {
    const size_t src = b == 0 ? PART_A : b == 1 ? PART_B1 : b == 3 ? PART_H : PART_C;
    const size_t dst = b == 0 ? 0 : b == 1 ? 64 : b == 3 ? 256 : 320;
    g1_acc r = G1::acc_inf();
    for (uint32_t i = 0; i < count; ++i) G1::add(r, *(const g1_acc*)(gathered + (size_t)i * PART_BYTES + src));
    if (b == 1 && fold_b1)
      for (uint32_t i = 0; i < count; ++i) G1::add(r, *(const g1_acc*)(gathered + (size_t)i * PART_BYTES + PART_A));
    *(g1_aff*)(out + dst) = G1::to_affine(r);
  }
}

static_assert(sizeof(CombineRes) == G16_COMBINE_RES_BYTES, "slot layout");
static_assert(sizeof(CombinePre) == sizeof(g16_combine_pre), "g16_combine_pre layout");

int32_t g16_combine_enqueue(g16_ctx* ctx, const g16_pkey* k, const void* partials, size_t count, uint32_t flags,
                            const void* mask_r, const void* mask_s, void* res_host, hipEvent_t done,
                            g16_combine_pre* pre_out) {
  int32_t rc;
  if ((rc = ensure(ctx, ctx->stage_p, count * PART_BYTES))) return rc;
  if ((rc = ensure_stage_o(ctx))) return rc;
  HIPCHK(ctx, hipMemcpyAsync(ctx->stage_p.p(), partials, count * PART_BYTES,
                             (flags & G16_SCALARS_DEVICE) ? hipMemcpyDeviceToDevice : hipMemcpyHostToDevice,
                             ctx->stream));
  unsigned char* d_res = (unsigned char*)stage_o_at(ctx, STAGE_O_COMBINE);
  KLAUNCH(ctx, "prove_combine", prove_combine_kernel, 5, 64, 0, (const unsigned char*)ctx->stage_p.p(), (uint32_t)count,
          k->b1_form != B1_PLAIN ? 1u : 0u, d_res);

  u256 r = Fr::zero(), s = Fr::zero();
  if (mask_r) memcpy(&r, mask_r, 32);
  if (mask_s) memcpy(&s, mask_s, 32);
  const CombinePre pre = host_combine_pre(k->alpha1, k->beta1, k->delta1, k->beta2, k->delta2, r, s);
  memcpy(pre_out, &pre, sizeof pre);
  HIPCHK(ctx, hipMemcpyAsync(res_host, d_res, sizeof(CombineRes), hipMemcpyDeviceToHost, ctx->stream));
  if (done) HIPCHK(ctx, hipEventRecord(done, ctx->stream));
  return G16_OK;
}

void g16_combine_finish(const g16_combine_pre* pre_in, const void* res_host, g16_proof* out) {
  CombinePre pre;
  CombineRes res;
  memcpy(&pre, pre_in, sizeof pre);
  memcpy(&res, res_host, sizeof res);
  g1_aff pi_a, pi_c;
  g2_aff pi_b;
  host_combine_finish(pre, res, pi_a, pi_b, pi_c);
  memcpy(out->pi_a, &pi_a, 64);
  memcpy(out->pi_b, &pi_b, 128);
  memcpy(out->pi_c, &pi_c, 64);
}

extern "C" int32_t g16_prove_combine(g16_ctx* ctx, const g16_pkey* k, const void* partials, size_t count,
                                     uint32_t flags, const void* mask_r, const void* mask_s, g16_proof* out) {
  if (!ctx) return G16_EINVAL;
  if (!k || !partials || !out || k->device != ctx->device || count == 0 || count > 1024) {
    ctx->err = "bad argument";
    return G16_EINVAL;
  }
  CTX_ENTER(ctx);
  int32_t rc;
  CombineRes res;
  g16_combine_pre pre;
  if ((rc = g16_combine_enqueue(ctx, k, partials, count, flags, mask_r, mask_s, &res, nullptr, &pre))) return rc;
  HIPCHK(ctx, hipStreamSynchronize(ctx->stream));
  g16_combine_finish(&pre, &res, out);
  return G16_OK;
}

extern "C" int32_t g16_prove(g16_ctx* ctx, const g16_pkey* k, const void* witness, uint32_t flags, const void* mask_r,
                             const void* mask_s, g16_proof* out) {
  if (!ctx) return G16_EINVAL;
  if (!k || !witness || !out || k->device != ctx->device) {
    ctx->err = "bad argument";
    return G16_EINVAL;
  }
  if (k->shard_count != 1) {
    ctx->err = "g16_prove needs an unsharded key; use g16_prove_partials + g16_prove_combine";
    return G16_EINVAL;
  }
  CTX_ENTER(ctx);
  int32_t rc;
  if ((rc = ensure_stage_o(ctx))) return rc;
  if ((rc = ensure(ctx, ctx->stage_s, PART_BYTES))) return rc;
  unsigned char* d_part = (unsigned char*)ctx->stage_s.p();
  if ((rc = g16_prove_partials(ctx, k, witness, flags | G16_OUT_DEVICE | G16_NO_HOST_SYNC, d_part))) return rc;
  rc = g16_prove_combine(ctx, k, d_part, 1, G16_SCALARS_DEVICE, mask_r, mask_s, out);
  if (rc != G16_OK) ctx_quiesce(ctx);
  return rc;
}

extern "C" int32_t g16_quotient(g16_ctx* ctx, const void* Az, const void* Bz, const void* Cz, uint32_t log2n,
                                uint32_t flavour, void* out) {
  if (!ctx) return G16_EINVAL;
  if (!Az || !Bz || !Cz || !out || log2n > 27 || flavour > 1) {
    ctx->err = "bad argument";
    return G16_EINVAL;
  }
  CTX_ENTER(ctx);
  const size_t n = size_t(1) << log2n;
  int32_t rc;
  if ((rc = ensure(ctx, ctx->prove, 4 * n * 32))) return rc;
  u256* d = (u256*)ctx->prove.p();
  HIPCHK(ctx, hipMemcpyAsync(d, Az, n * 32, hipMemcpyHostToDevice, ctx->stream));
  HIPCHK(ctx, hipMemcpyAsync(d + n, Bz, n * 32, hipMemcpyHostToDevice, ctx->stream));
  HIPCHK(ctx, hipMemcpyAsync(d + 2 * n, Cz, n * 32, hipMemcpyHostToDevice, ctx->stream));
  if ((rc = g16_quotient_device(ctx, d, d + n, d + 2 * n, log2n, (int)flavour, d + 3 * n))) return rc;
  HIPCHK(ctx, hipMemcpyAsync(out, d + 3 * n, n * 32, hipMemcpyDeviceToHost, ctx->stream));
  HIPCHK(ctx, hipStreamSynchronize(ctx->stream));
  return G16_OK;
}
extern "C" int32_t g16_quotient_dev(g16_ctx* ctx, const void* d_Az, const void* d_Bz, const void* d_Cz, uint32_t log2n,
                                    uint32_t flavour, void* d_out) {
  if (!ctx) return G16_EINVAL;
  if (!d_Az || !d_Bz || !d_Cz || !d_out || log2n > 27 || flavour > 1) {
    ctx->err = "bad argument";
    return G16_EINVAL;
  }
  CTX_ENTER(ctx);
  return g16_quotient_device(ctx, d_Az, d_Bz, d_Cz, log2n, (int)flavour, d_out);
}
```

Measured before the change: 133.1 proofs/s.

## Exploit A/B row symmetry to skip the A-polynomial NTT in the quotient

At key creation the code checks which constraint rows have identical A and B coefficient lists and records up to four rows that differ. It also precomputes a correction table on the coset domain. When the symmetry holds, the quotient transforms only B and C (batch 2 instead of 3) and rebuilds A's coset evaluations from B's plus a rank-k correction inside the fused last NTT pass. This removes one inverse and one forward NTT per proof. In exchange the key needs an extra n-element device table, and the last pass does more per-element multiplications for each asymmetric row.

```diff
diff --git a/include/g16hip.h b/include/g16hip.h
--- a/include/g16hip.h
+++ b/include/g16hip.h
@@ -153,6 +153,7 @@
 int32_t g16_pkey_inf_counts(const g16_pkey* key, size_t out[8]);
 int32_t g16_pkey_b1_fold(const g16_pkey* key, size_t out[3]);
 int32_t g16_pkey_b1_sparse(const g16_pkey* key, size_t out[3]);
+int32_t g16_pkey_quot_sym(const g16_pkey* key, size_t out[3]);
 int32_t g16_prove(g16_ctx* ctx, const g16_pkey* key, const void* witness, uint32_t flags, const void* mask_r,
                   const void* mask_s, g16_proof* out);
 #define G16_PARTIALS_BYTES 768
diff --git a/nim_groth16_amd/_lib.py b/nim_groth16_amd/_lib.py
--- a/nim_groth16_amd/_lib.py
+++ b/nim_groth16_amd/_lib.py
@@ -31,7 +31,7 @@
     "g16_pkey_create_zkey_lean", "g16_group_pkey_create_lean",
     "g16_setup_log2_domain", "g16_fake_setup", "g16_lagrange_fr", "g16_powers_fr",
     "g16_points_audit_g1", "g16_points_audit_g2", "g16_points_pairs_check", "g16_key_audit",
-    "g16_pkey_b1_fold", "g16_pkey_b1_sparse", "g16_circuit_audit",
+    "g16_pkey_b1_fold", "g16_pkey_b1_sparse", "g16_pkey_quot_sym", "g16_circuit_audit",
     "g16_points_intt_g1", "g16_points_intt_g2", "g16_circuit_setup",
     "g16_points_scale_g1", "g16_points_scale_g2", "g16_key_contribute", "g16_contributions_verify",
 ]
@@ -358,6 +358,7 @@
     lib.g16_pkey_inf_counts.argtypes = [vp, ctypes.POINTER(sz)]
     lib.g16_pkey_b1_fold.argtypes = [vp, ctypes.POINTER(sz)]
     lib.g16_pkey_b1_sparse.argtypes = [vp, ctypes.POINTER(sz)]
+    lib.g16_pkey_quot_sym.argtypes = [vp, ctypes.POINTER(sz)]
     lib.g16_points_info.argtypes = [vp, ctypes.POINTER(u32), ctypes.POINTER(u32)]
     lib.g16_msm_points.argtypes = [vp, vp, vp, u32, vp]
     lib.g16_points_check_g1.argtypes = [vp, vp, sz, ctypes.POINTER(sz)]
@@ -894,6 +895,11 @@
         self.ctx._check(self.ctx._lib.g16_pkey_b1_sparse(self._h, out))
         return {"sparse": bool(out[0]), "live": out[1], "max": out[2]}
 
+    def quot_sym(self) -> dict:
+        out = (ctypes.c_size_t * 3)()
+        self.ctx._check(self.ctx._lib.g16_pkey_quot_sym(self._h, out))
+        return {"active": bool(out[0]), "rows": out[1], "max": out[2]}
+
     def abc_info(self) -> dict:
         out = (ctypes.c_size_t * 11)()
         self.ctx._check(self.ctx._lib.g16_pkey_abc_info(self._h, out))
diff --git a/nim_groth16_amd/csrc/g16_env.hpp b/nim_groth16_amd/csrc/g16_env.hpp
--- a/nim_groth16_amd/csrc/g16_env.hpp
+++ b/nim_groth16_amd/csrc/g16_env.hpp
@@ -24,4 +24,5 @@
   int abc_dict = 1;
   int g2_first = -1;
   int b1_fold = 1;
+  int quot_sym = 1;
 };
diff --git a/nim_groth16_amd/csrc/g16_internal.hpp b/nim_groth16_amd/csrc/g16_internal.hpp
--- a/nim_groth16_amd/csrc/g16_internal.hpp
+++ b/nim_groth16_amd/csrc/g16_internal.hpp
@@ -269,8 +269,13 @@
 int32_t g16_spmat_apply(g16_ctx* ctx, const g16_spmat* m, const void* d_x, uint32_t x_mont, void* d_out,
                         bool need_cz = true);
 int32_t g16_ntt_device(g16_ctx* ctx, const void* d_src, void* d_dst, uint32_t log2n, int inverse);
+struct g16_quot_sym {
+  const void* d_t0;
+  uint32_t k;
+  uint32_t rows[g16::QUOT_SYM_MAX];
+};
 int32_t g16_quotient_device(g16_ctx* ctx, const void* d_a, const void* d_b, const void* d_c, uint32_t log2n,
-                            int flavour, void* d_out, int c_from_ab = 0);
+                            int flavour, void* d_out, int c_from_ab = 0, const g16_quot_sym* sym = nullptr);
 int32_t g16_coset_pipeline_device(g16_ctx* ctx, const void* d_in, uint32_t log2n, void* d_out);
 int32_t g16_abc_pointwise_device(g16_ctx* ctx, const void* d_a, const void* d_b, const void* d_c, size_t count,
                                  void* d_out);
diff --git a/nim_groth16_amd/csrc/g16hip.hip b/nim_groth16_amd/csrc/g16hip.hip
--- a/nim_groth16_amd/csrc/g16hip.hip
+++ b/nim_groth16_amd/csrc/g16hip.hip
@@ -29,6 +29,7 @@
   if (const char* v = getenv("G16_TAIL_QUAD")) e.tail_quad = v[0] != '0';
   if (const char* v = getenv("G16_G2_FIRST")) e.g2_first = v[0] == '2' ? 2 : v[0] != '0';
   if (const char* v = getenv("G16_B1_FOLD")) e.b1_fold = v[0] != '0';
+  if (const char* v = getenv("G16_QUOT_SYM")) e.quot_sym = v[0] != '0';
   if (const char* v = getenv("G16_MTAB")) e.mtab = v[0] == '1' ? 1 : 2;
   if (const char* v = getenv("G16_NTT_TILE")) e.ntt_tile = atoi(v) == 1024 ? 1024 : atoi(v) == 4096 ? 4096 : 2048;
   if (const char* v = getenv("G16_MSM_SORT")) e.msm_sort = v[0];
diff --git a/nim_groth16_amd/csrc/key_plan.hpp b/nim_groth16_amd/csrc/key_plan.hpp
--- a/nim_groth16_amd/csrc/key_plan.hpp
+++ b/nim_groth16_amd/csrc/key_plan.hpp
@@ -3,6 +3,7 @@
 #include <stdint.h>
 
 #include "g16_env.hpp"
+#include "ntt_plan.hpp"
 
 namespace g16 {
 
@@ -44,4 +45,59 @@
   return source != LIVE_NONE && points_sparse(dead, nw, env);
 }
 
+constexpr uint32_t QUOT_SYM_MAX = 4;
+inline bool quot_sym_active(size_t asym_rows, uint32_t log2n, const G16Env& env) {
+  return env.quot_sym && asym_rows <= QUOT_SYM_MAX && ntt_npass(ntt_geom(env.ntt_tile), log2n) <= 2;
 }
+
+struct CoeffList {
+  const unsigned char* base;
+  size_t count, stride, value_off;
+};
+inline uint32_t coeff_u32(const unsigned char* p) {
+  return (uint32_t)p[0] | (uint32_t)p[1] << 8 | (uint32_t)p[2] << 16 | (uint32_t)p[3] << 24;
+}
+inline size_t quot_sym_scratch_words(size_t count, size_t nrows, size_t ncols) {
+  return (nrows > ncols ? nrows : ncols) + 1 + 2 * count;
+}
+inline size_t quot_sym_rows(const CoeffList& c, size_t nrows, size_t ncols, uint32_t* scratch,
+                            uint32_t rows[QUOT_SYM_MAX]) {
+  const size_t nbins = nrows > ncols ? nrows : ncols;
+  uint32_t* const cnt = scratch;
+  uint32_t* const by_col = scratch + nbins + 1;
+  uint32_t* const by_row = by_col + c.count;
+  auto ent = [&](size_t e) { return c.base + e * c.stride; };
+  auto live = [&](const unsigned char* p) {
+    return coeff_u32(p) <= 1 && coeff_u32(p + 4) < nrows && coeff_u32(p + 8) < ncols;
+  };
+  for (size_t i = 0; i <= nbins; ++i) cnt[i] = 0;
+  for (size_t e = 0; e < c.count; ++e)
+    if (live(ent(e))) ++cnt[coeff_u32(ent(e) + 8) + 1];
+  for (size_t i = 0; i < nbins; ++i) cnt[i + 1] += cnt[i];
+  const size_t nlive = cnt[nbins];
+  for (size_t e = 0; e < c.count; ++e)
+    if (live(ent(e))) by_col[cnt[coeff_u32(ent(e) + 8)]++] = (uint32_t)e;
+  for (size_t i = 0; i <= nbins; ++i) cnt[i] = 0;
+  for (size_t i = 0; i < nlive; ++i) ++cnt[coeff_u32(ent(by_col[i]) + 4) + 1];
+  for (size_t i = 0; i < nbins; ++i) cnt[i + 1] += cnt[i];
+  for (size_t i = 0; i < nlive; ++i) by_row[cnt[coeff_u32(ent(by_col[i]) + 4)]++] = by_col[i];
+  size_t nasym = 0;
+  for (size_t r = 0, lo = 0; r < nrows; ++r) {
+    const size_t hi = cnt[r];
+    bool sym = ((hi - lo) & 1) == 0;
+    for (size_t i = lo; sym && i < hi; i += 2) {
+      const unsigned char *p = ent(by_row[i]), *q = ent(by_row[i + 1]);
+      sym = coeff_u32(p) != coeff_u32(q) && coeff_u32(p + 8) == coeff_u32(q + 8) &&
+            (i == lo || coeff_u32(p + 8) != coeff_u32(ent(by_row[i - 1]) + 8));
+      for (size_t b = 0; sym && b < 32; ++b) sym = p[c.value_off + b] == q[c.value_off + b];
+    }
+    if (!sym) {
+      if (nasym < QUOT_SYM_MAX) rows[nasym] = (uint32_t)r;
+      ++nasym;
+    }
+    lo = hi;
+  }
+  return nasym;
+}
+
+}
diff --git a/nim_groth16_amd/csrc/ntt.cuh b/nim_groth16_amd/csrc/ntt.cuh
--- a/nim_groth16_amd/csrc/ntt.cuh
+++ b/nim_groth16_amd/csrc/ntt.cuh
@@ -128,7 +128,7 @@
 
   u256* twl = lds + tile;
   for (uint32_t t = tid; t < (R >> 1); t += BLOCK) twl[t] = ntt_tw(tw, t << (log2n - rho), log2n, inverse);
-  if (mul_src && blockIdx.y == 2) {
+  if (mul_src && blockIdx.y == (uint32_t)mul_src) {
     const u256* xa = x - 2 * xstride;
     const u256* xb = x - xstride;
     for (uint32_t e = tid; e < tile; e += BLOCK) {
@@ -166,11 +166,18 @@
   }
 }
 
-template <int BLOCK, int TILE>
+struct QuotSym {
+  const u256* t0;
+  const u256* ab;
+  uint32_t k;
+  uint32_t rows[4];
+};
+constexpr uint32_t QUOT_SYM_ROWS = 4;
+template <int BLOCK, int TILE, int NV>
 static __global__ void __launch_bounds__(BLOCK) ntt_last_pass_abc(const u256* __restrict__ x, u256* __restrict__ out,
                                                                const u256* __restrict__ tw, uint32_t log2n,
                                                                uint32_t log2s, uint32_t rho, uint32_t log2b,
-                                                               size_t xstride, int mul_invz) {
+                                                               size_t xstride, int mul_invz, QuotSym sym) {
   extern __shared__ __align__(16) unsigned char smem[];
   u256* lds = reinterpret_cast<u256*>(smem);
   constexpr int PER = TILE / BLOCK;
@@ -181,9 +188,10 @@
   const uint32_t tid = threadIdx.x;
   u256* twl = lds + tile;
   for (uint32_t t = tid; t < (R >> 1); t += BLOCK) twl[t] = ntt_tw(tw, t << (log2n - rho), log2n, 0);
+  const uint32_t s_mask = (1u << log2s) - 1;
   u256 acc[PER];
 #pragma unroll 1
-  for (int v = 0; v < 3; ++v) {
+  for (int v = 0; v < NV; ++v) {
     const u256* xv = x + xstride * v;
     for (uint32_t e = tid; e < tile; e += BLOCK) {
       uint32_t b = e & (B - 1), r = e >> log2b;
@@ -197,12 +205,25 @@
       if (e < tile) {
         uint32_t b = e & (B - 1), q = e >> log2b;
         u256 z = lds[(bitrev(q, rho) << log2b) | b];
-        acc[i] = v == 0 ? z : v == 1 ? Fr::mul(acc[i], z) : Fr::sub(acc[i], z);
+        if constexpr (NV == 3) {
+          acc[i] = v == 0 ? z : v == 1 ? Fr::mul(acc[i], z) : Fr::sub(acc[i], z);
+        } else if (v == 0) {
+          const uint32_t base = base0 + b;
+          const uint32_t oi = (base & s_mask) + ((((base >> log2s) << rho) + q) << log2s);
+          const uint32_t n = 1u << log2n;
+          u256 a1 = z;
+          for (uint32_t r = 0; r < sym.k; ++r) {
+            const u256 e = Fr::sub(sym.ab[sym.rows[r]], sym.ab[(size_t)n + sym.rows[r]]);
+            a1 = Fr::add(a1, Fr::mul(e, sym.t0[(oi - sym.rows[r]) & (n - 1)]));
+          }
+          acc[i] = Fr::mul(a1, z);
+        } else {
+          acc[i] = Fr::sub(acc[i], z);
+        }
       }
     }
     __syncthreads();
   }
-  const uint32_t s_mask = (1u << log2s) - 1;
 #pragma unroll
   for (int i = 0; i < PER; ++i) {
     const uint32_t e = tid + i * BLOCK;
diff --git a/nim_groth16_amd/csrc/ntt.hip b/nim_groth16_amd/csrc/ntt.hip
--- a/nim_groth16_amd/csrc/ntt.hip
+++ b/nim_groth16_amd/csrc/ntt.hip
@@ -37,11 +37,15 @@
   static_assert((size_t(32) * NTT_TILE) + (size_t(16) << NTT_MAX_RHO) <= 160 * 1024, "tile + twiddles must fit the LDS");
   HIPCHK(ctx, hipFuncSetAttribute(reinterpret_cast<const void*>(&ntt_pass<NTT_BLOCK>),
                                   hipFuncAttributeMaxDynamicSharedMemorySize, max_shmem));
-  HIPCHK(ctx, hipFuncSetAttribute(reinterpret_cast<const void*>(&ntt_last_pass_abc<NTT_BLOCK, NTT_TILE>),
+  HIPCHK(ctx, hipFuncSetAttribute(reinterpret_cast<const void*>(&ntt_last_pass_abc<NTT_BLOCK, NTT_TILE, 3>),
+                                  hipFuncAttributeMaxDynamicSharedMemorySize, max_shmem));
+  HIPCHK(ctx, hipFuncSetAttribute(reinterpret_cast<const void*>(&ntt_last_pass_abc<NTT_BLOCK, NTT_TILE, 2>),
                                   hipFuncAttributeMaxDynamicSharedMemorySize, max_shmem));
   HIPCHK(ctx, hipFuncSetAttribute(reinterpret_cast<const void*>(&ntt_pass<NTT_BLOCK_MID>),
                                   hipFuncAttributeMaxDynamicSharedMemorySize, max_shmem));
-  HIPCHK(ctx, hipFuncSetAttribute(reinterpret_cast<const void*>(&ntt_last_pass_abc<NTT_BLOCK_MID, NTT_TILE_MID>),
+  HIPCHK(ctx, hipFuncSetAttribute(reinterpret_cast<const void*>(&ntt_last_pass_abc<NTT_BLOCK_MID, NTT_TILE_MID, 3>),
+                                  hipFuncAttributeMaxDynamicSharedMemorySize, max_shmem));
+  HIPCHK(ctx, hipFuncSetAttribute(reinterpret_cast<const void*>(&ntt_last_pass_abc<NTT_BLOCK_MID, NTT_TILE_MID, 2>),
                                   hipFuncAttributeMaxDynamicSharedMemorySize, max_shmem));
   done.store(true, std::memory_order_release);
   return G16_OK;
@@ -49,18 +53,22 @@
 
 struct NttKernels {
   uint32_t block;
-  decltype(&ntt_last_pass_abc<NTT_BLOCK, NTT_TILE>) last_pass_abc;
+  decltype(&ntt_last_pass_abc<NTT_BLOCK, NTT_TILE, 3>) last_pass_abc;
   decltype(&ntt_pass<NTT_BLOCK>) pass;
+  decltype(&ntt_last_pass_abc<NTT_BLOCK, NTT_TILE, 2>) last_pass_bc;
 };
 static const NttKernels ntt_kernels[3] = {
-    {NTT_BLOCK_SMALL, ntt_last_pass_abc<NTT_BLOCK_SMALL, NTT_TILE_SMALL>, ntt_pass<NTT_BLOCK_SMALL>},
-    {NTT_BLOCK_MID, ntt_last_pass_abc<NTT_BLOCK_MID, NTT_TILE_MID>, ntt_pass<NTT_BLOCK_MID>},
-    {NTT_BLOCK, ntt_last_pass_abc<NTT_BLOCK, NTT_TILE>, ntt_pass<NTT_BLOCK>},
+    {NTT_BLOCK_SMALL, ntt_last_pass_abc<NTT_BLOCK_SMALL, NTT_TILE_SMALL, 3>, ntt_pass<NTT_BLOCK_SMALL>,
+     ntt_last_pass_abc<NTT_BLOCK_SMALL, NTT_TILE_SMALL, 2>},
+    {NTT_BLOCK_MID, ntt_last_pass_abc<NTT_BLOCK_MID, NTT_TILE_MID, 3>, ntt_pass<NTT_BLOCK_MID>,
+     ntt_last_pass_abc<NTT_BLOCK_MID, NTT_TILE_MID, 2>},
+    {NTT_BLOCK, ntt_last_pass_abc<NTT_BLOCK, NTT_TILE, 3>, ntt_pass<NTT_BLOCK>, ntt_last_pass_abc<NTT_BLOCK, NTT_TILE, 2>},
 };
+static_assert(QUOT_SYM_ROWS == QUOT_SYM_MAX, "ntt.cuh and key_plan.hpp disagree on the rows a symmetric quotient corrects");
 
 static int32_t ntt_batched(g16_ctx* ctx, const u256* in, size_t in_stride, u256* out, size_t out_stride,
                            uint32_t batch, uint32_t log2n, int inverse, const u256* scale, int fuse_abc = 0,
-                           int c_from_ab = 0) {
+                           int c_from_ab = 0, const QuotSym* sym = nullptr) {
   const size_t n = size_t(1) << log2n;
   int32_t rc;
   if ((rc = ensure_twiddles(ctx, log2n))) return rc;
@@ -86,15 +94,21 @@
     const NttPass plan = ntt_pass_plan(geom, log2n, p);
     const bool last = p + 1 == npass;
     if (last && fuse_abc) {
-      KLAUNCH(ctx, "ntt_last_pass_abc", K.last_pass_abc, plan.ntiles, K.block, plan.shmem, src, out,
-              (const u256*)ctx->ntt_tw.p(), log2n, plan.log2s, plan.rho, plan.log2b, src_stride, fuse_abc == 2 ? 1 : 0);
+      if (sym)
+        KLAUNCH(ctx, "ntt_last_pass_abc", K.last_pass_bc, plan.ntiles, K.block, plan.shmem, src, out,
+                (const u256*)ctx->ntt_tw.p(), log2n, plan.log2s, plan.rho, plan.log2b, src_stride, fuse_abc == 2 ? 1 : 0,
+                *sym);
+      else
+        KLAUNCH(ctx, "ntt_last_pass_abc", K.last_pass_abc, plan.ntiles, K.block, plan.shmem, src, out,
+                (const u256*)ctx->ntt_tw.p(), log2n, plan.log2s, plan.rho, plan.log2b, src_stride, fuse_abc == 2 ? 1 : 0,
+                QuotSym{});
       break;
     }
     u256* dst = last ? out : ((p & 1) ? tmpB : tmpA);
     const size_t dst_stride = last ? out_stride : n;
     KLAUNCH(ctx, inverse ? "ntt_pass_inv" : "ntt_pass_fwd", K.pass, dim3(plan.ntiles, batch), K.block, plan.shmem, src, dst,
             (const u256*)ctx->ntt_tw.p(), log2n, plan.log2s, plan.rho, plan.log2b, inverse, last ? 1 : 0, src_stride,
-            dst_stride, last ? scale : (const u256*)nullptr, p == 0 ? c_from_ab : 0);
+            dst_stride, last ? scale : (const u256*)nullptr, p == 0 && c_from_ab ? (int)batch - 1 : 0);
     src = dst;
     src_stride = dst_stride;
   }
@@ -125,7 +139,7 @@
 }
 
 int32_t g16_quotient_device(g16_ctx* ctx, const void* d_a, const void* d_b, const void* d_c, uint32_t log2n,
-                            int flavour, void* d_out, int c_from_ab) {
+                            int flavour, void* d_out, int c_from_ab, const g16_quot_sym* sym) {
   if (log2n > 27) {
     ctx->err = "quotient needs the 2n domain: log2n <= 27";
     return G16_EINVAL;
@@ -140,6 +154,25 @@
   if (c_from_ab && ((const u256*)d_b != in + n || (const u256*)d_c != in + 2 * n || log2n == 0)) {
     ctx->err = "quotient: Cz can only be formed on the fly from contiguous Az | Bz | Cz";
     return G16_EINVAL;
+  }
+  if (sym) {
+    if ((const u256*)d_b != in + n || (const u256*)d_c != in + 2 * n || sym->k > QUOT_SYM_MAX || (sym->k && !sym->d_t0)) {
+      ctx->err = "quotient: the symmetric path needs contiguous Az | Bz | Cz and the key's table";
+      return G16_EINVAL;
+    }
+    QuotSym qs{(const u256*)sym->d_t0, in, sym->k, {0, 0, 0, 0}};
+    for (uint32_t r = 0; r < sym->k; ++r) {
+      if (sym->rows[r] >= n) {
+        ctx->err = "quotient: asymmetric row outside the domain";
+        return G16_EINVAL;
+      }
+      qs.rows[r] = sym->rows[r];
+    }
+    if ((rc = ntt_batched(ctx, in + n, n, X, n, 2, log2n, 1, (const u256*)ctx->coset[0].p(), 0, c_from_ab))) return rc;
+    if (flavour == 1) return ntt_batched(ctx, X, n, (u256*)d_out, 0, 2, log2n, 0, nullptr, 1, 0, &qs);
+    if ((rc = ensure_coset(ctx, log2n, 1))) return rc;
+    if ((rc = ntt_batched(ctx, X, n, Y, 0, 2, log2n, 0, nullptr, 2, 0, &qs))) return rc;
+    return ntt_batched(ctx, Y, n, (u256*)d_out, n, 1, log2n, 1, (const u256*)ctx->coset[1].p());
   }
   if ((const u256*)d_b != in + n || (const u256*)d_c != in + 2 * n) {
     HIPCHK(ctx, hipMemcpyAsync(X, d_a, n * 32, hipMemcpyDeviceToDevice, ctx->stream));
diff --git a/nim_groth16_amd/csrc/pkey.hip b/nim_groth16_amd/csrc/pkey.hip
--- a/nim_groth16_amd/csrc/pkey.hip
+++ b/nim_groth16_amd/csrc/pkey.hip
@@ -4,6 +4,7 @@
 
 #include "pkey.hpp"
 #include "b1_fold.cuh"
+#include "setup.cuh"
 
 using namespace g16;
 
@@ -33,6 +34,12 @@
 extern "C" int32_t g16_pkey_b1_sparse(const g16_pkey* k, size_t out[3]) {
   if (!k || !out) return G16_EINVAL;
   out[0] = k->b1_sparse ? 1 : 0, out[1] = k->b1_nlive, out[2] = B1_SPARSE_MAX;
+  return G16_OK;
+}
+
+extern "C" int32_t g16_pkey_quot_sym(const g16_pkey* k, size_t out[3]) {
+  if (!k || !out) return G16_EINVAL;
+  out[0] = k->quot_sym ? 1 : 0, out[1] = k->quot_asym_rows, out[2] = QUOT_SYM_MAX;
   return G16_OK;
 }
 
@@ -242,6 +249,37 @@
                           cs.stride, cs.count ? cs.base + cs.value_off : nullptr, cs.stride, &k->abc, cs.values_r2);
 }
 
+static int32_t quotient_symmetry(g16_ctx* ctx, const g16_pkey_desc* d, const CoeffSource& cs, g16_pkey* k) {
+  const size_t n = size_t(1) << d->log2_domain;
+  std::vector<uint32_t> scratch;
+  try {
+    scratch.resize(quot_sym_scratch_words(cs.count, n, d->nvars));
+  } catch (const std::bad_alloc&) {
+    ctx->err = "out of host memory";
+    return G16_ENOMEM;
+  }
+  k->quot_asym_rows = quot_sym_rows(CoeffList{cs.base, cs.count, cs.stride, cs.value_off}, n, d->nvars, scratch.data(),
+                                    k->quot_rows);
+  k->quot_sym = quot_sym_active(k->quot_asym_rows, d->log2_domain, g16_env());
+  if (!k->quot_sym || !k->quot_asym_rows) return G16_OK;
+  const u256 omega = setup_omega(d->log2_domain), eta = setup_omega(d->log2_domain + 1);
+  const u256 omega_inv = setup_pow_u32(omega, (uint32_t)(n - 1));
+  u256 c = Fr::add(Fr::one(), Fr::one());
+  for (uint32_t i = 0; i < d->log2_domain; ++i) c = Fr::div2(c);
+  c = Fr::neg(c);
+  HIPCHK(ctx, dev_alloc(k->quot_t0, n * sizeof(u256)));
+  uint32_t first_zero = 0;
+  const int32_t rc = counted_launch(ctx, 0xff, &first_zero, 1, [&](uint32_t* d_first_zero) {
+    return g16_setup_geometric(ctx, true, Fr::one(), omega_inv, c, eta, n, k->quot_t0.get(), d_first_zero);
+  });
+  if (rc) return rc;
+  if (first_zero != 0xffffffffu) {
+    ctx->err = "the table of the symmetric quotient met a zero denominator";
+    return G16_EINVAL;
+  }
+  return G16_OK;
+}
+
 static int32_t pkey_create(g16_ctx* ctx, const g16_pkey_desc* d, const CoeffSource& cs, uint32_t table_stride,
                            g16_pkey** out) {
   if (!desc_well_formed(d)) {
@@ -263,6 +301,7 @@
   if ((rc = g16_points_register_g1_lean(ctx, (const char*)d->pointsH1 + 64 * k->h.lo, k->h.size(), ts, &k->H1))) return rc;
   if ((rc = live_lists(ctx, k.get()))) return rc;
   if ((rc = bin_coefficients(ctx, d, cs, k.get()))) return rc;
+  if ((rc = quotient_symmetry(ctx, d, cs, k.get()))) return rc;
   *out = k.release();
   return G16_OK;
 }
diff --git a/nim_groth16_amd/csrc/pkey.hpp b/nim_groth16_amd/csrc/pkey.hpp
--- a/nim_groth16_amd/csrc/pkey.hpp
+++ b/nim_groth16_amd/csrc/pkey.hpp
@@ -22,4 +22,8 @@
   static constexpr size_t B1_VIEW_WORDS = 16;
   DevMem<uint32_t> b1_sparse;
   uint32_t b1_nlive = 0;
+  bool quot_sym = false;
+  size_t quot_asym_rows = 0;
+  uint32_t quot_rows[g16::QUOT_SYM_MAX] = {0, 0, 0, 0};
+  DevMem<g16::u256> quot_t0;
 };
diff --git a/nim_groth16_amd/csrc/proof_plan.hpp b/nim_groth16_amd/csrc/proof_plan.hpp
--- a/nim_groth16_amd/csrc/proof_plan.hpp
+++ b/nim_groth16_amd/csrc/proof_plan.hpp
@@ -52,6 +52,7 @@
   bool liveA, liveB;
   bool cfg_equal;
   int b1_form = B1_PLAIN;
+  bool quot_sym = false;
 };
 
 constexpr size_t G2_FIRST_MAX = size_t(1) << 18;
@@ -177,7 +178,7 @@
   const int fly = s.log2n >= 1 && env.cz_on_the_fly ? 1 : 0;
   if (!env.quotient_first) proof_plan_witness(p, env, s, EV_NONE);
   p.push(OP_BUILD_ABC, PS_MAIN, fly == 0);
-  p.push(OP_QUOTIENT, PS_MAIN, fly);
+  p.push(OP_QUOTIENT, PS_MAIN, fly, s.quot_sym && env.quot_sym ? 1 : 0);
   if (env.quotient_first) {
     if (s.nh) p.push(OP_SORT_H, PS_MAIN);
     int after = EV_NONE;
diff --git a/nim_groth16_amd/csrc/prover.hip b/nim_groth16_amd/csrc/prover.hip
--- a/nim_groth16_amd/csrc/prover.hip
+++ b/nim_groth16_amd/csrc/prover.hip
@@ -32,7 +32,7 @@
 
 static ProofShape proof_shape(const g16_pkey* k) {
   return ProofShape{k->w.size(), k->h.size(), k->log2n, k->liveA != nullptr, (bool)k->liveB,
-                    k->C1->cfg() == k->H1->cfg(), k->b1_form};
+                    k->C1->cfg() == k->H1->cfg(), k->b1_form, k->quot_sym};
 }
 
 struct ProofArgs {
@@ -99,9 +99,13 @@
         rc = g16_msm_sort(ctx, st, d_qs_slice, G16_SCALARS_MONT, nh, k->H1->cfg(), ctx->sort[SORT_H]);
         break;
       case OP_BUILD_ABC: rc = build_abc_device(ctx, k, d_w, wit_mont, d_abc, s.a != 0); break;
-      case OP_QUOTIENT:
-        rc = g16_quotient_device(ctx, d_abc, d_abc + n, d_abc + 2 * n, k->log2n, (int)k->flavour, d_qs, s.a);
-        break;
+      case OP_QUOTIENT: {
+        g16_quot_sym sym{k->quot_t0.get(), (uint32_t)k->quot_asym_rows, {0, 0, 0, 0}};
+        if (s.b) memcpy(sym.rows, k->quot_rows, sizeof sym.rows);
+        rc = g16_quotient_device(ctx, d_abc, d_abc + n, d_abc + 2 * n, k->log2n, (int)k->flavour, d_qs, s.a,
+                                 s.b ? &sym : nullptr);
+        break;
+      }
       case OP_COSET: {
         const int at = __builtin_popcount(task_mask & ((1u << s.a) - 1));
         rc = g16_coset_pipeline_device(ctx, d_abc + s.a * n, k->log2n, a.task_out + at * n);
```

Result: faster. 136.0 proofs/s, median of 6 (+2.1%).
